# Bostanabad-Research-Group/GP-Plus

Hardware: AMD Instinct MI355X
Metric: MLL evals/sec (fwd+grad), NxN exact GP, N=20k d=8 (higher is better)
Workload: dtype f64; 1 GPU; C2: synthetic Borehole (Sobol seed 0, unique rows, z-scored) N=20000 d=8 fp64, GP_Plus Rough_RBF exact GP at theta1, one replica per GPU (restart-parallel); N=20000, d=8, streams_per_gpu=1

## Files before the change

### gp-plus_amd/_lib.py

```python
from __future__ import annotations

import ctypes
import os
import subprocess
from ctypes import POINTER, c_char_p, c_double, c_int, c_int32, c_int64, c_size_t, c_void_p
from pathlib import Path

import torch

_PKG_DIR = Path(__file__).resolve().parent
_LIB_PATH = _PKG_DIR / "libgpp_hip.so"
_CSRC = _PKG_DIR / "csrc"

_SIGNATURES = {
    "gpp_version": (c_char_p, []),
    "gpp_create": (c_int, [POINTER(c_void_p), c_int]),
    "gpp_destroy": (c_int, [c_void_p]),
    "gpp_set_stream": (c_int, [c_void_p, c_void_p]),
    "gpp_internal_stream": (c_int, [c_void_p, c_int, POINTER(c_void_p)]),
    "gpp_set_option": (c_int, [c_void_p, c_int, c_int]),
    "gpp_workspace_bytes": (c_size_t, [c_void_p, c_int, c_int64, c_int64, c_int, c_int]),
    "gpp_set_workspace": (c_int, [c_void_p, c_void_p, c_size_t]),
    "gpp_kernel_build": (c_int, [c_void_p, c_void_p, c_int64, c_int, c_void_p, c_void_p, c_void_p, c_void_p, c_int,
                                 c_double, c_int, c_int, c_int, c_void_p, c_int64, c_int64, c_int64]),
    "gpp_cross_kernel": (c_int, [c_void_p, c_void_p, c_int64, c_void_p, c_int64, c_int, c_void_p, c_void_p, c_int,
                                 c_int, c_void_p, c_int64]),
    "gpp_kernel_apply": (c_int, [c_void_p, c_void_p, c_int64, c_void_p, c_int64, c_int, c_void_p, c_void_p, c_int, c_int, c_void_p,
                                 c_int64, c_int, c_double, c_void_p, c_int64]),
    "gpp_rff_apply": (c_int, [c_void_p, c_void_p, c_int64, c_int, c_void_p, c_void_p, c_int64, c_void_p, c_void_p, c_int64, c_int,
                              c_double, c_void_p, c_int64]),
    "gpp_kernel_apply_grad": (c_int, [c_void_p, c_void_p, c_int64, c_void_p, c_int64, c_int, c_void_p, c_void_p, c_int, c_int, c_void_p,
                                      c_int64, c_int, c_void_p, c_int64, c_double, c_void_p, c_int64]),
    "gpp_rff_apply_grad": (c_int, [c_void_p, c_void_p, c_int64, c_int, c_void_p, c_void_p, c_int64, c_void_p, c_void_p, c_int64, c_int,
                                   c_void_p, c_int64, c_double, c_void_p, c_int64]),
    "gpp_potrf": (c_int, [c_void_p, c_void_p, c_int64, c_int64, c_void_p, c_int64, c_void_p]),
    "gpp_potrf_ws": (c_int, [c_void_p, c_void_p, c_int64, c_int64, c_void_p, c_int64, c_void_p, c_int64, c_void_p]),
    "gpp_build_potrf_ws": (c_int, [c_void_p, c_void_p, c_int64, c_int, c_void_p, c_void_p, c_void_p, c_void_p, c_int, c_double, c_int,
                                   c_int, c_void_p, c_int64, c_void_p, c_int64, c_void_p, c_int64, c_void_p]),
    "gpp_trtri": (c_int, [c_void_p, c_void_p, c_int64, c_int64, c_void_p, c_int64, c_void_p, c_int64]),
    "gpp_lauum": (c_int, [c_void_p, c_void_p, c_int64, c_int64, c_void_p, c_int64]),
    "gpp_lauum_grad": (c_int, [c_void_p, c_void_p, c_int64, c_int64, c_void_p, c_int, c_void_p, c_void_p, c_void_p, c_int, c_int, c_int,
                               c_void_p, c_void_p, c_void_p, c_void_p]),
    "gpp_post_cov_train": (c_int, [c_void_p, c_void_p, c_int64, c_int64, c_void_p, c_void_p, c_int, c_void_p, c_double, c_void_p,
                                   c_int64]),
    "gpp_syrk_rows": (c_int, [c_void_p, c_void_p, c_int64, c_void_p, c_int64, c_int64, c_int64, c_int64, c_int64, c_int, c_int]),
    "gpp_gemm_lower_cols": (c_int, [c_void_p, c_void_p, c_int64, c_void_p, c_int64, c_void_p, c_int64, c_int64, c_int64, c_double,
                                    c_double, c_int64, c_int64, c_int, c_int, c_int64, c_int64, c_int]),
    "gpp_shard_list_begin": (c_int, [c_void_p, c_int64, c_int64, c_int, c_int, c_void_p, c_int64, c_void_p, c_void_p, c_int64, c_void_p,
                                     c_void_p, c_void_p, c_void_p, c_int64, c_void_p, c_int, POINTER(c_int)]),
    "gpp_shard_piece_cols": (c_int64, []),
    "gpp_shard_list_gate": (c_int, [c_void_p, c_void_p, c_int, c_int]),
    "gpp_shard_list_signal": (c_int, [c_void_p, c_void_p, c_int, c_int]),
    "gpp_shard_list_end": (c_int, [c_void_p]),
    "gpp_set_comm": (c_int, [c_void_p, c_void_p, c_int, c_int]),
    "gpp_comm_unique_id": (c_int, [c_void_p]),
    "gpp_comm_init_rccl": (c_int, [c_void_p, c_void_p, c_int, c_int]),
    "gpp_shard_buffer_doubles": (c_size_t, [c_int64, c_int64, c_int, c_int, c_int]),
    "gpp_shard_eval": (c_int, [c_void_p, c_int64, c_int64, c_void_p, c_int, c_void_p, c_void_p, c_void_p, c_void_p, c_int, c_int, c_int,
                               c_double, c_int, c_int, c_void_p, POINTER(c_int)]),
    "gpp_push_create": (c_int, [c_int, c_int, c_int, c_int64, POINTER(c_void_p), c_void_p]),
    "gpp_push_connect": (c_int, [c_void_p, c_void_p]),
    "gpp_push_send": (c_int, [c_void_p, c_void_p, c_int64, c_void_p, c_int, c_int, POINTER(c_void_p), POINTER(c_int64), POINTER(c_int64),
                              POINTER(c_int64), POINTER(c_int64), POINTER(c_int64)]),
    "gpp_push_recv": (c_int, [c_void_p, c_void_p, c_int64, c_void_p, c_int, c_int, POINTER(c_void_p), POINTER(c_int64), POINTER(c_int64),
                              POINTER(c_int64), POINTER(c_int64), POINTER(c_int64)]),
    "gpp_push_ack": (c_int, [c_void_p, c_void_p, c_int64]),
    "gpp_push_info": (c_int, [c_void_p, POINTER(c_int64), POINTER(c_int)]),
    "gpp_push_destroy": (c_int, [c_void_p, c_int]),
    "gpp_shard_back_list": (c_int, [c_void_p, c_int64, c_int64, c_int, c_int, c_void_p, c_int64, c_void_p, c_void_p, c_int64, c_void_p,
                                    c_void_p, c_int, POINTER(c_int)]),
    "gpp_trmv_lower_cols": (c_int, [c_void_p, c_void_p, c_int64, c_int64, c_void_p, c_void_p, c_int64, c_int, c_int, c_int, c_int]),
    "gpp_mll_scalars": (c_int, [c_void_p, c_void_p, c_int64, c_int64, c_void_p, c_void_p]),
    "gpp_grad_reduce_cols": (c_int, [c_void_p, c_void_p, c_int64, c_int, c_void_p, c_void_p, c_void_p, c_int, c_int, c_int,
                                     c_void_p, c_void_p, c_int64, c_int, c_int64, c_int, c_int, c_void_p, c_void_p, c_void_p,
                                     c_void_p, c_int]),
    "gpp_lauum_rows": (c_int, [c_void_p, c_void_p, c_int64, c_int64, c_void_p, c_int64, c_int, c_int]),
    "gpp_lauum_rows_range": (c_int, [c_void_p, c_void_p, c_int64, c_int64, c_void_p, c_int64, c_int, c_int, c_int64, c_int64]),
    "gpp_transpose": (c_int, [c_void_p, c_void_p, c_int64, c_int64, c_int64, c_void_p, c_int64]),
    "gpp_mll_reduce": (c_int, [c_void_p, c_void_p, c_int64, c_void_p, c_int64, c_int64, c_void_p, c_void_p, c_void_p]),
    "gpp_alpha": (c_int, [c_void_p, c_void_p, c_int64, c_int64, c_void_p, c_void_p]),
    "gpp_grad_reduce": (c_int, [c_void_p, c_void_p, c_int64, c_int, c_void_p, c_void_p, c_void_p, c_int, c_int, c_int,
                                c_void_p, c_void_p, c_int64, c_int, c_void_p, c_void_p, c_void_p, c_void_p]),
    "gpp_loo_scalars": (c_int, [c_void_p, c_void_p, c_int64, c_int64, c_void_p, c_void_p, c_void_p, c_void_p, c_void_p, c_void_p, c_void_p,
                                c_void_p]),
    "gpp_sym_rowscale": (c_int, [c_void_p, c_void_p, c_int64, c_int64, c_void_p, c_void_p, c_int64]),
    "gpp_loo_grad_reduce": (c_int, [c_void_p, c_void_p, c_int64, c_int, c_void_p, c_void_p, c_void_p, c_int, c_int, c_int,
                                    c_void_p, c_void_p, c_void_p, c_int64, c_int, c_void_p, c_void_p, c_void_p, c_void_p]),
    "gpp_grad_reduce_rows": (c_int, [c_void_p, c_void_p, c_int64, c_int, c_void_p, c_void_p, c_void_p, c_int, c_int, c_int,
                                     c_void_p, c_void_p, c_int64, c_int, c_int64, c_int, c_int, c_void_p, c_void_p, c_void_p,
                                     c_void_p]),
    "gpp_predict": (c_int, [c_void_p, c_void_p, c_int64, c_int64, c_void_p, c_void_p, c_int64, c_int64, c_void_p,
                            c_void_p, c_int64, c_void_p, c_void_p]),
    "gpp_predict_tn": (c_int, [c_void_p, c_void_p, c_int64, c_int64, c_void_p, c_void_p, c_int64, c_int64, c_void_p,
                               c_void_p, c_int64, c_void_p, c_void_p]),
    "gpp_cross_grad": (c_int, [c_void_p, c_void_p, c_int64, c_void_p, c_int64, c_int, c_void_p, c_void_p, c_int, c_int, c_void_p,
                               c_void_p, c_void_p, c_void_p, c_int64, c_void_p, c_int, c_void_p, c_int, c_void_p, c_void_p]),
    "gpp_gemm": (c_int, [c_void_p, c_int, c_int, c_int64, c_int64, c_int64, c_double, c_void_p, c_int64, c_void_p,
                         c_int64, c_double, c_void_p, c_int64, c_int, c_int, c_int, c_int, c_int]),
    "gpp_gemm_batched": (c_int, [c_void_p, c_int, c_int, c_int64, c_int64, c_int64, c_double, c_void_p, c_int64, c_int64,
                                 c_void_p, c_int64, c_int64, c_double, c_void_p, c_int64, c_int64, c_int, c_int, c_int, c_int,
                                 c_int, c_int]),
    "gpp_kernel_build_batched": (c_int, [c_void_p, c_void_p, c_int64, c_int64, c_int, c_void_p, c_void_p, c_void_p, c_void_p, c_int,
                                         c_double, c_int, c_int, c_int, c_void_p, c_int64, c_int64, c_int]),
    "gpp_potrf_batched": (c_int, [c_void_p, c_void_p, c_int64, c_int64, c_int64, c_void_p, c_int64, c_int64, c_void_p, c_int]),
    "gpp_trtri_batched": (c_int, [c_void_p, c_void_p, c_int64, c_int64, c_int64, c_void_p, c_int64, c_int64, c_void_p, c_int64,
                                  c_int64, c_int]),
    "gpp_lauum_batched": (c_int, [c_void_p, c_void_p, c_int64, c_int64, c_int64, c_void_p, c_int64, c_int64, c_int]),
    "gpp_mll_reduce_batched": (c_int, [c_void_p, c_void_p, c_int64, c_int64, c_void_p, c_int64, c_int64, c_int64, c_void_p,
                                       c_void_p, c_int64, c_void_p, c_int]),
    "gpp_alpha_batched": (c_int, [c_void_p, c_void_p, c_int64, c_int64, c_int64, c_void_p, c_void_p, c_int64, c_int]),
    "gpp_grad_reduce_batched": (c_int, [c_void_p, c_void_p, c_int64, c_int64, c_int, c_void_p, c_void_p, c_void_p, c_int, c_int,
                                        c_int, c_void_p, c_int64, c_void_p, c_int64, c_int64, c_int, c_void_p, c_void_p, c_void_p,
                                        c_void_p, c_int]),
    "gpp_loo_scalars_batched": (c_int, [c_void_p, c_void_p, c_int64, c_int64, c_int64, c_void_p, c_void_p, c_void_p, c_void_p, c_void_p,
                                        c_void_p, c_void_p, c_int64, c_void_p, c_int]),
    "gpp_sym_rowscale_batched": (c_int, [c_void_p, c_void_p, c_int64, c_int64, c_int64, c_void_p, c_int64, c_void_p, c_int64, c_int64,
                                         c_int]),
    "gpp_loo_grad_reduce_batched": (c_int, [c_void_p, c_void_p, c_int64, c_int64, c_int, c_void_p, c_void_p, c_void_p, c_int, c_int,
                                            c_int, c_void_p, c_void_p, c_int64, c_void_p, c_int64, c_int64, c_int, c_void_p, c_void_p,
                                            c_void_p, c_void_p, c_int]),
    "gpp_cv_blocks": (c_int, [c_void_p, c_void_p, c_int64, c_int64, c_void_p, c_void_p, c_int, c_int, c_void_p, c_int64, c_int64]),
    "gpp_cv_rows": (c_int, [c_void_p, c_void_p, c_int64, c_int64, c_void_p, c_void_p, c_int, c_void_p, c_int64, c_int64, c_void_p,
                            c_int64]),
    "gpp_chol_append": (c_int, [c_void_p, c_void_p, c_int64, c_void_p, c_int64, c_int64, c_int64, c_void_p, c_int64, c_void_p, c_int64,
                                c_void_p, c_void_p, c_void_p, c_void_p]),
    "gpp_post_cross_sq": (c_int, [c_void_p, c_void_p, c_int64, c_void_p, c_int64, c_int, c_void_p, c_void_p, c_int, c_int, c_void_p,
                                  c_int64, c_void_p, c_int64, c_int64, c_int, c_void_p, c_void_p]),
    "gpp_post_cross_min": (c_int, [c_void_p, c_void_p, c_int64, c_void_p, c_int64, c_int, c_void_p, c_void_p, c_int, c_int, c_void_p,
                                   c_int64, c_void_p, c_int64, c_int64, c_int, c_void_p, c_void_p, c_void_p, c_int, c_void_p]),
}

_lib = None


class GppError(RuntimeError):
    """A libgpp_hip call returned a non-zero status."""


def build(force: bool = False) -> Path:
    if force:
        subprocess.run(["make", "-C", str(_CSRC), "clean"], check=True, capture_output=True)
    proc = subprocess.run(["make", "-C", str(_CSRC), "-j4"], capture_output=True, text=True)
    if proc.returncode != 0:
        raise RuntimeError("building libgpp_hip.so failed:\n" + proc.stdout + proc.stderr)
    return _LIB_PATH


def load() -> ctypes.CDLL:
    global _lib
    if _lib is not None:
        return _lib
    if not _LIB_PATH.exists():
        raise GppError(
            f"{_LIB_PATH} not found: the HIP extension is required (build it with "
            f"`make -C {_CSRC}` or `python -c 'import __graft_entry__ as g; g.build()'`); there is no CPU fallback."
        )
    lib = ctypes.CDLL(os.fspath(_LIB_PATH))
    for name, (restype, argtypes) in _SIGNATURES.items():
        fn = getattr(lib, name)
        fn.restype = restype
        fn.argtypes = argtypes
    _lib = lib
    return lib


def exported_symbols() -> list:
    return sorted(_SIGNATURES)


def check(status: int, what: str) -> None:
    if status == 0:
        return
    if status < 0:
        raise GppError(f"{what}: bad argument #{-status}")
    raise GppError(f"{what}: HIP runtime error {status - 1000}")
```

### gp-plus_amd/backend.py

```python
from __future__ import annotations

import atexit
import ctypes
import os
import threading
import weakref
from typing import Dict, Optional, Tuple

import torch

from . import _lib, settings
from ._lib import GppError, check

KIND_RBF, KIND_MATERN32, KIND_MATERN52 = 0, 1, 2
UPLO_FULL, UPLO_LOWER, UPLO_UPPER = 0, 1, 2
OPT_COOP_PANEL, OPT_PANEL_FAULT, OPT_PANEL_TIMEOUT_MS, OPT_EXEC_SCHED, OPT_DAG_SCHED = 1, 2, 3, 4, 5
OPT_GEMM_TILE = 6
OP_MLL_EVAL, OP_PREDICT, OP_PREDICT_GRAD = 0, 1, 2
OP_APPLY = 3
OP_APPLY_GRAD = 4
OP_APPEND = 5
OP_POST_CROSS = 6
OP_POST_CROSS_MIN = 7
MAX_NODES = 64
APPLY_SPLIT = 2048
NOT_SUPPORTED = 2001
NO_WORKSPACE = 2002
MAX_FEATURES = 64


def _check_features(D: int) -> None:
    if D < 1 or D > MAX_FEATURES:
        raise GppError(f"the covariance kernels take 1..{MAX_FEATURES} feature columns per point (got {D})")

_contexts: Dict[Tuple[int, int], "GppContext"] = {}
_contexts_lock = threading.Lock()


def _ptr(t: Optional[torch.Tensor]) -> Optional[int]:
    return None if t is None else t.data_ptr()


def _need(t: torch.Tensor, dtype, name: str) -> None:
    if not t.is_cuda:
        raise GppError(f"{name} must live on the GPU (got {t.device}); libgpp_hip has no CPU path")
    if t.dtype != dtype:
        raise GppError(f"{name} must be {dtype} (got {t.dtype})")
    if not t.is_contiguous() and t.dim() == 1:
        raise GppError(f"{name} must be contiguous")


INFO_PANEL_TIMEOUT = 1 << 30
INFO_EXEC_TIMEOUT = (1 << 30) | (1 << 29)


def check_status(info: int) -> None:
    if info >= INFO_PANEL_TIMEOUT:
        what = "an executor launch" if info & (1 << 29) else "the cooperative panel kernel"
        raise GppError(f"gpp_potrf: {what} timed out waiting for one of its work-groups (another kernel holding the stream's CUs "
                       "for seconds, or a caller-supplied CU-masked stream with fewer CUs than the launch assumed); "
                       "GPP_COOP_PANEL=0 selects the leaf-step factorisation, GPP_DAG_SCHED=0 the launch-per-product one")


def panel_timed_out(ctx: "GppContext", info: int) -> bool:
    if info < INFO_PANEL_TIMEOUT:
        return False
    import warnings

    ms = info & 0xFFFFF
    if info & (1 << 29):
        if not ctx.dag_sched:
            check_status(info)
        warnings.warn(f"libgpp_hip: an executor launch timed out after {ms} ms (another tenant of this GPU held part of its CUs, or "
                      "dispatches are serialised); this context now factors with one launch per product", RuntimeWarning)
        ctx.set_option(OPT_DAG_SCHED, 0)
        return True
    if not ctx.coop_panel:
        check_status(info)
    warnings.warn(f"libgpp_hip: a cooperative panel launch timed out after {ms} ms (another tenant of this GPU held part "
                  "of its CUs); this context now factors with leaf-step launches", RuntimeWarning)
    ctx.set_option(OPT_COOP_PANEL, 0)
    return True


def row_stride(n: int) -> int:
    return max(16, (n + 15) // 16 * 16)


def rows_buffer(m: int, n: int, device) -> torch.Tensor:
    return torch.empty((m, row_stride(n)), dtype=torch.float64, device=device)[:, :n]


def square_buffer(n: int, device) -> torch.Tensor:
    return rows_buffer(n, n, device)


def _ld(m: torch.Tensor) -> int:
    if m.dim() != 2 or m.stride(1) != 1:
        raise GppError("matrix must be 2-D with unit column stride")
    return m.stride(0) if m.shape[0] > 1 else max(m.shape[1], m.stride(0))


def _on_own_device(fn):
    import functools

    @functools.wraps(fn)
    def wrapper(self, *args, **kwargs):
        if torch.cuda.current_device() == self.index:
            return fn(self, *args, **kwargs)
        with torch.cuda.device(self.index):
            return fn(self, *args, **kwargs)

    return wrapper


class GppContext:
    def __init__(self, device: torch.device):
        if device.type != "cuda":
            raise GppError("GppContext needs a cuda (HIP) device; there is no CPU fallback")
        if not torch.cuda.is_available():
            raise GppError("no GPU visible to PyTorch: the HIP path cannot run")
        self.lib = _lib.load()
        self.device = device
        self.index = device.index if device.index is not None else torch.cuda.current_device()
        h = ctypes.c_void_p()
        with torch.cuda.device(self.index):
            check(self.lib.gpp_create(ctypes.byref(h), self.index), "gpp_create")
        self.h = h
        self.coop_panel = settings.ENV_COOP_PANEL
        self.dag_sched = settings.ENV_DAG_SCHED
        if any(os.environ.get(v, "0") not in ("", "0") for v in ("HIP_LAUNCH_BLOCKING", "AMD_SERIALIZE_KERNEL", "CUDA_LAUNCH_BLOCKING")):
            self.set_option(OPT_DAG_SCHED, 0)
        self._ws: Optional[torch.Tensor] = None

    def _stream(self) -> None:
        s = torch.cuda.current_stream(self.index).cuda_stream
        check(self.lib.gpp_set_stream(self.h, ctypes.c_void_p(s)), "gpp_set_stream")

    def set_option(self, option: int, value: int) -> None:
        check(self.lib.gpp_set_option(self.h, int(option), int(value)), "gpp_set_option")
        if option == OPT_COOP_PANEL:
            self.coop_panel = bool(value)
        elif option in (OPT_DAG_SCHED, OPT_EXEC_SCHED):
            self.dag_sched = bool(value)

    @_on_own_device
    def internal_streams(self):
        if getattr(self, "_istreams", None) is None:
            out = []
            for which in (0, 1, 2):
                p = ctypes.c_void_p()
                check(self.lib.gpp_internal_stream(self.h, which, ctypes.byref(p)), "gpp_internal_stream")
                out.append(torch.cuda.ExternalStream(p.value, device=self.device))
            self._istreams = tuple(out)
        return self._istreams

    @_on_own_device
    def ensure_workspace(self, op: int, N: int, M: int, D: int, S: int) -> None:
        need = int(self.lib.gpp_workspace_bytes(self.h, op, N, M, D, S))
        if self._ws is None or self._ws.numel() < need:
            self._ws = torch.empty(need, dtype=torch.uint8, device=self.device)
            check(self.lib.gpp_set_workspace(self.h, self._ws.data_ptr(), self._ws.numel()), "gpp_set_workspace")

    def _check_groups(self, grp: torch.Tensor, N: int, S: int) -> None:
        _need(grp, torch.int32, "grp")
        if grp.numel() != N:
            raise GppError(f"noise-group index has {grp.numel()} entries for {N} points (stale fidel_indices?)")
        seen = getattr(self, "_grp_ok", None)
        if seen is None or seen[0]() is not grp or seen[1:] != (grp._version, N, S):
            lo, hi = int(grp.min()), int(grp.max())
# ... 16 lines not shown
        if not U.is_contiguous():
            raise GppError("U must be contiguous")
        self._stream()
        check(self.lib.gpp_kernel_build(self.h, U.data_ptr(), N, D, w.data_ptr(), sf2.data_ptr(), _ptr(tau), _ptr(grp), S,
                                        float(jitter), kind, d_split, uplo, out.data_ptr(), _ld(out), row0,
                                        N - row0 if nrows is None else nrows), "gpp_kernel_build")
        return out

    @_on_own_device
    def cross_kernel(self, Ua, Ub, w, sf2, out, *, kind=KIND_RBF, d_split=0):
        _check_features(Ua.shape[1])
        for t, n in ((Ua, "Ua"), (Ub, "Ub"), (w, "w"), (sf2, "sf2"), (out, "Kab")):
            _need(t, torch.float64, n)
        if not (Ua.is_contiguous() and Ub.is_contiguous()):
            raise GppError("Ua/Ub must be contiguous")
        self._stream()
        check(self.lib.gpp_cross_kernel(self.h, Ua.data_ptr(), Ua.shape[0], Ub.data_ptr(), Ub.shape[0], Ua.shape[1],
                                        w.data_ptr(), sf2.data_ptr(), kind, d_split, out.data_ptr(), _ld(out)),
              "gpp_cross_kernel")
        return out

    def _apply_checks(self, Ua, second, C, out, sf2, g_Ua=None):
        M, D = Ua.shape
        L, S = C.shape
        _check_features(D)
        for t, n in ((Ua, "Ua"), (second, "Ub / Omega"), (C, "C / Theta"), (out, "Out")):
            _need(t, torch.float64, n)
        if not (Ua.is_contiguous() and second.is_contiguous()):
            raise GppError("Ua and Ub / Omega must be contiguous")
        if second.shape != (L, D):
            raise GppError(f"the second operand must be {L} x {D} (got {tuple(second.shape)})")
        if out.shape != (M, S):
            raise GppError(f"Out must be {M} x {S} (got {tuple(out.shape)})")
        if min(M, L, S) < 1:
            raise GppError("gpp_kernel_apply / gpp_rff_apply take M, N (F), S >= 1")
        _need(sf2, torch.float64, "sf2")
        if sf2.numel() < 1:
            raise GppError("sf2 must hold one value")
        if g_Ua is not None:
            _need(g_Ua, torch.float64, "g_Ua")
            if g_Ua.shape != (M, D):
                raise GppError(f"g_Ua must be {M} x {D} (got {tuple(g_Ua.shape)})")
        self.ensure_workspace(OP_APPLY if g_Ua is None else OP_APPLY_GRAD, L, M, D, S)
        return M, D, L, S

    @_on_own_device
    def kernel_apply(self, Ua, Ub, w, sf2, C, out, *, beta=0.0, kind=KIND_RBF, d_split=0):
        M, D, N, S = self._apply_checks(Ua, Ub, C, out, sf2)
        _need(w, torch.float64, "w")
        if w.numel() != D:
            raise GppError(f"w has {w.numel()} entries for {D} features")
        self._stream()
        check(self.lib.gpp_kernel_apply(self.h, Ua.data_ptr(), M, Ub.data_ptr(), N, D, w.data_ptr(), sf2.data_ptr(), kind, d_split,
                                        C.data_ptr(), _ld(C), S, float(beta), out.data_ptr(), _ld(out)), "gpp_kernel_apply")
        return out

    @_on_own_device
    def rff_apply(self, Ua, omega, phase, sf2, theta, out, *, beta=0.0):
        M, D, F, S = self._apply_checks(Ua, omega, theta, out, sf2)
        _need(phase, torch.float64, "phase")
        if phase.numel() != F:
            raise GppError(f"phase has {phase.numel()} entries for {F} features")
        self._stream()
        check(self.lib.gpp_rff_apply(self.h, Ua.data_ptr(), M, D, omega.data_ptr(), phase.data_ptr(), F, sf2.data_ptr(),
                                     theta.data_ptr(), _ld(theta), S, float(beta), out.data_ptr(), _ld(out)), "gpp_rff_apply")
        return out

    @_on_own_device
    def kernel_apply_grad(self, Ua, Ub, w, sf2, C, gbar, g_Ua, *, beta=0.0, kind=KIND_RBF, d_split=0):
        M, D, N, S = self._apply_checks(Ua, Ub, C, gbar, sf2, g_Ua)
        _need(w, torch.float64, "w")
        if w.numel() != D:
            raise GppError(f"w has {w.numel()} entries for {D} features")
        self._stream()
        check(self.lib.gpp_kernel_apply_grad(self.h, Ua.data_ptr(), M, Ub.data_ptr(), N, D, w.data_ptr(), sf2.data_ptr(), kind, d_split,
                                             C.data_ptr(), _ld(C), S, gbar.data_ptr(), _ld(gbar), float(beta), g_Ua.data_ptr(),
                                             _ld(g_Ua)), "gpp_kernel_apply_grad")
        return g_Ua

    @_on_own_device
    def rff_apply_grad(self, Ua, omega, phase, sf2, theta, gbar, g_Ua, *, beta=0.0):
        M, D, F, S = self._apply_checks(Ua, omega, theta, gbar, sf2, g_Ua)
        _need(phase, torch.float64, "phase")
        if phase.numel() != F:
            raise GppError(f"phase has {phase.numel()} entries for {F} features")
        self._stream()
        check(self.lib.gpp_rff_apply_grad(self.h, Ua.data_ptr(), M, D, omega.data_ptr(), phase.data_ptr(), F, sf2.data_ptr(),
                                          theta.data_ptr(), _ld(theta), S, gbar.data_ptr(), _ld(gbar), float(beta), g_Ua.data_ptr(),
                                          _ld(g_Ua)), "gpp_rff_apply_grad")
        return g_Ua

    @_on_own_device
    def potrf(self, A, Linv, info, T=None):
        _need(A, torch.float64, "A"); _need(Linv, torch.float64, "Linv"); _need(info, torch.int32, "info")
        self._stream()
        if T is None:
            check(self.lib.gpp_potrf(self.h, A.data_ptr(), A.shape[0], _ld(A), Linv.data_ptr(), _ld(Linv), info.data_ptr()),
                  "gpp_potrf")
        else:
            check(self.lib.gpp_potrf_ws(self.h, A.data_ptr(), A.shape[0], _ld(A), Linv.data_ptr(), _ld(Linv), T.data_ptr(),
                                        _ld(T), info.data_ptr()), "gpp_potrf_ws")

    @_on_own_device
    def build_potrf(self, U, w, sf2, tau, grp, A, Linv, info, T, *, jitter=0.0, kind=KIND_RBF, d_split=0):
        N, D = U.shape
        _check_features(D)
        for t, n in ((U, "U"), (w, "w"), (sf2, "sf2"), (A, "A"), (Linv, "Linv"), (T, "T")):
            _need(t, torch.float64, n)
        _need(info, torch.int32, "info")
        if tau is not None:
            _need(tau, torch.float64, "tau")
        S = 0 if tau is None else tau.numel()
        if grp is not None:
            self._check_groups(grp, N, S)
        if not U.is_contiguous():
            raise GppError("U must be contiguous")
        self._stream()
        check(self.lib.gpp_build_potrf_ws(self.h, U.data_ptr(), N, D, w.data_ptr(), sf2.data_ptr(), _ptr(tau), _ptr(grp), S,
                                          float(jitter), kind, d_split, A.data_ptr(), _ld(A), Linv.data_ptr(), _ld(Linv),
                                          T.data_ptr(), _ld(T), info.data_ptr()), "gpp_build_potrf_ws")

    @_on_own_device
    def trtri(self, U, Linv, T):
        self._stream()
        check(self.lib.gpp_trtri(self.h, U.data_ptr(), U.shape[0], _ld(U), Linv.data_ptr(), _ld(Linv), T.data_ptr(), _ld(T)),
              "gpp_trtri")

    @_on_own_device
    def lauum(self, Linv, Kinv):
        self._stream()
        check(self.lib.gpp_lauum(self.h, Linv.data_ptr(), Linv.shape[0], _ld(Linv), Kinv.data_ptr(), _ld(Kinv)), "gpp_lauum")

    @_on_own_device
    def lauum_grad(self, Linv, U, w, sf2, grp, S, alpha, dU, g_w, g_sf2, g_tau, *, kind=KIND_RBF) -> bool:
        N, D = U.shape
        for t, n in ((Linv, "Linv"), (U, "U"), (w, "w"), (sf2, "sf2"), (alpha, "alpha"), (g_w, "g_w"), (g_sf2, "g_sf2"),
                     (g_tau, "g_tau")):
            _need(t, torch.float64, n)
        if grp is not None:
            self._check_groups(grp, N, S)
        if not U.is_contiguous():
            raise GppError("U must be contiguous")
        self.ensure_workspace(OP_MLL_EVAL, N, 0, D, S)
        self._stream()
        status = self.lib.gpp_lauum_grad(self.h, Linv.data_ptr(), N, _ld(Linv), U.data_ptr(), D, w.data_ptr(), sf2.data_ptr(),
                                         _ptr(grp), S, kind, dU, alpha.data_ptr(), g_w.data_ptr(), g_sf2.data_ptr(),
                                         g_tau.data_ptr())
        if status == NOT_SUPPORTED:
            return False
        if status == NO_WORKSPACE:
            raise GppError("gpp_lauum_grad: the handle's scratch workspace is missing or too small")
        check(status, "gpp_lauum_grad")
        return True

    @_on_own_device
    def post_cov_train(self, Kinv, tau, grp, d, out, *, jitter=0.0):
        N = Kinv.shape[0]
        for t, n in ((Kinv, "Kinv"), (tau, "tau"), (out, "A")):
            _need(t, torch.float64, n)
        if d is not None:
            _need(d, torch.float64, "d")
            if d.numel() != N or not d.is_contiguous():
                raise GppError(f"d must be a contiguous vector of {N} doubles")
        if grp is not None:
            self._check_groups(grp, N, tau.numel())
        if out.shape[0] != N or out.shape[1] != N:
            raise GppError("post_cov_train: shapes do not match")
        self._stream()
        check(self.lib.gpp_post_cov_train(self.h, Kinv.data_ptr(), N, _ld(Kinv), tau.data_ptr(), _ptr(grp), tau.numel(), _ptr(d),
                                          float(jitter), out.data_ptr(), _ld(out)), "gpp_post_cov_train")
        return out

    @_on_own_device
    def syrk_rows(self, Urow, C, nb, first_block, rank, nranks):
        self._stream()
        check(self.lib.gpp_syrk_rows(self.h, Urow.data_ptr(), _ld(Urow), C.data_ptr(), _ld(C), C.shape[0], Urow.shape[0], nb,
                                     first_block, rank, nranks), "gpp_syrk_rows")

    @_on_own_device
    def shard_list_begin(self, N, nb, rank, nranks, A, Kc, Lc, D, W, info, workers=0) -> bool:
        self._stream()
        used = ctypes.c_int(0)
        check(self.lib.gpp_shard_list_begin(self.h, N, nb, rank, nranks, A.data_ptr(), _ld(A), Kc.data_ptr(), Lc.data_ptr(), _ld(Kc),
                                            D.data_ptr(), W[0].data_ptr(), W[1].data_ptr(), W[2].data_ptr(), _ld(W[0]),
                                            info.data_ptr(), int(workers), ctypes.byref(used)), "gpp_shard_list_begin")
        return bool(used.value)

    def shard_messages(self, N: int, nb: int, k: int):
        o, o2 = k * nb, min((k + 2) * nb, N)
        W = int(self.lib.gpp_shard_piece_cols()) or N
        return [(o, o2)] + [(c, min(c + W, N)) for c in range(o2, N, W)]

    @_on_own_device
    def shard_list_gate(self, stream, tail: int, k: int) -> None:
        check(self.lib.gpp_shard_list_gate(self.h, ctypes.c_void_p(stream.cuda_stream), int(tail), k), "gpp_shard_list_gate")

    @_on_own_device
    def shard_list_signal(self, stream, tail: int, k: int) -> None:
        check(self.lib.gpp_shard_list_signal(self.h, ctypes.c_void_p(stream.cuda_stream), int(tail), k), "gpp_shard_list_signal")

    @_on_own_device
    def shard_list_end(self) -> None:
        self._stream()
        check(self.lib.gpp_shard_list_end(self.h), "gpp_shard_list_end")

    @_on_own_device
    def shard_back_list(self, N, nb, rank, nranks, A, Kc, Lc, D, info, workers=0) -> bool:
        self._stream()
        used = ctypes.c_int(0)
        check(self.lib.gpp_shard_back_list(self.h, N, nb, rank, nranks, A.data_ptr(), _ld(A), Kc.data_ptr(), Lc.data_ptr(), _ld(Kc),
                                           D.data_ptr(), info.data_ptr(), int(workers), ctypes.byref(used)), "gpp_shard_back_list")
        return bool(used.value)

    @_on_own_device
    def gemm_lower_cols(self, A, B, C, alpha, beta, nb, first_block, rank, nranks, row0=0, row1=None, compact=False):
        M, K = A.shape[1], A.shape[0]
        if compact:
            if B.shape[0] != K or C.shape[0] != M:
                raise GppError("gemm_lower_cols: shapes do not match")
        elif A.shape != B.shape or C.shape[0] != C.shape[1] or C.shape[0] != M:
            raise GppError("gemm_lower_cols: shapes do not match")
        self._stream()
        check(self.lib.gpp_gemm_lower_cols(self.h, A.data_ptr(), _ld(A), B.data_ptr(), _ld(B), C.data_ptr(), _ld(C), M,
                                           K, float(alpha), float(beta), nb, first_block, rank, nranks, row0,
                                           M if row1 is None else row1, 1 if compact else 0),
              "gpp_gemm_lower_cols")

    @_on_own_device
    def trmv_lower_cols(self, T, x, y, nb, rank, nranks, trans=False, compact=False):
        for t, n in ((x, "x"), (y, "y")):
            _need(t, torch.float64, n)
        if trans:
            self.ensure_workspace(OP_MLL_EVAL, T.shape[0], 0, 1, 1)
        self._stream()
        check(self.lib.gpp_trmv_lower_cols(self.h, T.data_ptr(), _ld(T), T.shape[0], x.data_ptr(), y.data_ptr(), nb, rank, nranks,
                                           1 if trans else 0, 1 if compact else 0), "gpp_trmv_lower_cols")

    @_on_own_device
    def mll_scalars(self, U, z, out3):
        self._stream()
        check(self.lib.gpp_mll_scalars(self.h, U.data_ptr(), _ld(U), U.shape[0], z.data_ptr(), out3.data_ptr()), "gpp_mll_scalars")

    @_on_own_device
    def lauum_rows(self, Linv, Kinv, rank, nranks):
        self._stream()
        check(self.lib.gpp_lauum_rows(self.h, Linv.data_ptr(), Linv.shape[0], _ld(Linv), Kinv.data_ptr(), _ld(Kinv), rank, nranks),
              "gpp_lauum_rows")

    @_on_own_device
    def lauum_rows_range(self, Linv, Kinv, rank, nranks, row0, row1):
        self._stream()
        check(self.lib.gpp_lauum_rows_range(self.h, Linv.data_ptr(), Linv.shape[0], _ld(Linv), Kinv.data_ptr(), _ld(Kinv), rank,
                                            nranks, row0, row1), "gpp_lauum_rows_range")

    @_on_own_device
    def transpose(self, src, dst):
        if src.shape[0] != dst.shape[1] or src.shape[1] != dst.shape[0]:
            raise GppError("transpose: shapes do not match")
        self._stream()
        check(self.lib.gpp_transpose(self.h, src.data_ptr(), src.stride(0), src.shape[0], src.shape[1], dst.data_ptr(), dst.stride(0)),
              "gpp_transpose")

    @_on_own_device
    def mll_reduce(self, L, Linv, r, z, out3):
        for t, n in ((r, "r"), (z, "z"), (out3, "out3")):
            _need(t, torch.float64, n)
        self._stream()
        check(self.lib.gpp_mll_reduce(self.h, L.data_ptr(), _ld(L), Linv.data_ptr(), _ld(Linv), L.shape[0], r.data_ptr(),
                                      z.data_ptr(), out3.data_ptr()), "gpp_mll_reduce")

    @_on_own_device
    def alpha(self, Linv, z, alpha):
        N = Linv.shape[0]
        self._stream()
        check(self.lib.gpp_alpha(self.h, Linv.data_ptr(), _ld(Linv), N, z.data_ptr(), alpha.data_ptr()), "gpp_alpha")

    @_on_own_device
    def grad_reduce(self, U, w, sf2, grp, S, alpha, Kinv, dU, g_w, g_sf2, g_tau, g_U, *, kind=KIND_RBF, d_split=0):
        N, D = U.shape
        if grp is not None:
            self._check_groups(grp, N, S)
        self.ensure_workspace(OP_MLL_EVAL, N, 0, D, S)
        self._stream()
        check(self.lib.gpp_grad_reduce(self.h, U.data_ptr(), N, D, w.data_ptr(), sf2.data_ptr(), _ptr(grp), S, kind,
                                       d_split, alpha.data_ptr(), Kinv.data_ptr(), _ld(Kinv), dU, g_w.data_ptr(),
                                       g_sf2.data_ptr(), g_tau.data_ptr(), _ptr(g_U)), "gpp_grad_reduce")

    @_on_own_device
    def loo_scalars(self, Linv, alpha, y, d, mu=None, s2=None, a=None, sqrtb=None, loo=None):
        N = Linv.shape[0]
        _need(Linv, torch.float64, "Linv")
        for t, n, size in ((alpha, "alpha", N), (y, "y", N), (d, "d", N), (mu, "mu", N), (s2, "s2", N), (a, "a", N),
                           (sqrtb, "sqrtb", N), (loo, "loo", 1)):
            if t is None:
                continue
            _need(t, torch.float64, n)
            if t.numel() < size or not t.is_contiguous():
                raise GppError(f"{n} must be a contiguous vector of {size} doubles")
        if mu is not None and y is None:
            raise GppError("loo_scalars: mu needs y")
        self._stream()
        check(self.lib.gpp_loo_scalars(self.h, Linv.data_ptr(), _ld(Linv), N, alpha.data_ptr(), _ptr(y), d.data_ptr(), _ptr(mu),
                                       _ptr(s2), _ptr(a), _ptr(sqrtb), _ptr(loo)), "gpp_loo_scalars")

    @_on_own_device
    def sym_rowscale(self, Kinv, s, out):
# ... 467 lines not shown
```

### gp-plus_amd/csrc/gpp_api.hip

```cpp
#include "../../include/gpp.h"
#include "gpp_internal.h"

#include <algorithm>
#include <cmath>
#include <cstdio>
#include <cstdlib>
#include <cstring>
#include <new>

const GppEnv& gpp_env() {
  static const GppEnv env = [] {
    auto num = [](const char* name, long long unset) { const char* v = getenv(name); return v ? atoll(v) : unset; };
    GppEnv e;
    e.coop_panel = num("GPP_COOP_PANEL", 1) != 0;
    e.dag_sched = num("GPP_DAG_SCHED", 1) != 0;
    e.dag_phased = num("GPP_DAG_PHASED", 0) != 0;
    e.shard_list = num("GPP_SHARD_LIST", 1) != 0;
    e.shard_workers = (int)num("GPP_SHARD_WORKERS", 0);
    e.shard_fill = (int)num("GPP_SHARD_FILL", -1);
    e.shard_timeout_ms = num("GPP_SHARD_TIMEOUT_MS", 60000);
    const int64_t cols = num("GPP_SHARD_PIECE_COLS", 8192);
    e.shard_piece_cols = cols <= 0 ? (int64_t)0 : std::max<int64_t>(GPP_TILE, cols / GPP_TILE * GPP_TILE);
    e.sharded_force_collectives = num("GPP_SHARDED_FORCE_COLLECTIVES", 0) != 0;
    e.exec_verbose = getenv("GPP_EXEC_VERBOSE") != nullptr;
    e.dag_dump = (int)num("GPP_DAG_DUMP", 0);
    e.dag_check_verbose = getenv("GPP_DAG_CHECK_VERBOSE") != nullptr;
    return e;
  }();
  return env;
}

namespace {

constexpr int NBLK = GPP_TILE;
constexpr int64_t LOOKAHEAD_NB = 1024;

inline int rc(hipError_t e) { return e == hipSuccess ? 0 : 1000 + (int)e; }
#define GPP_TRY(expr)                   \
  do {                                  \
    hipError_t _e = (expr);             \
    if (_e != hipSuccess) return rc(_e); \
  } while (0)

inline bool aligned16(const void* p) { return (reinterpret_cast<uintptr_t>(p) & 15) == 0; }

GemmArgs mk(const double* A, int64_t lda, const double* B, int64_t ldb, double* C, int64_t ldc, int64_t M, int64_t N,
            int64_t K, double alpha, double beta) {
  GemmArgs g{};
  g.A = A; g.B = B; g.C = C;
  g.lda = lda; g.ldb = ldb; g.ldc = ldc;
  g.M = (int)M; g.N = (int)N; g.K = (int)K;
  g.alpha = alpha; g.beta = beta;
  return g;
}

inline int64_t split(int64_t n) {
  int64_t h = ((n / 2 + NBLK - 1) / NBLK) * NBLK;
  if (h >= n) h -= NBLK;
  return h;
}

struct Ctx {
  hipStream_t s;
  double* A; int64_t ld;
  double* Li; int64_t ldi;
  int32_t* info;
};

hipError_t trsm_rec(const Ctx& c, int64_t c0, int64_t m, int64_t o, int64_t n) {
  if (m <= 0 || n <= 0) return hipSuccess;
  if (n <= NBLK) {
    double* Bp = c.A + o * c.ld + c0;
    GemmArgs g = mk(c.Li + o * c.ldi + o, c.ldi, Bp, c.ld, Bp, c.ld, n, m, n, 1.0, 0.0);
    g.a_mask = 1;
    return gpp_launch_gemm(c.s, 2, g, 1, NBLK, (m + NBLK - 1) / NBLK >= 512 ? NBLK : 32);
  }
  const int64_t n1 = split(n), n2 = n - n1;
  hipError_t e = trsm_rec(c, c0, m, o, n1);
  if (e != hipSuccess) return e;
  GemmArgs g = mk(c.A + o * c.ld + (o + n1), c.ld, c.A + o * c.ld + c0, c.ld, c.A + (o + n1) * c.ld + c0, c.ld, n2, m, n1,
                  -1.0, 1.0);
  e = gpp_launch_gemm(c.s, 2, g, 1);
  if (e != hipSuccess) return e;
  return trsm_rec(c, c0, m, o + n1, n2);
}

constexpr int64_t BLK_MAX = 6144;
hipError_t potrf_blk(const Ctx& c, int64_t o, int64_t n) {
  for (int64_t j0 = 0; j0 < n; j0 += NBLK) {
    const int64_t nb = std::min<int64_t>(NBLK, n - j0), oo = o + j0, rem = n - j0 - nb;
    hipError_t e = gpp_launch_leaf(c.s, c.A + oo * c.ld + oo, c.ld, c.Li + oo * c.ldi + oo, c.ldi, (int)nb, c.info, (int)oo);
    if (e != hipSuccess) return e;
    if (rem == 0) break;
    double* Bp = c.A + oo * c.ld + (oo + nb);
    GemmArgs g = mk(c.Li + oo * c.ldi + oo, c.ldi, Bp, c.ld, Bp, c.ld, nb, rem, nb, 1.0, 0.0);
    g.a_mask = 1;
    e = gpp_launch_gemm(c.s, 2, g, 1, NBLK, 32);
    if (e != hipSuccess) return e;
    GemmArgs u = mk(Bp, c.ld, Bp, c.ld, c.A + (oo + nb) * c.ld + (oo + nb), c.ld, rem, rem, nb, -1.0, 1.0);
    u.c_lower = 2;
    e = gpp_launch_gemm(c.s, 2, u, 1, 32, 32);
    if (e != hipSuccess) return e;
  }
  return hipSuccess;
}

hipError_t potrf_blk_batched(const Ctx& c, int64_t n, int batch, int64_t sA, int64_t sLi) {
  for (int64_t j0 = 0; j0 < n; j0 += NBLK) {
    const int64_t nb = std::min<int64_t>(NBLK, n - j0), oo = j0, rem = n - j0 - nb;
    hipError_t e = gpp_launch_leaf(c.s, c.A + oo * c.ld + oo, c.ld, c.Li + oo * c.ldi + oo, c.ldi, (int)nb, c.info, (int)oo,
                                   batch, sA, sLi);
    if (e != hipSuccess) return e;
    if (rem == 0) break;
    double* Bp = c.A + oo * c.ld + (oo + nb);
    GemmArgs g = mk(c.Li + oo * c.ldi + oo, c.ldi, Bp, c.ld, Bp, c.ld, nb, rem, nb, 1.0, 0.0);
    g.a_mask = 1;
    g.sA = sLi; g.sB = sA; g.sC = sA;
    e = gpp_launch_gemm(c.s, 2, g, batch, NBLK, 32);
    if (e != hipSuccess) return e;
    GemmArgs u = mk(Bp, c.ld, Bp, c.ld, c.A + (oo + nb) * c.ld + (oo + nb), c.ld, rem, rem, nb, -1.0, 1.0);
    u.c_lower = 2;
    u.sA = sA; u.sB = sA; u.sC = sA;
    e = gpp_launch_gemm(c.s, 2, u, batch, 32, 32);
    if (e != hipSuccess) return e;
  }
  return hipSuccess;
}

hipError_t potrf_rec(const Ctx& c, int64_t o, int64_t n) {
  if (n <= 0) return hipSuccess;
  if (n <= NBLK)
    return gpp_launch_leaf(c.s, c.A + o * c.ld + o, c.ld, c.Li + o * c.ldi + o, c.ldi, (int)n, c.info, (int)o);
  if (n <= BLK_MAX) return potrf_blk(c, o, n);
  const int64_t n1 = split(n), n2 = n - n1;
  hipError_t e = potrf_rec(c, o, n1);
  if (e != hipSuccess) return e;
  e = trsm_rec(c, o + n1, n2, o, n1);
  if (e != hipSuccess) return e;
  const double* U12 = c.A + o * c.ld + (o + n1);
  GemmArgs g = mk(U12, c.ld, U12, c.ld, c.A + (o + n1) * c.ld + (o + n1), c.ld, n2, n2, n1, -1.0, 1.0);
  g.c_lower = 2;
  e = gpp_launch_gemm(c.s, 2, g, 1);
  if (e != hipSuccess) return e;
  return potrf_rec(c, o + n1, n2);
}

constexpr int64_t PANEL_MAX_N = 2048;
inline bool panel_fits(const gpp_handle_s* h, int64_t n) {
  return h->coop_panel && h->panel_flags && h->ncu >= 2 && n > 2 * NBLK && n <= PANEL_MAX_N && (n + NBLK - 1) / NBLK <= gpp_panel_max_leaves();
}
hipError_t launch_panel_at(gpp_handle_s* h, const Ctx& c, int64_t o, int64_t n, int max_wgs) {
  if (h->panel_fault) {
    h->panel_fault = 0;
    return gpp_launch_fill_i32(c.s, c.info, 1, GPP_INFO_PANEL_TIMEOUT);
  }
  hipStreamCaptureStatus cap = hipStreamCaptureStatusNone;
  if (hipStreamIsCapturing(c.s, &cap) != hipSuccess) {
    (void)hipGetLastError();
    cap = hipStreamCaptureStatusNone;
  }
  int slot;
  if (cap == hipStreamCaptureStatusActive) slot = GPP_PANEL_RING + (h->cap_next++ % GPP_PANEL_CAP_RING);
  else slot = h->panel_next++ % GPP_PANEL_RING;
  int* fl = reinterpret_cast<int*>(h->panel_flags + (size_t)slot * gpp_panel_flag_bytes());
  return gpp_launch_panel(c.s, c.A, c.ld, c.Li, c.ldi, (int)n, c.info, (int)o, fl, max_wgs, h->panel_timeout_ms);
}

hipError_t launch_panel(gpp_handle_s* h, const Ctx& c, int64_t o, int64_t n, int max_wgs) {
  Ctx b = c;
// ... 438 lines not shown
    (void)hipGetLastError();
    (void)dag_abort(h, P);
  }
  hipEvent_t E = next_event(h), F = next_event(h);
  HIP_TRY(hipEventRecord(E, cu.s));
  HIP_TRY(hipEventRecord(F, cp.s));
  HIP_TRY(hipStreamWaitEvent(cm.s, E, 0));
  HIP_TRY(hipStreamWaitEvent(cm.s, F, 0));
  HIP_TRY(hipEventRecord(P->last_use, cm.s));
  if (perr != hipSuccess) return perr;
  dag_note_inverted(h, P, N);
  *used = true;
  return hipSuccess;
}

inline int64_t owned_cols(int64_t N, int64_t nb, int rank, int nranks) {
  const int64_t nblk = (N + nb - 1) / nb;
  int64_t cols = 0;
  for (int64_t b = rank; b < nblk; b += nranks) cols += std::min(nb, N - b * nb);
  return cols;
}

int check_mat(const void* p, int64_t ld, int64_t n, int argi) {
  if (!p) return -argi;
  if (!aligned16(p) || (ld & 1) || ld < n) return -(argi + 1);
  return 0;
}

}

extern "C" {

#ifndef GPP_SRC_HASH
#define GPP_SRC_HASH "unknown"
#endif
const char* gpp_version(void) { return "gpp_hip 0.3 (gfx950, fp64 MFMA) src " GPP_SRC_HASH; }

#ifdef GPP_PANEL_STAMP
int gpp_debug_panel_flags(gpp_handle_t h, int* out, int nints, int* next_slot) {
  if (next_slot) *next_slot = h->panel_next % GPP_PANEL_RING;
  return (int)hipMemcpy(out, h->panel_flags, (size_t)nints * sizeof(int), hipMemcpyDeviceToHost);
}
#endif

static DagPlan* dag_mru(gpp_handle_t h) {
  DagPlan* P = nullptr;
  if (h)
    for (int i = 0; i < GPP_DAG_PLANS; ++i)
      if (h->dag_plans[i] && (!P || h->dag_plans[i]->stamp > P->stamp)) P = h->dag_plans[i];
  return P;
}
int gpp_debug_split_builds(gpp_handle_t h) { return h ? h->split_builds : -1; }
int gpp_debug_dag_info(gpp_handle_t h, int64_t* info8) {
  const DagPlan* P = dag_mru(h);
  if (!P) return -1;
  info8[8] = P->inv_rows;
  info8[9] = P->N;
  info8[0] = (int64_t)P->tasks.size(); info8[1] = (int64_t)P->groups.size(); info8[2] = P->B; info8[3] = P->nt;
  info8[4] = P->ncounters; info8[5] = (int64_t)(P->sim_ms * 1000.0); info8[6] = (int64_t)(P->sim_busy * 1000.0); info8[7] = P->flags;
  return 0;
}
int gpp_debug_dag_counters(gpp_handle_t h, int* out, int nmax) {
  DagPlan* P = dag_mru(h);
  if (!P || !P->d_counters) return -1;
  if (hipDeviceSynchronize() != hipSuccess) return 1;
  std::vector<int> c(P->ncounters);
  if (hipMemcpy(c.data(), P->d_counters, c.size() * sizeof(int), hipMemcpyDeviceToHost) != hipSuccess) return 2;
  int n = 0;
  auto put = [&](int v) { if (n < nmax) out[n++] = v; };
  put(c[0]); put(c[1]); put(P->B);
  for (int b = 0; b < P->B; ++b) put(c[P->c_pd + b]);
  for (int b = 0; b < P->B; ++b) put(c[P->c_g1d + b]);
  if (P->flags & DAG_SHARD) {
    for (int b = 0; b < P->B; ++b) put(c[P->c_cph + b]);
    for (int b = 0; b < P->B; ++b) put(c[P->c_cpt + b * P->GP]);
    for (int b = 0; b < P->B; ++b) put(c[P->c_art + b * P->GP]);
  }
  return n;
}
int gpp_debug_dag_trace(gpp_handle_t h, int on) {
  DagPlan* P = dag_mru(h);
  if (!P) return -1;
  if (hipDeviceSynchronize() != hipSuccess) return 1;
  if (on && !P->d_trace) {
    if (hipMalloc(&P->d_trace, 4 * P->tasks.size() * sizeof(unsigned long long)) != hipSuccess) return 2;
    (void)hipMemset(P->d_trace, 0, 4 * P->tasks.size() * sizeof(unsigned long long));
  } else if (!on && P->d_trace) {
    (void)hipFree(P->d_trace);
    P->d_trace = nullptr;
  }
  return 0;
}
int gpp_debug_dag_fetch(gpp_handle_t h, void* tasks, void* trace) {
  const DagPlan* P = dag_mru(h);
  if (!P) return -1;
  if (hipDeviceSynchronize() != hipSuccess) return 1;
  if (tasks) memcpy(tasks, P->tasks.data(), P->tasks.size() * sizeof(DagTask));
  if (trace) {
    if (!P->d_trace) return 2;
    if (hipMemcpy(trace, P->d_trace, 4 * P->tasks.size() * sizeof(unsigned long long), hipMemcpyDeviceToHost) != hipSuccess) return 3;
  }
  return 0;
}

int gpp_create(gpp_handle_t* out, int device) {
  if (!out) return -1;
  int ndev = 0;
  hipError_t e = hipGetDeviceCount(&ndev);
  if (e != hipSuccess) return rc(e);
  if (device < 0 || device >= ndev) return -2;
  e = hipSetDevice(device);
  if (e != hipSuccess) return rc(e);
  gpp_handle_s* h = new (std::nothrow) gpp_handle_s();
  if (!h) return rc(hipErrorOutOfMemory);
  h->device = device;
  h->stream = nullptr;
  h->ws = nullptr;
  h->ws_bytes = 0;
  h->panel_stream = nullptr;
  h->upd_stream = nullptr;
  h->fill_stream = nullptr;
  h->full_stream = nullptr;
  h->cu_split = -1;
  h->panel_cus = 0;
  h->n_events = 0;
  h->ev_next = 0;
  h->inv_N = 0;
  h->inv_nblocks = 0;
  h->panel_flags = nullptr;
  h->panel_next = 0;
  h->coop_panel = gpp_env().coop_panel ? 1 : 0;
  h->panel_fault = 0;
  h->panel_timeout_ms = 500;
  for (int i = 0; i < GPP_DAG_PLANS; ++i) h->dag_plans[i] = nullptr;
  h->shard_cur = nullptr;
  h->shard_info = nullptr;
  h->shard_ready = nullptr;
  h->dag_clock = 0;
  h->dag_sched = 1;
  h->gemm_tile = 0;
  h->ncu = 0;
  if (hipDeviceGetAttribute(&h->ncu, hipDeviceAttributeMultiprocessorCount, device) != hipSuccess || h->ncu < 2) {
    (void)hipGetLastError();
    h->ncu = 0;
  }
  h->cap_next = 0;
  h->handoff = nullptr;
  if (hipMalloc(reinterpret_cast<void**>(&h->panel_flags), (GPP_PANEL_RING + GPP_PANEL_CAP_RING) * gpp_panel_flag_bytes()) != hipSuccess ||
      hipMemset(h->panel_flags, 0, (GPP_PANEL_RING + GPP_PANEL_CAP_RING) * gpp_panel_flag_bytes()) != hipSuccess) {
    (void)hipGetLastError();
    if (h->panel_flags) (void)hipFree(h->panel_flags);
    h->panel_flags = nullptr;
  }
  *out = h;
  return 0;
}

int gpp_destroy(gpp_handle_t h) {
  if (!h) return -1;
  for (hipStream_t s : {h->panel_stream, h->upd_stream, h->fill_stream, h->full_stream})
    if (s) (void)hipStreamSynchronize(s);
  if (h->full_stream) (void)hipStreamDestroy(h->full_stream);
  if (h->fill_stream) (void)hipStreamDestroy(h->fill_stream);
  if (h->upd_stream) (void)hipStreamDestroy(h->upd_stream);
  if (h->panel_stream) (void)hipStreamDestroy(h->panel_stream);
  for (int i = 0; i < h->n_events; ++i) (void)hipEventDestroy(h->events[i]);
  if (h->handoff) (void)hipEventDestroy(h->handoff);
  if (h->shard_ready) (void)hipEventDestroy(h->shard_ready);
  if (h->panel_flags) (void)hipFree(h->panel_flags);
  for (int i = 0; i < GPP_DAG_PLANS; ++i)
    if (h->dag_plans[i]) gpp_dag_free(h->dag_plans[i]);
  gpp_shard_release_comm(h);
  delete h;
  return 0;
}

int gpp_set_stream(gpp_handle_t h, void* stream) {
  if (!h) return -1;
  hipStream_t s = reinterpret_cast<hipStream_t>(stream);
  if (s != h->stream) {
    hipStreamCaptureStatus a = hipStreamCaptureStatusNone, b = hipStreamCaptureStatusNone;
    if (hipStreamIsCapturing(h->stream, &a) != hipSuccess || hipStreamIsCapturing(s, &b) != hipSuccess) {
      (void)hipGetLastError();
      a = b = hipStreamCaptureStatusActive;
    }
    auto internal = [&](hipStream_t q) { return q && (q == h->panel_stream || q == h->upd_stream || q == h->fill_stream || q == h->full_stream); };
    if (a == hipStreamCaptureStatusNone && b == hipStreamCaptureStatusNone && !internal(s) && !internal(h->stream)) {
      if (!h->handoff) GPP_TRY(hipEventCreateWithFlags(&h->handoff, hipEventDisableTiming));
      GPP_TRY(hipEventRecord(h->handoff, h->stream));
      GPP_TRY(hipStreamWaitEvent(s, h->handoff, 0));
    }
    h->stream = s;
  }
  return 0;
}

int gpp_set_option(gpp_handle_t h, int option, int value) {
  if (!h) return -1;
  if (option == GPP_OPT_COOP_PANEL) h->coop_panel = value ? 1 : 0;
  else if (option == GPP_OPT_PANEL_FAULT) h->panel_fault = value ? 1 : 0;
  else if (option == GPP_OPT_DAG_SCHED || option == GPP_OPT_EXEC_SCHED) h->dag_sched = value ? 1 : 0;
  else if (option == GPP_OPT_PANEL_TIMEOUT_MS) {
    if (value < 1 || value > 60000) return -3;
    h->panel_timeout_ms = value;
  } else if (option == GPP_OPT_GEMM_TILE) {
    if (value < 0 || value > 4) return -3;
    h->gemm_tile = value;
  } else return -2;
  return 0;
}

int gpp_internal_stream(gpp_handle_t h, int which, void** out) {
  if (!h) return -1;
  if (which < 0 || which > 2) return -2;
  if (!out) return -3;
  GPP_TRY(ensure_streams(h));
  *out = reinterpret_cast<void*>(which == 0 ? h->panel_stream : which == 1 ? h->upd_stream : h->full_stream);
  return 0;
}

constexpr int64_t SHARD_LIST_MIN_N = 4096;
static long long shard_budget(const gpp_handle_s* h) {
  (void)h;
  return gpp_env().shard_timeout_ms * 100000;
}

int gpp_shard_list_begin(gpp_handle_t h, int64_t N, int64_t nb, int rank, int nranks, double* A, int64_t ld, double* Kc, double* Lc,
                         int64_t ldc, double* D, double* W0, double* W1, double* W2, int64_t ldw, int32_t* info, int workers,
                         int* used) {
  if (!h) return -1;
  if (!used) return -18;
  *used = 0;
  if (N < 2 || nb < 128 || nb % 128 != 0) return -2;
  if (rank < 0 || nranks < 1 || rank >= nranks) return -4;
  if (int e = check_mat(A, ld, N, 6)) return e;
  if (!Kc || !aligned16(Kc)) return -8;
  if (!Lc || !aligned16(Lc)) return -9;
  const int64_t wc = ((N + nb - 1) / nb - rank + nranks - 1) / nranks * nb;
  if ((ldc & 1) || ldc < wc) return -10;
  if (!D || !aligned16(D)) return -11;
  if (!W0 || !W1 || !W2 || !aligned16(W0) || !aligned16(W1) || !aligned16(W2)) return -12;
  if ((ldw & 1) || ldw < N) return -15;
  if (!info) return -16;
  if (h->shard_cur) return -1;
  const GppEnv& env = gpp_env();
  if (workers <= 0 && env.shard_workers > 0) workers = env.shard_workers;
  if (!env.shard_list || !h->dag_sched || !h->coop_panel || N < SHARD_LIST_MIN_N || N > DAG_MAX_N) return 0;
  GPP_TRY(ensure_streams(h));
  if (h->cu_split != 1) return 0;
  if (!panel_fits(h, nb)) return 0;
  const int flags = DAG_INV | DAG_SHARD;
  const int nworkers = workers > 0 ? workers : 2 * (h->ncu - h->panel_cus);
  DagPlan* P = dag_plan_cached(h, PlanKey{N, nb, ld, ldc, ldw, flags, N, rank, nranks, workers}, [&]() -> DagPlan* {
    DagTuning tune = gpp_dag_default_tuning();
    tune.workers = nworkers;
    tune.fill = env.shard_fill >= 0 ? env.shard_fill : workers > 0 ? 0 : (nranks > 1 ? h->panel_cus : 2 * h->panel_cus);
    tune.inv_rows = 0;
    tune.fuse = dag_fuse(N);
    DagPlan* Q = gpp_dag_plan(N, nb, ld, ldc, ldw, 0, flags, tune, rank, nranks);
    if (!Q) return nullptr;
    Q->workers = workers;
    Q->fill = tune.fill;
    if (gpp_dag_upload(Q) != hipSuccess) {
      (void)hipGetLastError();
      gpp_dag_free(Q);
      return nullptr;
    }
    return Q;
  });
  if (!P) return 0;
  hipStream_t sm = h->stream, sp = h->panel_stream, su = h->upd_stream;
  GPP_TRY(gpp_launch_fill_i32(sm, P->d_counters, P->ncounters, 0));
  DagBases bases{{reinterpret_cast<char*>(A), reinterpret_cast<char*>(Kc), reinterpret_cast<char*>(Lc), reinterpret_cast<char*>(D),
                  reinterpret_cast<char*>(W0), reinterpret_cast<char*>(W1), reinterpret_cast<char*>(W2), nullptr}};
  GPP_TRY(gpp_launch_dag_bind(sm, P->d_groups, P->d_groups_abs, (int)P->groups.size(), bases));
  if (!h->shard_ready) GPP_TRY(hipEventCreateWithFlags(&h->shard_ready, hipEventDisableTiming));
  hipEvent_t ev = h->shard_ready;
  GPP_TRY(hipEventRecord(ev, sm));
  GPP_TRY(hipStreamWaitEvent(sp, ev, 0));
  GPP_TRY(hipStreamWaitEvent(su, ev, 0));
  const long long budget = shard_budget(h);
  DagLaunch dl{};
  dl.groups = P->d_groups_abs; dl.tasks = P->d_tasks; dl.ntasks = (int)P->tasks.size();
  dl.counters = P->d_counters; dl.info = info; dl.budget = budget;
  dl.max_tasks = 0; dl.quit_id = -1; dl.quit_val = 0; dl.ticket_limit = 0;
  dl.trace = P->d_trace; dl.tag = 0;
  if (dl.ntasks > 0) GPP_TRY(gpp_launch_dag(su, nworkers, dl));
  Ctx cp{sp, A, ld, D, nb, info};
  auto enqueue_panel_stream = [&]() -> int {
    for (const DagPlan::Op& op : P->stream_ops) {
      const int b = op.arg;
      const int64_t o = (int64_t)b * nb, rows = std::min(nb, N - o);
      if (op.kind == 0) {
        GPP_TRY(gpp_launch_exec_gate(sp, P->d_counters, P->c_g1d + b, P->gate_target[b], info, budget));
      } else if (op.kind == 1) {
        Ctx cb = cp;
        cb.A = A + o * ld + o;
        cb.Li = D + (int64_t)b * nb * nb;
        GPP_TRY(launch_panel_at(h, cb, o, rows, h->panel_cus));
      } else if (op.kind == 2) {
        GPP_TRY(gpp_launch_exec_signal(sp, P->d_counters, P->c_pd + b));
      } else {
        DagLaunch fl = dl;
        fl.max_tasks = op.arg;
        fl.quit_id = op.n >= 0 ? P->c_g1d + op.n : -1;
        fl.quit_val = 1;
        fl.ticket_limit = op.lim;
        fl.tag = op.n >= 0 ? op.n : P->B;
        GPP_TRY(gpp_launch_dag(sp, std::max(P->fill, 1), fl));
      }
    }
    return 0;
  };
  const int erc = enqueue_panel_stream();
  h->shard_cur = P;
  h->shard_info = info;
  if (erc != 0) {
    (void)hipGetLastError();
    (void)dag_abort(h, P);
    return erc;
  }
  *used = 1;
  return 0;
}

static int shard_pieces(const DagPlan* P, int k) {
  const int hi = P->tb[std::min(k + 2, P->B)];
  return hi >= P->nt ? 0 : (P->nt - hi + P->piece_tiles - 1) / P->piece_tiles;
}
int gpp_shard_list_gate(gpp_handle_t h, void* stream, int tail, int k) {
  if (!h || !h->shard_cur) return -1;
  const DagPlan* P = h->shard_cur;
  if (k < 0 || k >= P->B || k % P->nranks != P->rank) return -4;
  if (tail < 0 || tail > shard_pieces(P, k)) return -3;
  hipStream_t s = reinterpret_cast<hipStream_t>(stream);
  const long long budget = shard_budget(h);
  GPP_TRY(hipStreamWaitEvent(s, h->shard_ready, 0));
  GPP_TRY(gpp_launch_exec_gate(s, P->d_counters, P->c_pd + k, 1, h->shard_info, budget));
  const int piece = k * P->GP + tail - 1;
  const int target = tail ? P->cpt_target[piece] : P->cph_target[k];
  if (target > 0) GPP_TRY(gpp_launch_exec_gate(s, P->d_counters, tail ? P->c_cpt + piece : P->c_cph + k, target, h->shard_info, budget));
  return 0;
}

int gpp_shard_list_signal(gpp_handle_t h, void* stream, int tail, int k) {
  if (!h || !h->shard_cur) return -1;
  const DagPlan* P = h->shard_cur;
  if (k < 0 || k >= P->B || k % P->nranks == P->rank) return -4;
  if (tail < 0 || tail > shard_pieces(P, k)) return -3;
  GPP_TRY(hipStreamWaitEvent(reinterpret_cast<hipStream_t>(stream), h->shard_ready, 0));
  return rc(gpp_launch_exec_signal(reinterpret_cast<hipStream_t>(stream), P->d_counters, tail ? P->c_art + k * P->GP + tail - 1 : P->c_pd + k));
}

int gpp_shard_list_end(gpp_handle_t h) {
// ... 214 lines not shown
  if (ldu < D) return -16;
  if (gpp_apply_pieces(F) > 1 && (!h->ws || h->ws_bytes < gpp_apply_ws_bytes(F, M, D))) return GPP_NO_WORKSPACE;
  GPP_TRY(gpp_launch_rff_apply_grad(h->stream, Ua, M, D, Omega, phase, F, sf2, Theta, ldt, S, Gbar, ldg, beta, g_Ua, ldu, h->ws,
                                    h->ws_bytes));
  return 0;
}

static int potrf_ws_impl(gpp_handle_t h, double* A, int64_t N, int64_t ld, double* Linv, int64_t ldi, double* T, int64_t ldt,
                         int32_t* info_dev, const KyBuild* build) {
  if (!h) return -1;
  if (N < 0) return -3;
  if (int r = check_mat(A, ld, N, 2)) return r;
  if (int r = check_mat(Linv, ldi, N, 5)) return r;
  if (T) {
    if (int r = check_mat(T, ldt, N, 7)) return r;
  }
  if (!info_dev) return -9;
  GPP_TRY(gpp_launch_fill_i32(h->stream, info_dev, 1, 0));
  Ctx c{h->stream, A, ld, Linv, ldi, info_dev};
  h->inv_N = N;
  h->inv_nblocks = 0;
  const int64_t la_min = T ? BORDER_MIN_N : 6 * LOOKAHEAD_NB;
  bool dag_used = false;
  hipStreamCaptureStatus cap = hipStreamCaptureStatusNone;
  if (build) GPP_TRY(hipStreamIsCapturing(h->stream, &cap));
  if (build && cap != hipStreamCaptureStatusNone) {
    GPP_TRY((*build)(h->stream, c, N, 0, N));
    build = nullptr;
  }
  GPP_TRY(potrf_dag(h, c, N, T, ldt, &dag_used, build));
  if (dag_used) return 0;
  if (build) GPP_TRY((*build)(h->stream, c, N, 0, N));
  if (N >= la_min) {
    GPP_TRY(potrf_lookahead(h, c, N, LOOKAHEAD_NB, T, ldt));
  } else if (panel_fits(h, N)) {
    int wgs = h->ncu;
    if (h->cu_split == 1 && h->stream == h->panel_stream) wgs = h->panel_cus;
    else if (h->cu_split == 1 && (h->stream == h->upd_stream || h->stream == h->fill_stream)) wgs = h->ncu - h->panel_cus;
    else if (h->stream) {
      uint32_t mask[32] = {0};
      if (hipExtStreamGetCUMask(h->stream, 32, mask) == hipSuccess) {
        int cus = 0;
        for (int c = 0; c < h->ncu && c < 1024; ++c) cus += (mask[c >> 5] >> (c & 31)) & 1u;
        if (cus >= 2 && cus < wgs) wgs = cus;
      } else {
        (void)hipGetLastError();
      }
    }
    GPP_TRY(launch_panel(h, c, 0, N, wgs));
    h->inv_nblocks = 1;
    h->inv_o[0] = 0;
    h->inv_n[0] = N;
  } else {
    GPP_TRY(potrf_rec(c, 0, N));
  }
  return 0;
}

int gpp_potrf_ws(gpp_handle_t h, double* A, int64_t N, int64_t ld, double* Linv, int64_t ldi, double* T, int64_t ldt,
                 int32_t* info_dev) {
  return potrf_ws_impl(h, A, N, ld, Linv, ldi, T, ldt, info_dev, nullptr);
}

int gpp_build_potrf_ws(gpp_handle_t h, const double* U, int64_t N, int D, const double* w, const double* sf2, const double* tau,
                       const int32_t* grp, int S, double jitter, int kind, int d_split, double* A, int64_t ld, double* Linv,
                       int64_t ldi, double* T, int64_t ldt, int32_t* info_dev) {
  if (!h) return -1;
  if (!U) return -2;
  if (N < 0) return -3;
  if (D < 1 || D > 64) return -4;
  if (!w) return -5;
  if (!sf2) return -6;
  if (tau && S < 1) return -9;
  if (kind < 0 || kind > 2) return -11;
  if (d_split < 0 || d_split > D) return -12;
  if (int r = check_mat(A, ld, N, 13)) return r;
  if (int r = check_mat(Linv, ldi, N, 15)) return r;
  if (T) {
    if (int r = check_mat(T, ldt, N, 17)) return r;
  }
  if (!info_dev) return -19;
  const KyBuild build{U, w, sf2, tau, grp, D, S, kind, d_split, jitter};
  return potrf_ws_impl(h, A, N, ld, Linv, ldi, T, ldt, info_dev, &build);
}

int gpp_potrf(gpp_handle_t h, double* A, int64_t N, int64_t ld, double* Linv, int64_t ldi, int32_t* info_dev) {
  const int r = gpp_potrf_ws(h, A, N, ld, Linv, ldi, nullptr, 0, info_dev);
  return r == -9 ? -7 : r;
}

int gpp_trtri(gpp_handle_t h, const double* U, int64_t N, int64_t ld, double* Linv, int64_t ldi, double* T, int64_t ldt) {
  if (!h) return -1;
  if (N < 0) return -3;
  if (int r = check_mat(U, ld, N, 2)) return r;
  if (int r = check_mat(Linv, ldi, N, 5)) return r;
  if (int r = check_mat(T, ldt, N, 7)) return r;
  const bool have = (h->inv_N == N && h->inv_nblocks > 0);
  for (int64_t s = NBLK; s < N; s *= 2) {
    auto skip = [&](int64_t b) {
      if (!have) return false;
      for (int i = 0; i < h->inv_nblocks; ++i)
        if (b >= h->inv_o[i] && b + 2 * s <= h->inv_o[i] + h->inv_n[i]) return true;
      for (int i = 0; i < h->inv_nblocks; ++i)
        if (b >= h->inv_o[i] && h->inv_o[i] + h->inv_n[i] == N && b + s < N) return true;
      return false;
    };
    GPP_TRY(trtri_level(h->stream, U, ld, Linv, ldi, T, ldt, 0, N, s, skip));
  }
  h->inv_N = 0;
  return 0;
}

int gpp_lauum(gpp_handle_t h, const double* Linv, int64_t N, int64_t ldi, double* Kinv, int64_t ldk) {
  if (!h) return -1;
  if (N < 0) return -3;
  if (int r = check_mat(Linv, ldi, N, 2)) return r;
  if (int r = check_mat(Kinv, ldk, N, 5)) return r;
  GemmArgs g = mk(Linv, ldi, Linv, ldi, Kinv, ldk, N, N, N, 1.0, 0.0);
  g.a_mask = 2; g.b_mask = 2; g.klo_mode = 3; g.c_lower = 1; g.tag = 1;
  const int t = N <= 2560 ? 32 : N <= 5120 ? 64 : NBLK;
  GPP_TRY(gpp_launch_gemm(h->stream, 2, g, 1, t, t));
  return 0;
}

int gpp_lauum_grad(gpp_handle_t h, const double* Linv, int64_t N, int64_t ldi, const double* U, int D, const double* w,
                   const double* sf2, const int32_t* grp, int S, int kind, int dU, const double* alpha, double* g_w,
                   double* g_sf2, double* g_tau) {
  if (!h) return -1;
  if (N < 0) return -3;
  if (int r = check_mat(Linv, ldi, N, 2)) return r;
  if (!U) return -5;
  if (D < 1 || D > 64) return -6;
  if (!w) return -7;
  if (!sf2) return -8;
  if (S < 1 || S > 64) return -10;
  if (kind < 0 || kind > 2) return -11;
  if (dU < 0 || dU > D) return -12;
  if (!alpha) return -13;
  if (!g_w) return -14;
  if (!g_sf2) return -15;
  if (!g_tau) return -16;
  if (kind != GPP_KIND_RBF || D > 16 || dU != 0) return GPP_NOT_SUPPORTED;
  if (!h->ws || h->ws_bytes < gpp_lauum_grad_ws_bytes(N, D)) return GPP_NO_WORKSPACE;
  GemmArgs g = mk(Linv, ldi, Linv, ldi, nullptr, ldi, N, N, N, 1.0, 0.0);
  g.a_mask = 2; g.b_mask = 2; g.klo_mode = 3; g.c_lower = 1;
  const int64_t tiles = (N + NBLK - 1) / NBLK, nrec = tiles * (tiles + 1) / 2;
  double* rec = reinterpret_cast<double*>(h->ws);
  double* wdiag = rec + nrec * (D + 1);
  GPP_TRY(gpp_launch_lauum_grad(h->stream, g, GradEpiArgs{U, w, sf2, alpha, rec, wdiag, D}));
  GPP_TRY(gpp_launch_grad_finish(h->stream, rec, nrec, D, S, wdiag, grp, N, g_w, g_sf2, g_tau));
  return 0;
}

int gpp_post_cov_train(gpp_handle_t h, const double* Kinv, int64_t N, int64_t ldk, const double* tau, const int32_t* grp, int S,
                       const double* d, double jitter, double* A, int64_t lda) {
  if (!h) return -1;
  if (N < 0) return -3;
  if (int r = check_mat(Kinv, ldk, N, 2)) return r;
  if (!tau) return -5;
  if (S < 1) return -7;
  if (int r = check_mat(A, lda, N, 10)) return r;
  if (A == Kinv && lda != ldk) return -11;
  GPP_TRY(gpp_launch_post_cov_train(h->stream, Kinv, ldk, N, tau, grp, d, jitter, A, lda));
  return 0;
}

int gpp_lauum_rows(gpp_handle_t h, const double* Linv, int64_t N, int64_t ldi, double* Kinv, int64_t ldk, int rank, int nranks) {
  if (!h) return -1;
  if (N < 0) return -3;
  if (int r = check_mat(Linv, ldi, N, 2)) return r;
  if (int r = check_mat(Kinv, ldk, N, 5)) return r;
  if (nranks < 1 || rank < 0 || rank >= nranks) return -7;
  GemmArgs g = mk(Linv, ldi, Linv, ldi, Kinv, ldk, N, N, N, 1.0, 0.0);
  g.a_mask = 2; g.b_mask = 2; g.klo_mode = 3; g.c_lower = 1; g.tag = 1;
  g.row_mod = nranks; g.row_off = rank;
  GPP_TRY(gpp_launch_gemm(h->stream, 2, g, 1, NBLK, NBLK));
  return 0;
}

int gpp_lauum_rows_range(gpp_handle_t h, const double* Linv, int64_t N, int64_t ldi, double* Kinv, int64_t ldk, int rank,
                         int nranks, int64_t row0, int64_t row1) {
  if (!h) return -1;
  if (N < 0) return -3;
  if (int r = check_mat(Linv, ldi, N, 2)) return r;
  if (int r = check_mat(Kinv, ldk, N, 5)) return r;
  if (nranks < 1 || rank < 0 || rank >= nranks) return -7;
  if (row0 < 0 || row1 < row0 || row1 > N || (row0 % NBLK) != 0) return -9;
  if (row1 == row0) return 0;
  GemmArgs g = mk(Linv, ldi, Linv, ldi, Kinv, ldk, N, N, N, 1.0, 0.0);
  g.a_mask = 2; g.b_mask = 2; g.klo_mode = 3; g.c_lower = 1; g.tag = 1;
  g.row_mod = nranks; g.row_off = rank;
  const int64_t t0 = row0 / NBLK, t1 = (row1 + NBLK - 1) / NBLK;
  auto first_i = [&](int64_t t) { return t <= rank ? (int64_t)0 : (t - rank + nranks - 1) / nranks; };
  g.row_i0 = (int)first_i(t0);
  g.row_i1 = (int)first_i(t1);
  if (g.row_i1 <= g.row_i0) return 0;
  GPP_TRY(gpp_launch_gemm(h->stream, 2, g, 1, NBLK, NBLK));
  return 0;
}

int gpp_transpose(gpp_handle_t h, const double* src, int64_t lds, int64_t rows, int64_t cols, double* dst, int64_t ldd) {
  if (!h) return -1;
  if (!src || lds < cols) return -2;
  if (rows < 0 || cols < 0) return -4;
  if (!dst || ldd < rows) return -6;
  GPP_TRY(gpp_launch_transpose(h->stream, src, lds, rows, cols, dst, ldd));
  return 0;
}

int gpp_syrk_rows(gpp_handle_t h, const double* Urow, int64_t ldu, double* C, int64_t ldc, int64_t Nt, int64_t K, int64_t nb,
                  int64_t first_block, int rank, int nranks) {
  if (!h) return -1;
  if (!Urow || !aligned16(Urow) || (ldu & 1)) return -2;
  if (!C || !aligned16(C) || (ldc & 1)) return -4;
  if (Nt < 0 || K < 0) return -6;
  if (nb < NBLK || nb % NBLK != 0) return -8;
  if (first_block < 0) return -9;
  if (nranks < 1 || rank < 0 || rank >= nranks) return -10;
  if (Nt == 0 || K == 0) return 0;
  GemmArgs g = mk(Urow, ldu, Urow, ldu, C, ldc, Nt, Nt, K, -1.0, 1.0);
  g.c_lower = 2;
  g.own_mod = nranks;
  g.own_bt = (int)(nb / NBLK);
  g.own_off = (int)(((first_block - rank) % nranks + nranks) % nranks);
  GPP_TRY(gpp_launch_gemm(h->stream, 2, g, 1, NBLK, NBLK));
  return 0;
}

int gpp_gemm_lower_cols(gpp_handle_t h, const double* A, int64_t lda, const double* B, int64_t ldb, double* C, int64_t ldc,
                        int64_t M, int64_t K, double alpha, double beta, int64_t nb, int64_t first_block, int rank, int nranks,
                        int64_t row0, int64_t row1, int compact) {
  if (!h) return -1;
  if (!A || !aligned16(A) || (lda & 1)) return -2;
  if (!B || !aligned16(B) || (ldb & 1)) return -4;
  if (!C || !aligned16(C) || (ldc & 1)) return -6;
  if (M < 0 || K < 0) return -8;
  if (nb < NBLK || nb % NBLK != 0) return -12;
  if (first_block < 0) return -13;
  if (nranks < 1 || rank < 0 || rank >= nranks) return -14;
  if (row0 < 0 || row1 < row0 || row1 > M || row0 % NBLK != 0) return -16;
  if (M == 0 || K == 0 || row1 == row0) return 0;
  GemmArgs g = mk(A, lda, B, ldb, C, ldc, M, M, K, alpha, beta);
  g.c_lower = 1;
  g.row_t0 = (int)(row0 / NBLK);
  g.row_t1 = (int)((row1 + NBLK - 1) / NBLK);
  g.own_mod = nranks;
  g.own_bt = (int)(nb / NBLK);
  g.own_off = (int)(((first_block - rank) % nranks + nranks) % nranks);
  g.compact_bc = compact ? 1 : 0;
  GPP_TRY(gpp_launch_gemm(h->stream, 2, g, 1, NBLK, NBLK));
  return 0;
}

int gpp_trmv_lower_cols(gpp_handle_t h, const double* T, int64_t ldt, int64_t N, const double* x, double* y, int64_t nb, int rank,
                        int nranks, int trans, int compact) {
  if (!h) return -1;
  if (N < 0) return -4;
  if (int q = check_mat(T, ldt, compact ? std::min<int64_t>(N, ldt) : N, 2)) return q;
  if (!x || !aligned16(x)) return -5;
  if (!y) return -6;
  if (nb < 64 || nb % 64 != 0) return -7;
  if (nranks < 1 || rank < 0 || rank >= nranks) return -8;
  if (trans != 0 && trans != 1) return -10;
  if (trans && (!h->ws || h->ws_bytes < gpp_trmv_t_ws_bytes(N))) return -1;
  if (compact && nranks >= 1 && rank >= 0 && ldt < owned_cols(N, nb, rank, nranks)) return -3;
  GPP_TRY(gpp_launch_trmv_lower_cols(h->stream, T, ldt, N, x, y, nb, rank, nranks, trans, h->ws, h->ws_bytes, compact));
  return 0;
}

int gpp_mll_scalars(gpp_handle_t h, const double* U, int64_t ld, int64_t N, const double* z, double* out3) {
  if (!h) return -1;
  if (N < 0) return -4;
  if (int q = check_mat(U, ld, N, 2)) return q;
  if (!z) return -5;
  if (!out3) return -6;
  GPP_TRY(gpp_launch_mll_scalars(h->stream, U, ld, N, z, out3));
  return 0;
}

int gpp_mll_reduce(gpp_handle_t h, const double* U, int64_t ld, const double* Linv, int64_t ldi, int64_t N,
                   const double* r, double* z, double* out3) {
  if (!h) return -1;
  if (N < 0) return -6;
  if (int q = check_mat(U, ld, N, 2)) return q;
  if (int q = check_mat(Linv, ldi, N, 4)) return q;
  if (!r || !aligned16(r)) return -7;
  if (!z) return -8;
  if (!out3) return -9;
  GPP_TRY(gpp_launch_trmv_lower(h->stream, Linv, ldi, N, r, z));
  GPP_TRY(gpp_launch_mll_scalars(h->stream, U, ld, N, z, out3));
  return 0;
}

int gpp_alpha(gpp_handle_t h, const double* Linv, int64_t ldi, int64_t N, const double* z, double* alpha) {
  if (!h) return -1;
  if (N < 0) return -4;
  if (int q = check_mat(Linv, ldi, N, 2)) return q;
  if (!z || !aligned16(z)) return -5;
  if (!alpha) return -6;
  GPP_TRY(gpp_launch_trmv_upper(h->stream, Linv, ldi, N, z, alpha));
  return 0;
}

int gpp_grad_reduce(gpp_handle_t h, const double* U, int64_t N, int D, const double* w, const double* sf2,
                    const int32_t* grp, int S, int kind, int d_split, const double* alpha, const double* Kinv,
                    int64_t ldk, int dU, double* g_w, double* g_sf2, double* g_tau, double* g_U) {
// ... 441 lines not shown
```

### gp-plus_amd/csrc/gpp_gemm.hip

```cpp
#include "../../include/gpp.h"
#include "gpp_internal.h"

#include <algorithm>
#include <atomic>
#include <cstdlib>

typedef double v2d __attribute__((ext_vector_type(2)));
typedef double v4d __attribute__((ext_vector_type(4)));

namespace {

constexpr int BK16 = 16;
constexpr int ldt_mc(int T, int BK = 16) { return BK == 16 ? T + 16 : T + 4; }
constexpr int LDK = BK16 + 2;

__device__ __forceinline__ bool keep_elem(int mask, int k, int row) {
  return (mask == 0) | ((mask == 1) & (k <= row)) | ((mask == 2) & (k >= row));
}

template <int T>
__device__ __forceinline__ unsigned load_kc(const double* __restrict__ P, int64_t ld, int R, int r0, int kb, int kend,
                                            int mask, int tid, v2d (&reg)[T / 32]) {
  unsigned keep = 0;
  const double* ptr[T / 32];
// ... 230 lines not shown
  constexpr bool SPLIT = (VAR == 2 && RB == 16 && CB == 4 && BK == 16);
  if constexpr (SPLIT) {
    if (row0 + TM <= Mld && col0 + TN <= Nld && nch > 1) {
      int k_lo = klo, k_hi = khi;
      if (p.a_mask == 1) k_hi = min(k_hi, row0 + 1);
      if (p.a_mask == 2) k_lo = max(k_lo, row0 + TM - 1);
      if (p.b_mask == 1) k_hi = min(k_hi, col0 + 1);
      if (p.b_mask == 2) k_lo = max(k_lo, col0 + TN - 1);
      int j_lo = (k_lo - klo + BK - 1) / BK, j_hi = (k_hi - klo) / BK;
      j_lo = max(j_lo, 0);
      j_hi = min(j_hi, nch);
      if (j_hi > j_lo) {
        const int ci_lo = p.k_reverse ? nch - j_hi : j_lo, ci_hi = p.k_reverse ? nch - j_lo : j_hi;
        ca = max(ci_lo - 1, 0);
        cb = min(ci_hi - 1, nch - 1);
        if (cb < ca) ca = cb = 0;
      }
    }
  }
  auto general_iter = [&](int c) {
    const int cur = (NBUF == 2) ? (c & 1) : 0;
    const bool more = (c + 1 < nch);
    if (more) stage_load(kpos(c + 1));
    compute(cur);
    if (NBUF == 1) __syncthreads();
    if (more) {
      const int nxt = (NBUF == 2) ? (cur ^ 1) : 0;
      stage_store(smem + nxt * (OPA + OPB), smem + nxt * (OPA + OPB) + OPA);
    }
    __syncthreads();
  };
  int c = 0;
  for (; c < ca; ++c) general_iter(c);
  if constexpr (SPLIT) {
    for (; c < cb; ++c) {
      const int cur = (NBUF == 2) ? (c & 1) : 0, nxt = (NBUF == 2) ? (cur ^ 1) : 0;
      const int kb = kpos(c + 1);
      load_fast<NVA>(ubaseA + (int64_t)kb * stepA, offa, ra);
      load_fast<NVB>(ubaseB + (int64_t)kb * stepB, offb, rb);
      if constexpr (TAG != 0) __builtin_amdgcn_s_setprio(1);
      compute(cur);
      if constexpr (TAG != 0) __builtin_amdgcn_s_setprio(0);
      if (NBUF == 1) __syncthreads();
      store_mc<TM, BK, false, NTH>(smem + nxt * (OPA + OPB), tid, ra, 0);
      store_mc<TN, BK, false, NTH>(smem + nxt * (OPA + OPB) + OPA, tid, rb, 0);
      __syncthreads();
    }
  }
  for (; c < nch; ++c) general_iter(c);
  before_epilogue();
  if constexpr (!__is_same(E, GemmStoreC)) {
    static_assert((VAR == 2 || VAR == 0) && WTM == 64 && WTN == 64 && WR == 2, "accumulator epilogues are written for the big tile");
    epi(acc4, row0, col0, p.M, smem);
    return;
  }

  const double alpha = p.alpha, beta = p.beta;
  constexpr int GA = RB < 4 ? RB : 4;
#pragma unroll
  for (int a0 = 0; a0 < RB; a0 += GA) {
    double cold[GA][CB];
    if (beta != 0.0) {
#pragma unroll
      for (int a = 0; a < GA; ++a) {
        const int m = row0 + wm + 4 * (a0 + a) + lk;
#pragma unroll
        for (int b = 0; b < CB; ++b) {
          const int n = col0 + wn + 16 * b + li;
          const bool ok = (m < p.M) && (n < p.N) && (p.c_lower == 0 || (p.c_lower == 1 ? n <= m : n >= m));
          const double* src = ok ? C + (int64_t)m * p.ldc + n : Cd;
          cold[a][b] = *src;
        }
      }
    }
#pragma unroll
    for (int a = 0; a < GA; ++a) {
      const int m = row0 + wm + 4 * (a0 + a) + lk;
#pragma unroll
      for (int b = 0; b < CB; ++b) {
        const int n = col0 + wn + 16 * b + li;
        const bool ok = (m < p.M) && (n < p.N) && (p.c_lower == 0 || (p.c_lower == 1 ? n <= m : n >= m));
        double v = alpha * acc4[(a0 + a) >> 2][b][(a0 + a) & 3];
        if (beta != 0.0) v = fma(beta, cold[a][b], v);
        if (ok) {
          C[(int64_t)m * p.ldc + n] = v;
          if (C2)
            C2[(int64_t)n * p.ldc2 + m] = v;
        }
      }
    }
  }
}

template <int VAR, int WTM, int WTN, int TAG = 0, int BK = 16, int NBUF = 2, int WR = 2>
__global__ __launch_bounds__(128 * WR, ((VAR == 2 && !(BK > 16 && WTM >= 64)) || WTM < 64) ? 2 : 1) void gpp_gemm_f64(GemmArgs p) {
  constexpr int TM = WR * WTM, TN = 2 * WTN;
  extern __shared__ __attribute__((aligned(16))) double smem[];
  int tm, tn;
  if (p.swz) {
    const int b = blockIdx.x, xcd = b & 7, i = b >> 3;
    const int S = (i >> 6) * 8 + xcd, w = i & 63;
    const int super_n = (p.tiles_n + 7) >> 3;
    const int sm = S / super_n, sn = S - sm * super_n;
    tm = sm * 8 + (w >> 3);
    tn = sn * 8 + (w & 7);
    if (tm >= p.tiles_m || tn >= p.tiles_n) return;
    if ((p.c_lower == 1 && tn > tm) || (p.c_lower == 2 && tn < tm)) return;
  } else {
    const int t = (p.batch_fast ? (int)(blockIdx.x / (unsigned)p.nbatch) : (int)blockIdx.x) + (int)p.tile_base;
    if (p.c_lower == 1 && p.row_mod >= 1) {
      const float a = 0.5f * (float)p.row_mod, b = (float)p.row_off + 1.f - a;
      int i = (int)((-b + sqrtf(b * b + 4.f * a * (float)t)) / (2.f * a));
      auto S = [&](int q) { return q * (p.row_off + 1) + p.row_mod * (q * (q - 1) / 2); };
      while (S(i + 1) <= t) ++i;
      while (S(i) > t) --i;
      tm = p.row_off + p.row_mod * i;
      tn = t - S(i);
    } else if (p.c_lower == 1 && TM == 2 * TN) {
      tm = (int)((sqrtf(4.f * (float)t + 1.f) - 1.f) * 0.5f);
      while ((tm + 1) * (tm + 2) <= t) ++tm;
      while (tm * (tm + 1) > t) --tm;
      tn = t - tm * (tm + 1);
      if (tn >= p.tiles_n) return;
    } else if (p.c_lower) {
      tm = (int)((sqrtf(8.f * (float)t + 1.f) - 1.f) * 0.5f);
      while ((tm + 1) * (tm + 2) / 2 <= t) ++tm;
      while (tm * (tm + 1) / 2 > t) --tm;
      tn = t - tm * (tm + 1) / 2;
      if (p.c_lower == 1 && p.own_mod > 1 && (tn / p.own_bt + p.own_off) % p.own_mod != 0) return;
      if (p.c_lower == 2) {
        const int q = tm;
        tm = tn;
        tn = q;
        if (p.own_mod > 1 && (tm / p.own_bt + p.own_off) % p.own_mod != 0) return;
        if ((tn + 1) * TN <= p.skip_lead) return;
        if (p.row_limit > 0 && tm * TM >= p.row_limit) return;
      }
    } else if (p.col_major) {
      tn = t / p.tiles_m;
      tm = t - tn * p.tiles_m;
    } else {
      tm = t / p.tiles_n;
      tn = t - tm * p.tiles_n;
      if (p.row_reverse) tm = p.tiles_m - 1 - tm;
    }
  }
  const int64_t bi = p.batch_fast ? (int64_t)(blockIdx.x % (unsigned)p.nbatch) : (int64_t)blockIdx.y;
  gemm_tile<VAR, WTM, WTN, TAG, BK, NBUF, WR>(p, tm, tn, p.A + bi * p.sA + (int64_t)blockIdx.z * p.zA, p.B + bi * p.sB + (int64_t)blockIdx.z * p.zB,
                                             p.C + bi * p.sC + (int64_t)blockIdx.z * p.zC,
                                             p.C2 ? p.C2 + bi * p.sC2 + (int64_t)blockIdx.z * p.zC2 : nullptr, smem);

}

__device__ __forceinline__ double wave_sum(double v) {
#pragma unroll
  for (int o = 32; o > 0; o >>= 1) v += __shfl_xor(v, o);
  return v;
}
template <int DT>
struct GradEpilogue {
  GradEpiArgs e;
  int tile;
  static constexpr int T = 128;
  static constexpr int FIXED = 2 * DT * T + 2 * T + DT + 4 * (DT + 1);
  static constexpr int SLAB = (FIXED + 1) & ~1;
  static_assert((SLAB + 16 * 256) * sizeof(double) <= 2 * 2 * BK16 * ldt_mc(T) * sizeof(double), "the epilogue lives in the main loop's LDS");
  __device__ __forceinline__ void operator()(const v4d (&acc4)[4][4], int row0, int col0, int N, double* __restrict__ smem) const {
    const int tid = threadIdx.x, wave = tid >> 6, lane = tid & 63;
    const int wm = (wave >> 1) * 64, wn = (wave & 1) * 64, li = lane & 15, lk = lane >> 4;
    const int D = e.D;
    double* __restrict__ sa = smem;
    double* __restrict__ sb = sa + DT * T;
    double* __restrict__ sal_a = sb + DT * T;
    double* __restrict__ sal_b = sal_a + T;
    double* __restrict__ sw = sal_b + T;
    double* __restrict__ red = sw + DT;
    double* __restrict__ slab = smem + SLAB;
    for (int x = tid; x < DT * T; x += 256) {
      const int d = x / T, r = x - d * T;
      sa[x] = (d < D && row0 + r < N) ? e.U[(int64_t)(row0 + r) * D + d] : 0.0;
      sb[x] = (d < D && col0 + r < N) ? e.U[(int64_t)(col0 + r) * D + d] : 0.0;
    }
    if (tid < T) {
      sal_a[tid] = (row0 + tid < N) ? e.alpha[row0 + tid] : 0.0;
      sal_b[tid] = (col0 + tid < N) ? e.alpha[col0 + tid] : 0.0;
    }
    if (tid < DT) sw[tid] = (tid < D) ? e.w[tid] : 0.0;
    __syncthreads();

    const double sf2 = *e.sf2;
    const GppExpConsts ec = gpp_exp_consts();
    const bool diag_tile = (row0 == col0);
    double my_sf2 = 0.0, my_w[DT];
#pragma unroll
    for (int d = 0; d < DT; ++d) my_w[d] = 0.0;
#pragma unroll
    for (int a4 = 0; a4 < 4; ++a4) {
#pragma unroll
      for (int v = 0; v < 4; ++v)
#pragma unroll
        for (int b = 0; b < 4; ++b) slab[(v * 4 + b) * 256 + tid] = acc4[a4][b][v];
#pragma unroll 1
      for (int h = 0; h < 2; ++h) {
        const int ra = wm + 16 * a4 + 8 * h + lk;
        const int cb = wn + li;
        double r2[2][4];
#pragma unroll
        for (int a = 0; a < 2; ++a)
#pragma unroll
          for (int b = 0; b < 4; ++b) r2[a][b] = 0.0;
#pragma unroll 2
        for (int d = 0; d < DT; ++d) {
          const double ua[2] = {sa[d * T + ra], sa[d * T + ra + 4]};
          const double wd = sw[d];
#pragma unroll
          for (int b = 0; b < 4; ++b) {
            const double ub = sb[d * T + cb + 16 * b];
#pragma unroll
            for (int a = 0; a < 2; ++a) {
              const double df = ua[a] - ub;
              r2[a][b] = fma(wd * df, df, r2[a][b]);
            }
          }
        }
        __asm__ volatile("" ::: "memory");
        double g2[2][4];
#pragma unroll
        for (int a = 0; a < 2; ++a) {
          const int i = row0 + ra + 4 * a;
          const double al_i = sal_a[ra + 4 * a];
#pragma unroll
          for (int b = 0; b < 4; ++b) {
            const int j = col0 + cb + 16 * b;
            const bool ok = (i < N) & (j <= i);
            const double kv = gpp_exp_nonpos(-r2[a][b], ec);
            const double kin = slab[((2 * h + a) * 4 + b) * 256 + tid];
            double Wij = 0.5 * (al_i * sal_b[cb + 16 * b] - kin);
            Wij = ok ? Wij : 0.0;
            const double mult = (i == j) ? 1.0 : 2.0;
            my_sf2 = fma(mult * Wij, kv, my_sf2);
            g2[a][b] = mult * Wij * sf2 * kv;
            if (diag_tile && ok && i == j) e.wdiag[i] = Wij;
          }
        }
#pragma unroll
        for (int d = 0; d < DT; ++d) {
          const double ua[2] = {sa[d * T + ra], sa[d * T + ra + 4]};
          double s = 0.0;
#pragma unroll
          for (int b = 0; b < 4; ++b) {
            const double ub = sb[d * T + cb + 16 * b];
#pragma unroll
            for (int a = 0; a < 2; ++a) {
              const double df = ua[a] - ub;
              s = fma(-g2[a][b] * df, df, s);
            }
          }
          my_w[d] += s;
          __builtin_amdgcn_sched_barrier(0);
        }
      }
    }
#pragma unroll
    for (int q = 0; q <= DT; ++q) {
      const double v = wave_sum(q < DT ? my_w[q < DT ? q : 0] : my_sf2);
      if (lane == 0) red[wave * (DT + 1) + q] = v;
    }
    __syncthreads();
    if (tid <= D) {
      const int q = (tid == D) ? DT : tid;
      e.rec[(int64_t)tile * (D + 1) + tid] = ((red[q] + red[(DT + 1) + q]) + red[2 * (DT + 1) + q]) + red[3 * (DT + 1) + q];
    }
  }
};

template <int DT>
__global__ __launch_bounds__(256, 2) void gpp_lauum_grad_f64(GemmArgs p, GradEpiArgs e) {
  extern __shared__ __attribute__((aligned(16))) double smem[];
  const int t = (int)blockIdx.x;
  int tm = (int)((sqrtf(8.f * (float)t + 1.f) - 1.f) * 0.5f);
  while ((tm + 1) * (tm + 2) / 2 <= t) ++tm;
  while (tm * (tm + 1) / 2 > t) --tm;
  const int tn = t - tm * (tm + 1) / 2;
  gemm_tile<2, 64, 64, 2, 16, 2, 2>(p, tm, tn, p.A, p.B, nullptr, nullptr, smem, GemmNoHook(), GradEpilogue<DT>{e, t});
}

template <bool MAT>
struct PostCrossEpilogue {
  PostCrossArgs e;
  int tile, Mr;
  static constexpr int T = 128, DC = 16;
  static constexpr int SLAB = 2 * DC * T + T + 2 * T;
  static_assert((SLAB & 1) == 0 && (SLAB + 16 * 256) * sizeof(double) <= 2 * 2 * BK16 * ldt_mc(T) * sizeof(double) &&
                    (SLAB + 16 * 256) * sizeof(double) <= 2 * 2 * T * LDK * sizeof(double),
                "the epilogue lives in the main loop's LDS");
  __device__ __forceinline__ void operator()(const v4d (&acc4)[4][4], int row0, int col0, int Mc, double* __restrict__ smem) const {
    const int tid = threadIdx.x, wave = tid >> 6, lane = tid & 63;
    const int wm = (wave >> 1) * 64, wn = (wave & 1) * 64, li = lane & 15, lk = lane >> 4;
    const int D = e.dk & 255, kind = (e.dk >> 8) & 255;
    const int dsp = (!MAT || kind == 0) ? D : (e.dk >> 16);
    double* __restrict__ sa = smem;
    double* __restrict__ sb = sa + DC * T;
    double* __restrict__ som = sb + DC * T;
    double* __restrict__ rs = som + T;
    double* __restrict__ slab = smem + SLAB;
    const double* __restrict__ Uc = e.Uc;
    const double* __restrict__ Ur = e.Ur;
    const double* __restrict__ wp = e.w;
    double* __restrict__ rec = e.rec + (int64_t)tile * T;
    Uc += (int64_t)row0 * (e.dk & 255);
    Ur += (int64_t)col0 * (e.dk & 255);
    int rlim = Mc - row0, clim = Mr - col0;
    asm volatile("" : "+v"(Uc), "+v"(Ur), "+v"(wp), "+v"(rec), "+v"(rlim), "+v"(clim));
    auto stage = [&](int d0) {
      for (int x = tid; x < DC * T; x += 256) {
        const int dd = x / T, r = x - dd * T, d = d0 + dd;
        const bool okd = d < D;
        const double sw = okd ? sqrt(wp[okd ? d : 0]) : 0.0;
        sa[x] = (okd && r < rlim) ? Uc[r * D + d] * sw : 0.0;
        sb[x] = (okd && r < clim) ? Ur[r * D + d] * sw : 0.0;
      }
    };
    if (tid < T) som[tid] = (tid < clim) ? (e.omega ? e.omega[col0 + tid] : 1.0) : 0.0;
    const bool one = (D <= DC);
    if (one) stage(0);
    __syncthreads();

    const double sf2 = *e.sf2;
    const GppExpConsts ec = gpp_exp_consts();
#pragma unroll
    for (int a4 = 0; a4 < 4; ++a4) {
#pragma unroll
      for (int v = 0; v < 4; ++v)
#pragma unroll
        for (int b = 0; b < 4; ++b) slab[(v * 4 + b) * 256 + tid] = acc4[a4][b][v];
#pragma unroll 1
      for (int h = 0; h < 2; ++h) {
        const int ra = wm + 16 * a4 + 8 * h + lk;
        const int cb = wn + li;
        double r2[2][4], r2m[MAT ? 2 : 1][MAT ? 4 : 1];
#pragma unroll
        for (int a = 0; a < 2; ++a)
#pragma unroll
          for (int b = 0; b < 4; ++b) {
            r2[a][b] = 0.0;
            if (MAT) r2m[MAT ? a : 0][MAT ? b : 0] = 0.0;
          }
#pragma unroll 1
        for (int d0 = 0; d0 < D; d0 += DC) {
          if (!one) {
            __syncthreads();
            stage(d0);
            __syncthreads();
          }
          const int nd = min(DC, D - d0);
#pragma unroll 2
          for (int dd = 0; dd < nd; ++dd) {
            const double ua[2] = {sa[dd * T + ra], sa[dd * T + ra + 4]};
            const bool second = MAT && (d0 + dd >= dsp);
#pragma unroll
            for (int b = 0; b < 4; ++b) {
              const double ub = sb[dd * T + cb + 16 * b];
#pragma unroll
              for (int a = 0; a < 2; ++a) {
                const double df = ua[a] - ub;
                if (MAT && second) r2m[MAT ? a : 0][MAT ? b : 0] = fma(df, df, r2m[MAT ? a : 0][MAT ? b : 0]);
                else r2[a][b] = fma(df, df, r2[a][b]);
              }
            }
          }
        }
#pragma unroll
        for (int a = 0; a < 2; ++a) {
          double s = 0.0;
#pragma unroll
          for (int b = 0; b < 4; ++b) {
            double kv = gpp_exp_nonpos(-r2[a][b], ec);
            if constexpr (MAT) {
              if (kind == 1) {
                const double r = sqrt(3.0 * 2.0 * r2m[MAT ? a : 0][MAT ? b : 0]);
                kv *= (1.0 + r) * gpp_exp_nonpos(-r, ec);
              } else if (kind == 2) {
                const double r = sqrt(5.0 * 2.0 * r2m[MAT ? a : 0][MAT ? b : 0]);
                kv *= (1.0 + r + r * r * (1.0 / 3.0)) * gpp_exp_nonpos(-r, ec);
              }
            }
            const double c = sf2 * kv - slab[((2 * h + a) * 4 + b) * 256 + tid];
            double t = c * c;
            t = (cb + 16 * b < clim) ? t : 0.0;
            s = fma(som[cb + 16 * b], t, s);
          }
#pragma unroll
          for (int o = 8; o > 0; o >>= 1) s += __shfl_xor(s, o);
          if (li == 0) rs[(wave & 1) * T + ra + 4 * a] = s;
        }
      }
    }
    __syncthreads();
    if (tid < T) rec[tid] = rs[tid] + rs[T + tid];
  }
};

template <int VAR, bool MAT>
__global__ __launch_bounds__(256, VAR == 2 ? 2 : 1) void gpp_post_cross_f64(GemmArgs p, PostCrossArgs e) {
  extern __shared__ __attribute__((aligned(16))) double smem[];
  const int t = (int)blockIdx.x;
  const int tm = t / p.tiles_n, tn = t - tm * p.tiles_n;
  gemm_tile<VAR, 64, 64, 2, 16, 2, 2>(p, tm, tn, p.A, p.B, nullptr, nullptr, smem, GemmNoHook(), PostCrossEpilogue<MAT>{e, t, p.N});
}

template <bool MAT>
struct PostCrossMinEpilogue {
  PostCrossMinArgs e;
  int tile, Mr;
  static constexpr int T = 128, DC = 16, QMAX = 64;
  static constexpr int SLAB = 2 * DC * T + 2 * T + QMAX;
  static_assert((SLAB & 1) == 0 && (SLAB + 16 * 256) * sizeof(double) <= 2 * 2 * BK16 * ldt_mc(T) * sizeof(double) &&
                    (SLAB + 16 * 256) * sizeof(double) <= 2 * 2 * T * LDK * sizeof(double),
                "the epilogue lives in the main loop's LDS");
  __device__ __forceinline__ void operator()(const v4d (&acc4)[4][4], int row0, int col0, int Mc, double* __restrict__ smem) const {
    const int tid = threadIdx.x, wave = tid >> 6, lane = tid & 63;
    const int wm = (wave >> 1) * 64, wn = (wave & 1) * 64, li = lane & 15, lk = lane >> 4;
    const int D = e.dk & 255, kind = (e.dk >> 8) & 255;
    const int dsp = (!MAT || kind == 0) ? D : ((e.dk >> 16) & 255);
    const int Q = e.dk >> 24;
    double* __restrict__ sa = smem;
    double* __restrict__ sb = sa + DC * T;
    double* __restrict__ sm = sb + DC * T;
    double* __restrict__ ss = sm + T;
    double* __restrict__ sz = ss + T;
    double* __restrict__ slab = smem + SLAB;
    const double* __restrict__ Uc = e.Uc;
    const double* __restrict__ Ur = e.Ur;
    const double* __restrict__ wp = e.w;
    double* __restrict__ rec = e.rec + ((int64_t)tile * 2 + (wave & 1)) * T * Q;
    Uc += (int64_t)row0 * (e.dk & 255);
    Ur += (int64_t)col0 * (e.dk & 255);
// ... 8 lines not shown
        sb[x] = (okd && r < clim) ? Ur[r * D + d] * sw : 0.0;
      }
    };
    if (tid < T) sm[tid] = (tid < clim) ? e.m[col0 + tid] : __builtin_huge_val();
    else ss[tid - T] = (tid - T < rlim) ? e.scale[row0 + tid - T] : 0.0;
    if (tid < Q) sz[tid] = e.nodes[tid];
    const bool one = (D <= DC);
    if (one) stage(0);
    __syncthreads();

    const double sf2 = *e.sf2;
    const GppExpConsts ec = gpp_exp_consts();
#pragma unroll
    for (int a4 = 0; a4 < 4; ++a4) {
#pragma unroll
      for (int v = 0; v < 4; ++v)
#pragma unroll
        for (int b = 0; b < 4; ++b) slab[(v * 4 + b) * 256 + tid] = acc4[a4][b][v];
#pragma unroll 1
      for (int h = 0; h < 2; ++h) {
        const int ra = wm + 16 * a4 + 8 * h + lk;
        const int cb = wn + li;
        double r2[2][4], r2m[MAT ? 2 : 1][MAT ? 4 : 1];
#pragma unroll
        for (int a = 0; a < 2; ++a)
#pragma unroll
          for (int b = 0; b < 4; ++b) {
            r2[a][b] = 0.0;
            if (MAT) r2m[MAT ? a : 0][MAT ? b : 0] = 0.0;
          }
#pragma unroll 1
        for (int d0 = 0; d0 < D; d0 += DC) {
          if (!one) {
            __syncthreads();
            stage(d0);
            __syncthreads();
          }
          const int nd = min(DC, D - d0);
#pragma unroll 2
          for (int dd = 0; dd < nd; ++dd) {
            const double ua[2] = {sa[dd * T + ra], sa[dd * T + ra + 4]};
            const bool second = MAT && (d0 + dd >= dsp);
#pragma unroll
            for (int b = 0; b < 4; ++b) {
              const double ub = sb[dd * T + cb + 16 * b];
#pragma unroll
              for (int a = 0; a < 2; ++a) {
                const double df = ua[a] - ub;
                if (MAT && second) r2m[MAT ? a : 0][MAT ? b : 0] = fma(df, df, r2m[MAT ? a : 0][MAT ? b : 0]);
                else r2[a][b] = fma(df, df, r2[a][b]);
              }
            }
          }
        }
        double cv[2][4], mb[4];
#pragma unroll
        for (int b = 0; b < 4; ++b) mb[b] = sm[cb + 16 * b];
#pragma unroll
        for (int a = 0; a < 2; ++a)
#pragma unroll
          for (int b = 0; b < 4; ++b) {
            double kv = gpp_exp_nonpos(-r2[a][b], ec);
            if constexpr (MAT) {
              if (kind == 1) {
                const double r = sqrt(3.0 * 2.0 * r2m[MAT ? a : 0][MAT ? b : 0]);
                kv *= (1.0 + r) * gpp_exp_nonpos(-r, ec);
              } else if (kind == 2) {
                const double r = sqrt(5.0 * 2.0 * r2m[MAT ? a : 0][MAT ? b : 0]);
                kv *= (1.0 + r + r * r * (1.0 / 3.0)) * gpp_exp_nonpos(-r, ec);
              }
            }
            const double c = sf2 * kv - slab[((2 * h + a) * 4 + b) * 256 + tid];
            cv[a][b] = (cb + 16 * b < clim) ? c : 0.0;
          }
        const double sc[2] = {ss[ra], ss[ra + 4]};
        double keep[2] = {0.0, 0.0};
#pragma unroll 1
        for (int k = 0; k < Q; ++k) {
          const double z = sz[k];
#pragma unroll
          for (int a = 0; a < 2; ++a) {
            const double t = z * sc[a];
            double s = fma(cv[a][0], t, mb[0]);
#pragma unroll
            for (int b = 1; b < 4; ++b) s = fmin(s, fma(cv[a][b], t, mb[b]));
#pragma unroll
            for (int o = 8; o > 0; o >>= 1) s = fmin(s, __shfl_xor(s, o));
            keep[a] = (li == (k & 15)) ? s : keep[a];
          }
          if ((k & 15) == 15 || k + 1 == Q) {
            const int kn = (k & ~15) + li;
            if (kn <= k) {
              rec[(int64_t)ra * Q + kn] = keep[0];
              rec[(int64_t)(ra + 4) * Q + kn] = keep[1];
            }
          }
        }
      }
    }
    __syncthreads();
  }
};

template <int VAR, bool MAT>
__global__ __launch_bounds__(256, VAR == 2 ? 2 : 1) void gpp_post_cross_min_f64(GemmArgs p, PostCrossMinArgs e) {
  extern __shared__ __attribute__((aligned(16))) double smem[];
  const int t = (int)blockIdx.x;
  const int tm = t / p.tiles_n, tn = t - tm * p.tiles_n;
  gemm_tile<VAR, 64, 64, 2, 16, 2, 2>(p, tm, tn, p.A, p.B, nullptr, nullptr, smem, GemmNoHook(), PostCrossMinEpilogue<MAT>{e, t, p.N});
}

constexpr size_t gemm_lds_bytes(int var, int tm, int tn, int bk, int nbuf) {
  const int tx = tm > tn ? tm : tn;
  const int mc = bk * ldt_mc(tx, bk), kc = tx * LDK;
  return (size_t)nbuf * 2 * ((var != 2 && kc > mc) ? kc : mc) * sizeof(double);
}
template <int VAR, int WTM, int WTN, int TAG, int BK, int NBUF>
hipError_t launch_inst(hipStream_t s, dim3 grid, const GemmArgs& a) {
  constexpr size_t bytes = gemm_lds_bytes(VAR, 2 * WTM, 2 * WTN, BK, NBUF);
  auto* fn = gpp_gemm_f64<VAR, WTM, WTN, TAG, BK, NBUF>;
  if (bytes > 48 * 1024) {
    static std::atomic<bool> attr_set[64];
    int dev = 0;
    hipError_t e = hipGetDevice(&dev);
    if (e != hipSuccess) return e;
    if (dev < 0 || dev >= 64 || !attr_set[dev]) {
      e = hipFuncSetAttribute(reinterpret_cast<const void*>(fn), hipFuncAttributeMaxDynamicSharedMemorySize, (int)bytes);
      if (e != hipSuccess) return e;
      if (dev >= 0 && dev < 64) attr_set[dev] = true;
    }
  }
  hipLaunchKernelGGL(fn, grid, dim3(256), bytes, s, a);
  return hipGetLastError();
}
#ifndef GPP_SMALL_BK
#define GPP_SMALL_BK 64
#endif
template <int VAR>
hipError_t launch_var(hipStream_t s, int tm, int tn, dim3 grid, const GemmArgs& a) {
  constexpr int SBK = (VAR == 2) ? GPP_SMALL_BK : 16;
  constexpr int SNB = (VAR == 2 && GPP_SMALL_BK > 16) ? 1 : 2;
  if (tm == 128 && tn == 128 && a.tag == 1 && VAR == 2) return launch_inst<2, 64, 64, 1, 16, 2>(s, grid, a);
  if (tm == 128 && tn == 128) return launch_inst<VAR, 64, 64, 0, 16, 2>(s, grid, a);
  if (tm == 64 && tn == 64) return launch_inst<VAR, 32, 32, 0, SBK, SNB>(s, grid, a);
  if (tm == 32 && tn == 32) return launch_inst<VAR, 16, 16, 0, SBK, SNB>(s, grid, a);
  if (tm == 128 && tn == 32) return launch_inst<VAR, 64, 16, 0, SBK, SNB>(s, grid, a);
  return hipErrorInvalidValue;
}


#define GPP_AS4 __attribute__((address_space(4)))
typedef const GemmArgs GPP_AS4 CGemmArgs;

__device__ __forceinline__ int exec_load(const int* p) { return __hip_atomic_load(p, __ATOMIC_RELAXED, __HIP_MEMORY_SCOPE_AGENT); }

__device__ __forceinline__ bool exec_poll(int* counters, int w0, int v0, int w1, int v1, long long budget, int32_t* info,
                                          int status = GPP_INFO_EXEC_TIMEOUT) {
  long long t0 = 0;
  bool timed = false;
  for (;;) {
    const bool r0 = w0 < 0 || exec_load(counters + w0) >= v0;
    const bool r1 = w1 < 0 || exec_load(counters + w1) >= v1;
    if (r0 & r1) return true;
    if (!timed) {
      t0 = (long long)wall_clock64();
      timed = true;
    }
    const long long waited = (long long)wall_clock64() - t0;
    if (exec_load(counters) != 0) return false;
    if (waited > budget) {
      const long long ms = waited / 100000;
      __hip_atomic_store(counters, 1, __ATOMIC_RELAXED, __HIP_MEMORY_SCOPE_AGENT);
      atomicCAS(info, 0, status | (int)(ms > 0xFFFFF ? 0xFFFFF : ms));
      return false;
    }
    __builtin_amdgcn_s_sleep(2);
  }
}

typedef const DagTask GPP_AS4 CDagTask;
__global__ __launch_bounds__(64) void gpp_dag_bind(const GemmArgs* rel, GemmArgs* abs, int n, DagBases bases) {
  const int g = blockIdx.x * 64 + threadIdx.x;
  if (g >= n) return;
  GemmArgs a = rel[g];
  auto base = [&](int b) {
    return b == 0 ? bases.p[0] : b == 1 ? bases.p[1] : b == 2 ? bases.p[2] : b == 3 ? bases.p[3] : b == 4 ? bases.p[4] : b == 5 ? bases.p[5]
                                                                                                     : b == 6 ? bases.p[6] : bases.p[7];
  };
  a.A = reinterpret_cast<const double*>(base(a.buf[0]) + reinterpret_cast<uintptr_t>(a.A));
  a.B = reinterpret_cast<const double*>(base(a.buf[1]) + reinterpret_cast<uintptr_t>(a.B));
  a.C = reinterpret_cast<double*>(base(a.buf[2]) + reinterpret_cast<uintptr_t>(a.C));
  a.C2 = a.buf[3] >= 0 ? reinterpret_cast<double*>(base(a.buf[3]) + reinterpret_cast<uintptr_t>(a.C2)) : nullptr;
  abs[g] = a;
}
__global__ __launch_bounds__(256, 2) void gpp_dag_f64(DagLaunch e) {
  extern __shared__ __attribute__((aligned(16))) double smem[];
  __shared__ int s_idx, s_ok;
  const int tid = threadIdx.x;
#pragma clang diagnostic push
#pragma clang diagnostic ignored "-Wold-style-cast"
  CDagTask* tasks = (CDagTask*)e.tasks;
  CGemmArgs* groups = (CGemmArgs*)e.groups;
#pragma clang diagnostic pop
  int pre = -2;
  auto take = [&](int done_after) -> int {
    if (e.max_tasks > 0 && done_after >= e.max_tasks) return -1;
    if (e.quit_id >= 0 && (exec_load(e.counters) != 0 || exec_load(e.counters + e.quit_id) >= e.quit_val)) return -1;
    if (e.ticket_limit <= 0) return __hip_atomic_fetch_add(e.counters + 1, 1, __ATOMIC_RELAXED, __HIP_MEMORY_SCOPE_AGENT);
    int old = exec_load(e.counters + 1);
    while (old < e.ticket_limit &&
           !__hip_atomic_compare_exchange_strong(e.counters + 1, &old, old + 1, __ATOMIC_RELAXED, __ATOMIC_RELAXED, __HIP_MEMORY_SCOPE_AGENT)) {
    }
    return old < e.ticket_limit ? old : -1;
  };
  for (int done = 0;; ++done) {
    if (tid == 0) {
      s_idx = pre != -2 ? pre : take(done);
      pre = -2;
    }
    __syncthreads();
    const int idx = __builtin_amdgcn_readfirstlane(s_idx);
    __syncthreads();
    if (idx < 0 || idx >= e.ntasks) break;
    if (e.trace && tid == 0) {
      e.trace[4 * (size_t)idx] = wall_clock64();
      e.trace[4 * (size_t)idx + 3] = (unsigned long long)blockIdx.x | ((unsigned long long)(unsigned)e.tag << 32);
    }
    const int w0 = tasks[idx].wait_id[0], w1 = tasks[idx].wait_id[1], w2 = tasks[idx].wait_id[2];
    if (w0 >= 0 || w1 >= 0 || w2 >= 0) {
      if (tid == 0) {
        const int v0 = tasks[idx].wait_val[0], v1 = tasks[idx].wait_val[1], v2 = tasks[idx].wait_val[2];
        const int c0 = w0 >= 0 ? exec_load(e.counters + w0) : v0, c1 = w1 >= 0 ? exec_load(e.counters + w1) : v1,
                  c2 = w2 >= 0 ? exec_load(e.counters + w2) : v2;
        bool ok = (c0 >= v0) & (c1 >= v1) & (c2 >= v2);
        if (!ok) {
          ok = exec_poll(e.counters, w0, v0, w1, v1, e.budget, e.info, GPP_INFO_EXEC_TIMEOUT);
          if (ok && w2 >= 0) ok = exec_poll(e.counters, w2, v2, -1, 0, e.budget, e.info, GPP_INFO_EXEC_TIMEOUT);
        }
        s_ok = ok ? 1 : 0;
      }
      __syncthreads();
      const int ok = s_ok;
      __builtin_amdgcn_fence(__ATOMIC_ACQUIRE, "agent");
      __syncthreads();
      if (!ok) break;
    }
    if (e.trace && tid == 0) e.trace[4 * (size_t)idx + 1] = wall_clock64();
    const CGemmArgs& p = groups[tasks[idx].group];
    const int tm = tasks[idx].tm, tn = tasks[idx].tn;
    if (p.op == 0) {
      auto ahead = [&]() {
        if (tid == 0) pre = take(done + 1);
      };
      if (p.etile == 64) gemm_tile<2, 32, 32, 0, 64, 1, 2>(p, tm, tn, p.A, p.B, p.C, p.C2, smem);
      else gemm_tile<2, 64, 64, 0, 16, 2, 2>(p, tm, tn, p.A, p.B, p.C, p.C2, smem, ahead);
    } else {
      const int c = tn * 128 + ((tid & 63) << 1), r4 = tid >> 6;
      if (c < p.N) {
        const bool pair = c + 1 < p.N;
        for (int r0 = 0; r0 < p.M; r0 += 32) {
          v2d v[8];
#pragma unroll
          for (int q = 0; q < 8; ++q) {
            const int r = r0 + 4 * q + r4;
            const double* src = p.B + (int64_t)(r < p.M ? r : 0) * p.ldb + c;
            if (pair) v[q] = *reinterpret_cast<const v2d*>(src);
            else v[q] = (v2d){*src, 0.0};
          }
#pragma unroll
          for (int q = 0; q < 8; ++q) {
            const int r = r0 + 4 * q + r4;
            if (r < p.M) {
              double* dst = p.C + (int64_t)r * p.ldc + c;
              if (pair) *reinterpret_cast<v2d*>(dst) = v[q];
              else *dst = v[q].x;
            }
          }
        }
      }
    }
    const int i0 = tasks[idx].inc_id[0], i1 = tasks[idx].inc_id[1];
    if (i0 >= 0 || i1 >= 0) {
      asm volatile("s_waitcnt vmcnt(0)" ::: "memory");
      __syncthreads();
      if (tid == 0) {
        __builtin_amdgcn_fence(__ATOMIC_RELEASE, "agent");
        asm volatile("s_waitcnt vmcnt(0)" ::: "memory");
        if (i0 >= 0) __hip_atomic_fetch_add(e.counters + i0, (int)tasks[idx].inc_val[0], __ATOMIC_RELAXED, __HIP_MEMORY_SCOPE_AGENT);
        if (i1 >= 0) __hip_atomic_fetch_add(e.counters + i1, (int)tasks[idx].inc_val[1], __ATOMIC_RELAXED, __HIP_MEMORY_SCOPE_AGENT);
      }
    }
    if (e.trace) {
      asm volatile("s_waitcnt vmcnt(0)" ::: "memory");
      if (tid == 0) e.trace[4 * (size_t)idx + 2] = wall_clock64();
    }
  }
}

__global__ __launch_bounds__(64) void gpp_exec_gate(int* counters, int id, int target, int32_t* info, long long budget) {
  if (threadIdx.x == 0) (void)exec_poll(counters, id, target, -1, 0, budget, info);
}
__global__ __launch_bounds__(64) void gpp_exec_signal(int* counters, int id) {
  if (threadIdx.x == 0) {
    __builtin_amdgcn_fence(__ATOMIC_RELEASE, "agent");
    asm volatile("s_waitcnt vmcnt(0)" ::: "memory");
    __hip_atomic_fetch_add(counters + id, 1, __ATOMIC_RELAXED, __HIP_MEMORY_SCOPE_AGENT);
  }
}

}

hipError_t gpp_launch_gemm(hipStream_t s, int variant, const GemmArgs& a_in, int batch, int tile_m, int tile_n) {
  GemmArgs a = a_in;
  if (a.M <= 0 || a.N <= 0 || batch <= 0) return hipSuccess;
  auto ntiles = [&](int T) -> int64_t {
    const int64_t tm = (a.M + T - 1) / T, tn = (a.N + T - 1) / T;
    return (a.c_lower ? tm * (tm + 1) / 2 : tm * tn) * batch * (a.batch2 > 1 ? a.batch2 : 1);
  };
  if (tile_m == 0) {
    constexpr int64_t t128 = 256, t64 = 192;
    const int64_t cus = a.cu_hint > 0 ? a.cu_hint : 256;
    if (ntiles(128) * 256 >= t128 * cus) tile_m = 128;
    else if (ntiles(64) * 256 >= t64 * cus) tile_m = 64;
    else tile_m = 32;
    tile_n = tile_m;
  }
  if (a.c_lower && tile_m != tile_n) return hipErrorInvalidValue;
  a.tiles_m = (a.M + tile_m - 1) / tile_m;
  a.tiles_n = (a.N + tile_n - 1) / tile_n;
  int64_t nt = a.c_lower ? (int64_t)a.tiles_m * (a.tiles_m + 1) / 2 : (int64_t)a.tiles_m * a.tiles_n;
  a.tile_base = 0;
  if (a.c_lower == 1 && (a.row_mod > 1 || a.row_i1 > 0)) {
    if (a.row_mod < 1) { a.row_mod = 1; a.row_off = 0; }
    if (a.row_off < 0 || a.row_off >= a.row_mod) return hipErrorInvalidValue;
    const int64_t rows = a.tiles_m > a.row_off ? (a.tiles_m - a.row_off + a.row_mod - 1) / a.row_mod : 0;
    auto S = [&](int64_t i) { return i * (a.row_off + 1) + (int64_t)a.row_mod * (i * (i - 1) / 2); };
    const int64_t i0 = std::min<int64_t>(std::max(a.row_i0, 0), rows), i1 = a.row_i1 > 0 ? std::min<int64_t>(a.row_i1, rows) : rows;
    if (i1 <= i0) return hipSuccess;
    a.tile_base = S(i0);
    nt = S(i1) - S(i0);
  } else {
    a.row_mod = 0;
    if (a.c_lower == 1 && a.row_t1 > 0) {
      const int64_t t0 = std::min<int64_t>(std::max(a.row_t0, 0), a.tiles_m), t1 = std::min<int64_t>(a.row_t1, a.tiles_m);
      if (t1 <= t0) return hipSuccess;
      a.tile_base = t0 * (t0 + 1) / 2;
      nt = t1 * (t1 + 1) / 2 - a.tile_base;
    }
  }
  a.swz = 0;
  if (false && nt >= 1024) {
    const int64_t n_super = (int64_t)((a.tiles_m + 7) / 8) * ((a.tiles_n + 7) / 8);
    nt = ((n_super + 7) / 8) * 8 * 64;
    a.swz = 1;
  }
  const int batch2 = a.batch2 > 1 ? a.batch2 : 1;
  dim3 grid((unsigned)nt, (unsigned)batch, (unsigned)batch2);
  if (a.batch_fast && batch > 1 && !a.swz && nt * batch < (int64_t)1 << 31) {
    a.nbatch = batch;
    grid = dim3((unsigned)(nt * batch), 1u, (unsigned)batch2);
  } else {
    a.batch_fast = 0;
  }
  switch (variant) {
    case 0: return launch_var<0>(s, tile_m, tile_n, grid, a);
    case 1: return launch_var<1>(s, tile_m, tile_n, grid, a);
    case 2: return launch_var<2>(s, tile_m, tile_n, grid, a);
    default: return hipErrorInvalidValue;
  }
}

hipError_t gpp_launch_lauum_grad(hipStream_t s, const GemmArgs& a_in, const GradEpiArgs& e) {
  GemmArgs a = a_in;
  if (a.M <= 0) return hipSuccess;
  if (a.M != a.N || a.c_lower != 1 || e.D < 1 || e.D > 16) return hipErrorInvalidValue;
  a.tiles_m = a.tiles_n = (a.M + 127) / 128;
  a.row_mod = 0;
  a.swz = 0;
  a.batch_fast = 0;
  a.tile_base = 0;
  const int64_t nt = (int64_t)a.tiles_m * (a.tiles_m + 1) / 2;
  constexpr size_t bytes = gemm_lds_bytes(2, 128, 128, 16, 2);
  auto* fn = e.D <= 8 ? gpp_lauum_grad_f64<8> : gpp_lauum_grad_f64<16>;
  static std::atomic<bool> attr_set[2][64];
  int dev = 0;
  hipError_t err = hipGetDevice(&dev);
  if (err != hipSuccess) return err;
  const int which = e.D <= 8 ? 0 : 1;
  if (dev < 0 || dev >= 64 || !attr_set[which][dev]) {
    err = hipFuncSetAttribute(reinterpret_cast<const void*>(fn), hipFuncAttributeMaxDynamicSharedMemorySize, (int)bytes);
    if (err != hipSuccess) return err;
    if (dev >= 0 && dev < 64) attr_set[which][dev] = true;
  }
  hipLaunchKernelGGL(fn, dim3((unsigned)nt), dim3(256), bytes, s, a, e);
  return hipGetLastError();
}

hipError_t gpp_launch_post_cross(hipStream_t s, int variant, const GemmArgs& a_in, const PostCrossArgs& e) {
  GemmArgs a = a_in;
  if (a.M <= 0 || a.N <= 0 || a.K <= 0 || (variant != 0 && variant != 2)) return hipErrorInvalidValue;
  a.tiles_m = (a.M + 127) / 128;
  a.tiles_n = (a.N + 127) / 128;
  const int64_t nt = (int64_t)a.tiles_m * a.tiles_n;
  if (nt >= (int64_t)1 << 31) return hipErrorInvalidValue;
  const bool mat = ((e.dk >> 8) & 255) != 0;
  const size_t bytes = gemm_lds_bytes(variant, 128, 128, 16, 2);
  auto* fn = variant == 2 ? (mat ? gpp_post_cross_f64<2, true> : gpp_post_cross_f64<2, false>)
                          : (mat ? gpp_post_cross_f64<0, true> : gpp_post_cross_f64<0, false>);
  static std::atomic<bool> attr_set[4][64];
  int dev = 0;
  hipError_t err = hipGetDevice(&dev);
  if (err != hipSuccess) return err;
  const int which = (variant == 2 ? 2 : 0) + (mat ? 1 : 0);
  if (dev < 0 || dev >= 64 || !attr_set[which][dev]) {
    err = hipFuncSetAttribute(reinterpret_cast<const void*>(fn), hipFuncAttributeMaxDynamicSharedMemorySize, (int)bytes);
    if (err != hipSuccess) return err;
    if (dev >= 0 && dev < 64) attr_set[which][dev] = true;
  }
  hipLaunchKernelGGL(fn, dim3((unsigned)nt), dim3(256), bytes, s, a, e);
  return hipGetLastError();
}

hipError_t gpp_launch_post_cross_min(hipStream_t s, int variant, const GemmArgs& a_in, const PostCrossMinArgs& e) {
  GemmArgs a = a_in;
  const int Q = e.dk >> 24;
  if (a.M <= 0 || a.N <= 0 || a.K <= 0 || (variant != 0 && variant != 2) || Q < 1 || Q > 64) return hipErrorInvalidValue;
  a.tiles_m = (a.M + 127) / 128;
  a.tiles_n = (a.N + 127) / 128;
  const int64_t nt = (int64_t)a.tiles_m * a.tiles_n;
  if (nt >= (int64_t)1 << 31) return hipErrorInvalidValue;
  const bool mat = ((e.dk >> 8) & 255) != 0;
  const size_t bytes = gemm_lds_bytes(variant, 128, 128, 16, 2);
  auto* fn = variant == 2 ? (mat ? gpp_post_cross_min_f64<2, true> : gpp_post_cross_min_f64<2, false>)
                          : (mat ? gpp_post_cross_min_f64<0, true> : gpp_post_cross_min_f64<0, false>);
  static std::atomic<bool> attr_set[4][64];
  int dev = 0;
  hipError_t err = hipGetDevice(&dev);
  if (err != hipSuccess) return err;
  const int which = (variant == 2 ? 2 : 0) + (mat ? 1 : 0);
  if (dev < 0 || dev >= 64 || !attr_set[which][dev]) {
    err = hipFuncSetAttribute(reinterpret_cast<const void*>(fn), hipFuncAttributeMaxDynamicSharedMemorySize, (int)bytes);
    if (err != hipSuccess) return err;
    if (dev >= 0 && dev < 64) attr_set[which][dev] = true;
  }
  hipLaunchKernelGGL(fn, dim3((unsigned)nt), dim3(256), bytes, s, a, e);
  return hipGetLastError();
}

hipError_t gpp_launch_dag_bind(hipStream_t s, const GemmArgs* rel, GemmArgs* abs, int n, const DagBases& bases) {
  if (n <= 0) return hipSuccess;
  hipLaunchKernelGGL(gpp_dag_bind, dim3((unsigned)((n + 63) / 64)), dim3(64), 0, s, rel, abs, n, bases);
  return hipGetLastError();
}
hipError_t gpp_launch_dag(hipStream_t s, int nworkers, const DagLaunch& e) {
  if (nworkers <= 0) return hipSuccess;
  constexpr size_t b128 = gemm_lds_bytes(2, 128, 128, 16, 2), b64 = gemm_lds_bytes(2, 64, 64, 64, 1);
  constexpr size_t bytes = b128 > b64 ? b128 : b64;
  static std::atomic<bool> attr_set[64];
  int dev = 0;
  hipError_t err = hipGetDevice(&dev);
  if (err != hipSuccess) return err;
  if (dev < 0 || dev >= 64 || !attr_set[dev]) {
    err = hipFuncSetAttribute(reinterpret_cast<const void*>(gpp_dag_f64), hipFuncAttributeMaxDynamicSharedMemorySize, (int)bytes);
    if (err != hipSuccess) return err;
    if (dev >= 0 && dev < 64) attr_set[dev] = true;
  }
  hipLaunchKernelGGL(gpp_dag_f64, dim3((unsigned)nworkers), dim3(256), bytes, s, e);
  return hipGetLastError();
}
hipError_t gpp_launch_exec_gate(hipStream_t s, int* counters, int id, int target, int32_t* info, long long budget) {
  hipLaunchKernelGGL(gpp_exec_gate, dim3(1), dim3(64), 0, s, counters, id, target, info, budget);
  return hipGetLastError();
}
hipError_t gpp_launch_exec_signal(hipStream_t s, int* counters, int id) {
  hipLaunchKernelGGL(gpp_exec_signal, dim3(1), dim3(64), 0, s, counters, id);
  return hipGetLastError();
}
```

### gp-plus_amd/csrc/gpp_internal.h

```cpp
#pragma once
#include <hip/hip_runtime.h>
#include <stdint.h>
#include <stddef.h>
#include <vector>
#include "../../include/gpp.h"

#define GPP_TILE 128
#define GPP_DAG_PLANS 20

struct gpp_handle_s {
  int device;
  hipStream_t stream;
  void* ws;
  size_t ws_bytes;
  hipStream_t panel_stream;
  hipStream_t upd_stream;
  hipStream_t full_stream;
  hipStream_t fill_stream;
  int panel_cus;
  int cu_split;
  hipEvent_t events[16];
  int n_events, ev_next;
  int64_t inv_N;
  int inv_nblocks;
  int64_t inv_o[128], inv_n[128];
  char* panel_flags;
  int panel_next;
  int cap_next;
  hipEvent_t handoff;
  int ncu;
  int coop_panel;
  int panel_fault;
  int panel_timeout_ms;
  struct DagPlan* dag_plans[GPP_DAG_PLANS];
  uint64_t dag_clock;
  struct DagPlan* shard_cur;
  int32_t* shard_info;
  hipEvent_t shard_ready;
  int dag_sched;
  int gemm_tile;
  int split_builds;
  gpp_comm_t comm;
  int comm_rank, comm_nranks;
  void* rccl_comm;
  hipStream_t comm_stream;
  hipEvent_t comm_event;
};
struct GppInvBlocks {
  int64_t N;
  int nblocks;
  decltype(gpp_handle_s::inv_o) o;
  decltype(gpp_handle_s::inv_n) n;
};
inline GppInvBlocks gpp_inv_blocks_save(const gpp_handle_s* h) {
  GppInvBlocks k;
  k.N = h->inv_N;
  k.nblocks = h->inv_nblocks;
  static_assert(sizeof(k.o) == sizeof(h->inv_o) && sizeof(k.n) == sizeof(h->inv_n), "one record");
  for (size_t i = 0; i < sizeof(k.o) / sizeof(k.o[0]); ++i) { k.o[i] = h->inv_o[i]; k.n[i] = h->inv_n[i]; }
  return k;
}
inline void gpp_inv_blocks_restore(gpp_handle_s* h, const GppInvBlocks& k) {
  h->inv_N = k.N;
  h->inv_nblocks = k.nblocks;
  for (size_t i = 0; i < sizeof(k.o) / sizeof(k.o[0]); ++i) { h->inv_o[i] = k.o[i]; h->inv_n[i] = k.n[i]; }
}
extern "C" void gpp_shard_release_comm(gpp_handle_s* h);

struct GppEnv {
  bool coop_panel;
  bool dag_sched;
  bool dag_phased;
  bool shard_list;
  int shard_workers;
  int shard_fill;
  long long shard_timeout_ms;
  int64_t shard_piece_cols;
  bool sharded_force_collectives;
  bool exec_verbose;
  int dag_dump;
  bool dag_check_verbose;
};
const GppEnv& gpp_env();
constexpr int GPP_PANEL_RING = 8;
constexpr int GPP_PANEL_CAP_RING = 16;

#ifdef __HIPCC__
struct GppExpConsts {
  double log2e, ln2_hi, ln2_lo, c[11];
};
__device__ __forceinline__ GppExpConsts gpp_exp_consts() {
  GppExpConsts k = {1.44269504088896338700e+00, 6.93147180369123816490e-01, 1.90821492927058770002e-10,
                    {2.08767569878680989792e-09,
                     2.50521083854417187751e-08,
                     2.75573192239858906526e-07,
                     2.75573192239858906526e-06,
                     2.48015873015873015873e-05,
                     1.98412698412698412698e-04,
                     1.38888888888888888889e-03,
                     8.33333333333333333333e-03,
                     4.16666666666666666667e-02,
                     1.66666666666666666667e-01,
                     0.5}};
  asm volatile("" : "+s"(k.log2e), "+s"(k.ln2_hi), "+s"(k.ln2_lo));
#pragma unroll
  for (int i = 0; i < 10; ++i) asm volatile("" : "+s"(k.c[i]));
  return k;
}
__device__ __forceinline__ double gpp_exp_nonpos(double x, const GppExpConsts& k) {
  x = (x < -800.0) ? -800.0 : x;
  const double n = __builtin_rint(x * k.log2e);
  double r = __builtin_fma(-n, k.ln2_hi, x);
  r = __builtin_fma(-n, k.ln2_lo, r);
  double p = k.c[0];
#pragma unroll
  for (int i = 1; i < 11; ++i) p = __builtin_fma(p, r, k.c[i]);
  p = __builtin_fma(p, r, 1.0);
  p = __builtin_fma(p, r, 1.0);
  return __builtin_ldexp(p, (int)n);
}
#endif

struct GemmArgs {
  const double* A;
  const double* B;
  double* C;
  int64_t lda, ldb, ldc;
  int M, N, K;
  double alpha, beta;
  int a_mask, b_mask;
  int klo_mode, khi_mode;
  int c_lower;
  int64_t sA, sB, sC;
  int64_t zA, zB, zC, zC2;
  int batch2;
  int tiles_m, tiles_n;
  double* C2;
  int64_t ldc2, sC2;
  int k_reverse;
  int tag;
  int col_major;
  int row_reverse;
  int swz;
  int own_mod, own_off, own_bt;
  int skip_lead;
  int row_limit;
  int batch_fast, nbatch;
  int row_i0, row_i1;
  int64_t tile_base;
  int row_t0, row_t1;
  int cu_hint;
  int row_mod, row_off;
  int op;
  int compact_bc;
  int etile;
  int buf[4];
  int pad_ok;
};
hipError_t gpp_launch_gemm(hipStream_t s, int variant, const GemmArgs& a, int batch, int tile_m = 0, int tile_n = 0);

struct GradEpiArgs {
  const double* U;
  const double* w;
  const double* sf2;
  const double* alpha;
  double* rec;
  double* wdiag;
  int D;
};
hipError_t gpp_launch_lauum_grad(hipStream_t s, const GemmArgs& lauum, const GradEpiArgs& e);

struct PostCrossArgs {
  const double* Uc;
  const double* Ur;
  const double* w;
  const double* sf2;
  const double* omega;
  double* rec;
  int dk;
};
hipError_t gpp_launch_post_cross(hipStream_t s, int variant, const GemmArgs& p, const PostCrossArgs& e);
size_t gpp_post_cross_ws_bytes(int64_t Mc, int64_t Mr);

struct PostCrossMinArgs {
  const double* Uc;
  const double* Ur;
  const double* w;
  const double* sf2;
  const double* m;
  const double* scale;
  const double* nodes;
  double* rec;
  int dk;
};
hipError_t gpp_launch_post_cross_min(hipStream_t s, int variant, const GemmArgs& p, const PostCrossMinArgs& e);
size_t gpp_post_cross_min_ws_bytes(int64_t Mc, int64_t Mr, int Q);

hipError_t gpp_launch_exec_gate(hipStream_t s, int* counters, int id, int target, int32_t* info, long long budget);
hipError_t gpp_launch_exec_signal(hipStream_t s, int* counters, int id);

struct DagTask {
  int32_t group;
  int16_t tm, tn;
  int32_t wait_id[3];
  int32_t wait_val[3];
  int32_t inc_id[2];
  int32_t kind;
  int16_t inc_val[2];
};
static_assert(sizeof(DagTask) == 48, "the device reads 48-byte task records");
struct DagLaunch {
  const GemmArgs* groups;
  const DagTask* tasks;
  int ntasks;
  int* counters;
  int32_t* info;
  long long budget;
  int max_tasks;
  int quit_id, quit_val;
  int ticket_limit;
  unsigned long long* trace;
  int tag;
};
hipError_t gpp_launch_dag(hipStream_t s, int nworkers, const DagLaunch& e);
struct DagBases { char* p[8]; };
hipError_t gpp_launch_dag_bind(hipStream_t s, const GemmArgs* rel, GemmArgs* abs, int n, const DagBases& bases);

enum { DK_S = 0, DK_U = 1, DK_CP = 2, DK_XB = 3, DK_XA = 4, DK_SH = 5, DK_UD = 6, DK_NKINDS = 7 };
struct DagTuning {
  double t0_big, tc_big;
  double t0_64, tc_64;
  double t0_32, tc_32;
  double t_copy;
  double t_panel0, t_panel_leaf;
  double t_gate;
  int chain_tile;
  int workers;
  int fill;
  int fuse;
  int64_t inv_rows;
  int64_t piece_cols;
};
struct DagPlan {
  int64_t N = 0, nb = 0, ld = 0, ldi = 0, ldt = 0, ldk = 0, inv_rows = 0;
  int rank = 0, nranks = 1, workers = 0, fill = 0;
  int c_cph = 0, c_cpt = 0, c_art = 0;
  int piece_tiles = 0, GP = 1;
  std::vector<int> cph_target, cpt_target;
  int flags = 0;
  int B = 0, nt = 0;
  std::vector<int> tb;
  std::vector<GemmArgs> groups;
  std::vector<DagTask> tasks;
  struct Op { int kind, arg, n, lim; };
  std::vector<Op> stream_ops;
  std::vector<int> gate_target;
  std::vector<int> level_first;
  int ncounters = 0;
  int c_pd = 0, c_g1d = 0;
  double sim_ms = 0, sim_busy = 0;
  GemmArgs* d_groups = nullptr;
  GemmArgs* d_groups_abs = nullptr;
  DagTask* d_tasks = nullptr;
  int* d_counters = nullptr;
  unsigned long long* d_trace = nullptr;
  hipEvent_t last_use = nullptr;
  uint64_t stamp = 0;
};
enum { DAG_INV = 1, DAG_SHARD = 4, DAG_BACK = 8 };
DagPlan* gpp_dag_plan(int64_t N, int64_t nb, int64_t ld, int64_t ldi, int64_t ldt, int64_t ldk, int flags, const DagTuning& tune,
                      int rank = 0, int nranks = 1);
DagTuning gpp_dag_default_tuning();
hipError_t gpp_dag_upload(DagPlan* P);
void gpp_dag_free(DagPlan* P);

hipError_t gpp_launch_fill_i32(hipStream_t s, int32_t* p, int n, int32_t value);
size_t gpp_panel_flag_bytes();
int gpp_panel_max_leaves();
hipError_t gpp_launch_panel(hipStream_t s, double* A, int64_t lda, double* Linv, int64_t ldi, int n, int32_t* info, int row_offset,
                            int* flags, int max_wgs, int timeout_ms);
hipError_t gpp_launch_leaf(hipStream_t s, double* A, int64_t lda, double* Linv, int64_t ldi, int n, int32_t* info,
                           int row_offset, int batch = 1, int64_t sA = 0, int64_t sLi = 0);

hipError_t gpp_launch_kernel_build(hipStream_t s, const double* U, int64_t N, int D, const double* w, const double* sf2,
                                   const double* tau, const int32_t* grp, int S, double jitter, int kind, int d_split,
                                   int uplo, double* Ky, int64_t ld, int64_t row0, int64_t nrows, int batch = 1,
                                   int64_t sU = 0, int64_t sK = 0);
hipError_t gpp_launch_cross_kernel(hipStream_t s, const double* Ua, int64_t Ma, const double* Ub, int64_t Nb, int D,
                                   const double* w, const double* sf2, int kind, int d_split, double* Kab, int64_t ld);
hipError_t gpp_launch_post_cov_train(hipStream_t s, const double* Kinv, int64_t ldk, int64_t N, const double* tau, const int32_t* grp,
                                     const double* d, double jitter, double* A, int64_t lda);
hipError_t gpp_launch_sym_rowscale(hipStream_t s, const double* Kinv, int64_t ldk, int64_t N, const double* sv, double* S, int64_t lds);
hipError_t gpp_launch_sym_rowscale_batched(hipStream_t s, const double* Kinv, int64_t ldk, int64_t N, const double* sv, double* S,
                                           int64_t lds, int batch, int64_t sK, int64_t sv_stride, int64_t sS);

int gpp_apply_pieces(int64_t L);
size_t gpp_apply_ws_bytes(int64_t L, int64_t M, int S);
hipError_t gpp_launch_kernel_apply(hipStream_t s, const double* Ua, int64_t M, const double* Ub, int64_t N, int D, const double* w,
                                   const double* sf2, int kind, int d_split, const double* C, int64_t ldc, int S, double beta,
                                   double* Out, int64_t ldo, void* ws, size_t ws_bytes);
hipError_t gpp_launch_rff_apply(hipStream_t s, const double* Ua, int64_t M, int D, const double* Omega, const double* phase, int64_t F,
                                const double* sf2, const double* Theta, int64_t ldt, int S, double beta, double* Out, int64_t ldo,
                                void* ws, size_t ws_bytes);
hipError_t gpp_launch_kernel_apply_grad(hipStream_t s, const double* Ua, int64_t M, const double* Ub, int64_t N, int D, const double* w,
                                        const double* sf2, int kind, int d_split, const double* C, int64_t ldc, int S,
                                        const double* Gbar, int64_t ldg, double beta, double* g_Ua, int64_t ldu, void* ws,
                                        size_t ws_bytes);
hipError_t gpp_launch_rff_apply_grad(hipStream_t s, const double* Ua, int64_t M, int D, const double* Omega, const double* phase,
                                     int64_t F, const double* sf2, const double* Theta, int64_t ldt, int S, const double* Gbar,
                                     int64_t ldg, double beta, double* g_Ua, int64_t ldu, void* ws, size_t ws_bytes);

size_t gpp_append_ws_bytes(int64_t N, int64_t q);

hipError_t gpp_launch_trmv_lower(hipStream_t s, const double* T, int64_t ldt, int64_t N, const double* x, double* y,
                                 int batch = 1, int64_t sT = 0, int64_t sv = 0);
hipError_t gpp_launch_trmv_upper(hipStream_t s, const double* T, int64_t ldt, int64_t N, const double* x, double* y,
                                 int batch = 1, int64_t sT = 0, int64_t sv = 0);
hipError_t gpp_launch_mll_scalars(hipStream_t s, const double* L, int64_t ld, int64_t N, const double* z, double* out3,
                                  int batch = 1, int64_t sL = 0, int64_t sv = 0);
size_t gpp_grad_ws_bytes(int64_t N, int D, int S, int dU);
hipError_t gpp_launch_grad_reduce(hipStream_t s, const double* U, int64_t N, int D, const double* w, const double* sf2,
                                  const int32_t* grp, int S, int kind, int d_split, const double* alpha,
                                  const double* Kinv, int64_t ldk, int dU, double* g_w, double* g_sf2, double* g_tau,
// ... 24 lines not shown
```

### gp-plus_amd/csrc/gpp_reduce.hip

```cpp
#include "gpp_internal.h"

#include <algorithm>

typedef double v2d __attribute__((ext_vector_type(2)));

namespace {

__device__ __forceinline__ double wave_sum(double v) {
#pragma unroll
  for (int o = 32; o > 0; o >>= 1) v += __shfl_xor(v, o);
  return v;
}

__global__ __launch_bounds__(256) void gpp_trmv_lower(const double* __restrict__ T, int64_t ldt, int64_t N,
                                                      const double* __restrict__ x, double* __restrict__ y, int64_t sT,
                                                      int64_t sv) {
  const int wave = threadIdx.x >> 6, lane = threadIdx.x & 63;
  const int64_t i = (int64_t)blockIdx.x * 4 + wave;
  if (i >= N) return;
  T += (int64_t)blockIdx.y * sT;
  x += (int64_t)blockIdx.y * sv;
  y += (int64_t)blockIdx.y * sv;
  const double* row = T + i * ldt;
  double acc = 0.0;
  const int64_t len = i + 1;
  const int64_t len2 = len & ~(int64_t)1;
  for (int64_t k = 2 * lane; k < len2; k += 128) {
    const v2d t = *reinterpret_cast<const v2d*>(row + k);
    const v2d xx = *reinterpret_cast<const v2d*>(x + k);
    acc = fma(t.x, xx.x, acc);
    acc = fma(t.y, xx.y, acc);
  }
  if (lane == 0 && (len & 1)) acc = fma(row[len - 1], x[len - 1], acc);
  acc = wave_sum(acc);
  if (lane == 0) y[i] = acc;
}

__global__ __launch_bounds__(256) void gpp_trmv_upper(const double* __restrict__ T, int64_t ldt, int64_t N,
                                                      const double* __restrict__ x, double* __restrict__ y, int64_t sT,
                                                      int64_t sv) {
  const int wave = threadIdx.x >> 6, lane = threadIdx.x & 63;
  const int64_t j = (int64_t)blockIdx.x * 4 + wave;
  if (j >= N) return;
  T += (int64_t)blockIdx.y * sT;
  x += (int64_t)blockIdx.y * sv;
  y += (int64_t)blockIdx.y * sv;
  const double* row = T + j * ldt;
  double acc = 0.0;
  int64_t k0 = j;
  if (k0 & 1) {
    if (lane == 0) acc = fma(row[k0], x[k0], acc);
    ++k0;
  }
  const int64_t nvec = (N - k0) >> 1;
  for (int64_t v = lane; v < nvec; v += 64) {
    const v2d t = *reinterpret_cast<const v2d*>(row + k0 + 2 * v);
    const v2d xx = *reinterpret_cast<const v2d*>(x + k0 + 2 * v);
    acc = fma(t.x, xx.x, acc);
    acc = fma(t.y, xx.y, acc);
  }
  if (lane == 0 && ((N - k0) & 1)) acc = fma(row[N - 1], x[N - 1], acc);
  acc = wave_sum(acc);
  if (lane == 0) y[j] = acc;
}

__global__ __launch_bounds__(256) void gpp_trmv_lower_cols(const double* __restrict__ T, int64_t ldt, int64_t N,
                                                           const double* __restrict__ x, double* __restrict__ y, int64_t nb,
                                                           int rank, int nranks, int compact) {
  const int wave = threadIdx.x >> 6, lane = threadIdx.x & 63;
  const int64_t i = (int64_t)blockIdx.x * 4 + wave;
  if (i >= N) return;
  const double* row = T + i * ldt;
  double acc = 0.0;
  int64_t q = 0;
  for (int64_t c0 = (int64_t)rank * nb; c0 <= i; c0 += (int64_t)nranks * nb, ++q) {
    const int64_t c1 = (c0 + nb < i + 1) ? c0 + nb : i + 1;
    const int64_t len = c1 - c0, len2 = len & ~(int64_t)1;
    const double* seg = row + (compact ? q * nb : c0);
    for (int64_t k = 2 * lane; k < len2; k += 128) {
      const v2d t = *reinterpret_cast<const v2d*>(seg + k);
      const v2d xx = *reinterpret_cast<const v2d*>(x + c0 + k);
      acc = fma(t.x, xx.x, acc);
      acc = fma(t.y, xx.y, acc);
    }
    if (lane == 0 && (len & 1)) acc = fma(seg[len - 1], x[c1 - 1], acc);
  }
  acc = wave_sum(acc);
  if (lane == 0) y[i] = acc;
}

constexpr int TRT_CHUNKS = 16;
__global__ __launch_bounds__(256) void gpp_trmv_lower_t_cols(const double* __restrict__ T, int64_t ldt, int64_t N,
                                                             const double* __restrict__ x, double* __restrict__ part, int64_t nb,
                                                             int rank, int nranks, int64_t chunk, int compact) {
  __shared__ double red[4][64];
  const int wave = threadIdx.x >> 6, lane = threadIdx.x & 63;
  const int64_t k0 = (int64_t)blockIdx.x * 64, k = k0 + lane;
  const bool owned = (int)((k0 / nb) % nranks) == rank;
  double acc = 0.0;
  const int64_t r0 = (int64_t)blockIdx.y * chunk, r1 = (r0 + chunk < N) ? r0 + chunk : N;
  if (owned && k < N && r1 > k0) {
    int64_t i = (r0 > k0 ? r0 : k0) + wave;
    const double* p = T + (compact ? ((k0 / nb) / nranks) * nb + (k0 % nb) + lane : k);
    for (; i + 28 < r1; i += 32) {
      double t[8], xv[8];
#pragma unroll
      for (int u = 0; u < 8; ++u) {
        t[u] = p[(i + 4 * u) * ldt];
        xv[u] = x[i + 4 * u];
      }
#pragma unroll
      for (int u = 0; u < 8; ++u) acc = (i + 4 * u >= k) ? fma(t[u], xv[u], acc) : acc;
    }
    for (; i < r1; i += 4)
      if (i >= k) acc = fma(p[i * ldt], x[i], acc);
  }
  red[wave][lane] = acc;
  __syncthreads();
  if (wave == 0 && k < N) part[(int64_t)blockIdx.y * N + k] = (red[0][lane] + red[1][lane]) + (red[2][lane] + red[3][lane]);
}
__global__ __launch_bounds__(256) void gpp_trmv_lower_t_finish(const double* __restrict__ part, int64_t N, int chunks,
                                                               double* __restrict__ y) {
  const int64_t k = (int64_t)blockIdx.x * 256 + threadIdx.x;
  if (k >= N) return;
  double s = 0.0;
  for (int r = 0; r < chunks; ++r) s += part[(int64_t)r * N + k];
  y[k] = s;
}

__global__ __launch_bounds__(1024) void gpp_mll_scalars(const double* __restrict__ L, int64_t ld, int64_t N,
                                                        const double* __restrict__ z, double* __restrict__ out3, int64_t sL,
                                                        int64_t sv) {
  __shared__ double sq[16], sl[16];
  L += (int64_t)blockIdx.x * sL;
  z += (int64_t)blockIdx.x * sv;
  out3 += 3 * (int64_t)blockIdx.x;
  double q = 0.0, l = 0.0;
  for (int64_t i = threadIdx.x; i < N; i += 1024) {
    const double zi = z[i];
    q = fma(zi, zi, q);
    l += log(L[i * ld + i]);
  }
  q = wave_sum(q);
  l = wave_sum(l);
  const int wave = threadIdx.x >> 6, lane = threadIdx.x & 63;
  if (lane == 0) {
    sq[wave] = q;
    sl[wave] = l;
  }
  __syncthreads();
  if (threadIdx.x == 0) {
    double qq = 0.0, ll = 0.0;
    for (int w = 0; w < 16; ++w) {
      qq += sq[w];
      ll += sl[w];
    }
    ll *= 2.0;
    out3[0] = qq;
    out3[1] = ll;
    out3[2] = -0.5 * (qq + ll + (double)N * 1.8378770664093454835606594728112);
  }
}

__global__ __launch_bounds__(256) void gpp_loo_rows(const double* __restrict__ Linv, int64_t ldi, int64_t N,
                                                    const double* __restrict__ alpha, const double* __restrict__ y,
                                                    double* __restrict__ d, double* __restrict__ mu, double* __restrict__ s2,
                                                    double* __restrict__ a, double* __restrict__ sb, int64_t sLi, int64_t sv) {
  const int wave = threadIdx.x >> 6, lane = threadIdx.x & 63;
  const int64_t i = (int64_t)blockIdx.x * 4 + wave;
  if (i >= N) return;
  const int64_t vo = (int64_t)blockIdx.y * sv;
  const double* row = Linv + (int64_t)blockIdx.y * sLi + i * ldi;
  double acc = 0.0;
  int64_t k0 = i;
  if (k0 & 1) {
    if (lane == 0) acc = row[k0] * row[k0];
    ++k0;
  }
  const int64_t nvec = (N - k0) >> 1;
#pragma unroll 4
  for (int64_t v = lane; v < nvec; v += 64) {
    const v2d t = *reinterpret_cast<const v2d*>(row + k0 + 2 * v);
    acc = fma(t.x, t.x, acc);
    acc = fma(t.y, t.y, acc);
  }
  if (lane == 0 && ((N - k0) & 1)) acc = fma(row[N - 1], row[N - 1], acc);
  acc = wave_sum(acc);
  if (lane == 0) {
    const int64_t o = vo + i;
    const double di = acc, al = alpha[o], inv = 1.0 / di;
    d[o] = di;
    if (mu) mu[o] = y[o] - al * inv;
    if (s2) s2[o] = inv;
    if (a) a[o] = -al * inv;
    if (sb) sb[o] = sqrt(0.5 * inv + 0.5 * (al * inv) * (al * inv));
  }
}

__global__ __launch_bounds__(1024) void gpp_loo_value(const double* __restrict__ d, const double* __restrict__ alpha, int64_t N,
                                                      double* __restrict__ out, int64_t sv) {
  __shared__ double sp[16];
  d += (int64_t)blockIdx.x * sv;
  alpha += (int64_t)blockIdx.x * sv;
  out += blockIdx.x;
  double s = 0.0;
  for (int64_t i = threadIdx.x; i < N; i += 1024) {
    const double di = d[i], al = alpha[i];
    s += 0.5 * log(di) - 0.5 * al * al / di;
  }
  s = wave_sum(s);
  const int wave = threadIdx.x >> 6, lane = threadIdx.x & 63;
  if (lane == 0) sp[wave] = s;
  __syncthreads();
  if (threadIdx.x == 0) {
    double t = 0.0;
// ... 751 lines not shown
```

### gp-plus_amd/linalg.py

```python
from __future__ import annotations

import math
import threading
from contextlib import contextmanager, nullcontext
from dataclasses import dataclass
from typing import Dict, Optional, Tuple

import torch

from .backend import KIND_RBF, UPLO_FULL, UPLO_UPPER, GppContext, get_context, rows_buffer, square_buffer
from .psd_safe import inputs_nan_probe, psd_safe
from . import settings

__all__ = ["KernelSpec", "exact_mll", "ExactMLLFunction", "exact_loo", "ExactLOOFunction", "loo_moments", "exact_cv", "ExactCVFunction",
           "cv_moments", "EvalWorkspace", "dense_kernel", "cross_kernel",
           "FactorCache", "factorize", "append_to_cache", "dense_log_prob", "predict_mean", "predict_var", "predictive_cov_upper",
           "train_post_cov_upper", "mvn_root", "mvn_draw"]


@dataclass
class KernelSpec:
    w: torch.Tensor
    sf2: torch.Tensor
    kind: int = KIND_RBF
    d_split: int = 0


class EvalWorkspace:

    def __init__(self, ctx: GppContext, N: int):
        dev = ctx.device
        self.N = N
        self.A = square_buffer(N, dev)
        self.Li = square_buffer(N, dev)
        self.Ki = square_buffer(N, dev)
        self.z = torch.empty(N, dtype=torch.float64, device=dev)
        self.alpha = torch.empty(N, dtype=torch.float64, device=dev)
        self.r = torch.empty(N, dtype=torch.float64, device=dev)
        self.out3 = torch.empty(3, dtype=torch.float64, device=dev)
        self.info = torch.zeros(1, dtype=torch.int32, device=dev)
        self.info_host = torch.zeros(1, dtype=torch.int32).pin_memory()
        self.info_event = torch.cuda.Event()
        self.epoch = 0
        self._loo = None

    def loo_vectors(self):
        if self._loo is None:
            from types import SimpleNamespace
            v = lambda n: torch.empty(n, dtype=torch.float64, device=self.A.device)
            self._loo = SimpleNamespace(d=v(self.N), a=v(self.N), sb=v(self.N), beta=v(self.N), z=v(self.N), out3=v(3), val=v(1))
        return self._loo


_workspaces: Dict[Tuple[int, int, int], EvalWorkspace] = {}
_workspaces_lock = threading.Lock()
_tls = threading.local()


@contextmanager
def eval_slot(slot: int):
    old = getattr(_tls, "slot", 0)
    _tls.slot = slot
    try:
        yield
    finally:
        _tls.slot = old


def current_slot() -> int:
    return getattr(_tls, "slot", 0)

LOOKAHEAD_MIN_N = 3840

FUSED_GRAD_MIN_N = 5120

STAGE_EVENTS = None


class _stage:
    def __init__(self, name: str):
        self.name = name

    def __enter__(self):
        if STAGE_EVENTS is not None:
            self.e0 = torch.cuda.Event(enable_timing=True)
            self.e0.record()
        return self

    def __exit__(self, *exc):
        if STAGE_EVENTS is not None:
            e1 = torch.cuda.Event(enable_timing=True)
            e1.record()
            STAGE_EVENTS.append((self.name, self.e0, e1))
        return False


def get_workspace(ctx: GppContext, N: int, slot: int = 0) -> EvalWorkspace:
    key = (ctx.index, N, slot)
    ws = _workspaces.get(key)
    if ws is None:
        with _workspaces_lock:
            for k in [k for k in _workspaces if k[0] == ctx.index and k[2] == slot]:
                del _workspaces[k]
            ws = EvalWorkspace(ctx, N)
            _workspaces[key] = ws
    return ws


def _as_f64(t: torch.Tensor, device) -> torch.Tensor:
    return t.to(device=device, dtype=torch.float64).contiguous()


def _factor(ctx: GppContext, ws: EvalWorkspace, U, w, sf2, tau, grp, kind, d_split, after=None) -> float:
    if torch.cuda.is_current_stream_capturing():
        if ws.N >= LOOKAHEAD_MIN_N:
            raise RuntimeError("graph capture of the evaluation is limited to the single-stream factorisation (N < 3840)")
        ctx.kernel_build(U, w, sf2, tau, grp, ws.A, jitter=0.0, kind=kind, d_split=d_split, uplo=UPLO_UPPER)
        ctx.potrf(ws.A, ws.Li, ws.info, ws.Ki)
        if after is not None:
            after()
        return 0.0

    def attempt(jit):
        if ws.N >= LOOKAHEAD_MIN_N:
            torch.cuda.current_stream(ctx.index).synchronize()
        with _stage("kernel_build"):
            pass
        with _stage("potrf"):
            ctx.build_potrf(U, w, sf2, tau, grp, ws.A, ws.Li, ws.info, ws.Ki, jitter=jit, kind=kind, d_split=d_split)
        ws.info_host.copy_(ws.info, non_blocking=True)
        ws.info_event.record(torch.cuda.current_stream(ctx.index))
        if after is not None:
            after()
        ws.info_event.synchronize()
        return int(ws.info_host[0])

    return psd_safe(ctx, attempt, inputs_nan_probe(U, w, sf2, tau))


def _operands(U, w, sf2, tau, grp):
    dev = U.device
    Ud, wd, sd, td = _as_f64(U.detach(), dev), _as_f64(w.detach(), dev), _as_f64(sf2.detach().reshape(1), dev), \
        _as_f64(tau.detach().reshape(-1), dev)
    if grp is not None and grp.dtype != torch.int32:
        grp = grp.to(torch.int32)
    return Ud, wd, sd, td, grp


def _eval_operands(ctx, U, w, sf2, tau, mean, y, grp, dU):
    Ud, wd, sd, td, grp = _operands(U, w, sf2, tau, grp)
    need = ctx.needs_input_grad
    ctx.in_dtypes = (U.dtype, w.dtype, sf2.dtype, tau.dtype, mean.dtype, y.dtype)
    ctx.shapes = (sf2.shape, tau.shape)
    return Ud, wd, sd, td, grp, td.numel(), any(need[:6]), need[0] and dU > 0


def _eval_backward(ctx, grad_out, g_w, g_s, g_t, g_Ud, g_mean):
    need = ctx.needs_input_grad
    go = grad_out.to(torch.float64)
    g_U = None
    if need[0]:
        g_U = torch.zeros(g_mean.shape[0], g_w.shape[0], dtype=torch.float64, device=g_mean.device)
        if g_Ud is not None:
            g_U[:, :g_Ud.shape[1]] = g_Ud
    dt = ctx.in_dtypes
    sf2_shape, tau_shape = ctx.shapes
    return (None if g_U is None else (go * g_U).to(dt[0]),
            (go * g_w).to(dt[1]) if need[1] else None,
            (go * g_s).reshape(sf2_shape).to(dt[2]) if need[2] else None,
            (go * g_t).reshape(tau_shape).to(dt[3]) if need[3] else None,
            (go * g_mean).to(dt[4]) if need[4] else None,
            (-go * g_mean).to(dt[5]) if need[5] else None)


def _exact_forward(fn, ctx, U, w, sf2, tau, mean, y, grp, kind, d_split, dU, slot):
    gctx = get_context(U.device)
    with torch.cuda.device(U.device):
        if not fn.capturable and torch.cuda.is_current_stream_capturing():
            raise NotImplementedError(f"{getattr(fn, 'what', 'the leave-one-out objective')} is not available inside a graph capture")
        dev = U.device
        N, D = U.shape
        Ud, wd, sd, td, grp, S, need_grad, need_U = _eval_operands(ctx, U, w, sf2, tau, mean, y, grp, dU)
        ws = get_workspace(gctx, N, slot)
        ws.epoch += 1
        torch.sub(_as_f64(y.detach(), dev), _as_f64(mean.detach(), dev), out=ws.r)
        g_w = g_s = g_t = g_Ud = None
        if need_grad:
            g_w = torch.empty(D, dtype=torch.float64, device=dev)
            g_s = torch.empty(1, dtype=torch.float64, device=dev)
            g_t = torch.empty(S, dtype=torch.float64, device=dev)
            g_Ud = torch.empty(N, dU, dtype=torch.float64, device=dev) if need_U else None
        ops, grads = (Ud, wd, sd, grp, S), (dU if need_U else 0, g_w, g_s, g_t, g_Ud)

        def rest():
            with _stage("trtri"):
                gctx.trtri(ws.A, ws.Li, ws.Ki)
            with _stage("mll_reduce"):
                gctx.mll_reduce(ws.A, ws.Li, ws.r, ws.z, ws.out3)
            if need_grad or fn.value_needs_alpha:
                with _stage("alpha"):
                    gctx.alpha(ws.Li, ws.z, ws.alpha)
            fn.tail(gctx, ws, need_grad, ops, grads, kind, d_split)

        _factor(gctx, ws, Ud, wd, sd, td, grp, kind, d_split, after=rest)
        value, g_mean = fn.result(ws, need_grad)
        ctx.saved = (g_w, g_s, g_t, g_Ud, g_mean)
        return value


class ExactMLLFunction(torch.autograd.Function):

    capturable, value_needs_alpha = True, False

    @staticmethod
    def forward(ctx, U, w, sf2, tau, mean, y, grp, kind, d_split, dU, slot):
        return _exact_forward(ExactMLLFunction, ctx, U, w, sf2, tau, mean, y, grp, kind, d_split, dU, slot)

    @staticmethod
    def tail(gctx, ws, need_grad, ops, grads, kind, d_split):
        if not need_grad:
            return
        fused = False
        with _stage("lauum"):
            if ws.N > FUSED_GRAD_MIN_N:
                fused = gctx.lauum_grad(ws.Li, *ops, ws.alpha, *grads[:4], kind=kind)
            if not fused:
                gctx.lauum(ws.Li, ws.Ki)
        with _stage("grad_reduce"):
            if not fused:
                gctx.grad_reduce(*ops, ws.alpha, ws.Ki, *grads, kind=kind, d_split=d_split)

    @staticmethod
    def result(ws, need_grad):
        return ws.out3[2].clone(), (ws.alpha.clone() if need_grad else None)

    @staticmethod
    def backward(ctx, grad_out):
        return _eval_backward(ctx, grad_out, *ctx.saved) + (None,) * 5


def exact_mll(U: torch.Tensor, spec: KernelSpec, tau: torch.Tensor, mean: torch.Tensor, y: torch.Tensor,
              grp: Optional[torch.Tensor] = None, n_grad_dims: Optional[int] = None, slot: Optional[int] = None) -> torch.Tensor:
    if slot is None:
        slot = current_slot()
    if n_grad_dims is None:
        n_grad_dims = U.shape[1] if U.requires_grad else 0
    shard = settings.sharded_evaluation.value()
    if shard is not None:
        from .sharded import sharded_mll
        return sharded_mll(U, spec.w, spec.sf2, tau, mean, y, grp, spec.kind, spec.d_split, int(n_grad_dims),
                           group=shard.get("group"), nb=int(shard.get("nb", 1024)))
    return ExactMLLFunction.apply(U, spec.w, spec.sf2, tau, mean, y, grp, spec.kind, spec.d_split, int(n_grad_dims), slot)


class ExactLOOFunction(torch.autograd.Function):

    capturable, value_needs_alpha = False, True

    @staticmethod
    def forward(ctx, U, w, sf2, tau, mean, y, grp, kind, d_split, dU, slot):
        return _exact_forward(ExactLOOFunction, ctx, U, w, sf2, tau, mean, y, grp, kind, d_split, dU, slot)

    @staticmethod
    def tail(gctx, ws, need_grad, ops, grads, kind, d_split):
        N, lv = ws.N, ws.loo_vectors()
        with _stage("loo_scalars"):
            gctx.loo_scalars(ws.Li, ws.alpha, None, lv.d, a=lv.a, sqrtb=lv.sb, loo=lv.val)
        if not need_grad:
            return
        with _stage("loo_beta"):
            gctx.mll_reduce(ws.A, ws.Li, lv.a, lv.z, lv.out3)
            gctx.alpha(ws.Li, lv.z, lv.beta)
        with _stage("lauum"):
            gctx.lauum(ws.Li, ws.Ki)
        with _stage("sym_rowscale"):
            gctx.sym_rowscale(ws.Ki, lv.sb, ws.A)
        with _stage("loo_gemm"):
            gctx.gemm(1, 0, N, N, N, 1.0, ws.A, ws.A, 0.0, ws.Li, c_tri=1)
        with _stage("loo_grad_reduce"):
            gctx.loo_grad_reduce(*ops, ws.alpha, lv.beta, ws.Li, *grads, kind=kind, d_split=d_split)

    @staticmethod
    def result(ws, need_grad):
        lv = ws.loo_vectors()
        return lv.val[0].clone(), (lv.beta.neg() if need_grad else None)

    @staticmethod
    def backward(ctx, grad_out):
        return _eval_backward(ctx, grad_out, *ctx.saved) + (None,) * 5


def exact_loo(U: torch.Tensor, spec: KernelSpec, tau: torch.Tensor, mean: torch.Tensor, y: torch.Tensor,
              grp: Optional[torch.Tensor] = None, n_grad_dims: Optional[int] = None, slot: Optional[int] = None) -> torch.Tensor:
    if slot is None:
        slot = current_slot()
    if n_grad_dims is None:
        n_grad_dims = U.shape[1] if U.requires_grad else 0
    if settings.sharded_evaluation.value() is not None:
        raise NotImplementedError("the leave-one-out objective is not available under settings.sharded_evaluation")
    return ExactLOOFunction.apply(U, spec.w, spec.sf2, tau, mean, y, grp, spec.kind, spec.d_split, int(n_grad_dims), slot)


class _CVEvaluation:

    capturable, value_needs_alpha, what = False, True, "the cross-validation objective"

    def __init__(self, folds):
        self.folds, self.terms, self.infos = folds, None, None

    def tail(self, gctx, ws, need_grad, ops, grads, kind, d_split):
        from .cv import fold_gradient_factors, fold_solves
        N, lv = ws.N, ws.loo_vectors()
        with _stage("cv_folds"):
            a, _, self.terms, self.infos, kept = fold_solves(gctx, ws.Li, ws.alpha, self.folds, keep_factors=need_grad)
        if not need_grad:
            return
        lv.a.copy_(a)
        with _stage("cv_beta"):
            gctx.mll_reduce(ws.A, ws.Li, lv.a, lv.z, lv.out3)
            gctx.alpha(ws.Li, lv.z, lv.beta)
        with _stage("lauum"):
            gctx.lauum(ws.Li, ws.Ki)
        with _stage("sym_rowscale"):
            gctx.sym_rowscale(ws.Ki, torch.ones(N, dtype=torch.float64, device=ws.A.device), ws.A)
        with _stage("cv_rows"):
            for b, Li_b, z, na, out3 in kept:
                G = fold_gradient_factors(b, Li_b, z, na, out3)
                gctx.cv_rows(G, b.idx, b.off, ws.A, ws.Li[b.base:b.base + b.rows])
                del G
        del kept
        with _stage("cv_gemm"):
            gctx.gemm(1, 0, N, N, N, 1.0, ws.Li, ws.Li, 0.0, ws.A, c_tri=1)
        with _stage("loo_grad_reduce"):
            gctx.loo_grad_reduce(*ops, ws.alpha, lv.beta, ws.A, *grads, kind=kind, d_split=d_split)

    def result(self, ws, need_grad):
        from .cv import check_infos
        check_infos(self.infos, self.folds)
        value = self.terms.sum() - 0.5 * ws.N * math.log(2.0 * math.pi)
        return value, (ws.loo_vectors().beta.neg() if need_grad else None)


class ExactCVFunction(torch.autograd.Function):

    @staticmethod
    def forward(ctx, U, w, sf2, tau, mean, y, grp, kind, d_split, dU, slot, folds):
        return _exact_forward(_CVEvaluation(folds), ctx, U, w, sf2, tau, mean, y, grp, kind, d_split, dU, slot)

    @staticmethod
    def backward(ctx, grad_out):
        return _eval_backward(ctx, grad_out, *ctx.saved) + (None,) * 6


def exact_cv(U: torch.Tensor, spec: KernelSpec, tau: torch.Tensor, mean: torch.Tensor, y: torch.Tensor, folds,
             grp: Optional[torch.Tensor] = None, n_grad_dims: Optional[int] = None, slot: Optional[int] = None) -> torch.Tensor:
    from .cv import FoldIndex
    folds = FoldIndex.make(folds, U.shape[0])
    if slot is None:
        slot = current_slot()
    if n_grad_dims is None:
        n_grad_dims = U.shape[1] if U.requires_grad else 0
    if settings.sharded_evaluation.value() is not None:
        raise NotImplementedError("the cross-validation objective is not available under settings.sharded_evaluation")
    return ExactCVFunction.apply(U, spec.w, spec.sf2, tau, mean, y, grp, spec.kind, spec.d_split, int(n_grad_dims), slot, folds)

# ... 584 lines not shown
```

### include/gpp.h

```cpp
#ifndef GPP_H
#define GPP_H

#include <stddef.h>
#include <stdint.h>

#ifdef __cplusplus
extern "C" {
#endif

typedef struct gpp_handle_s* gpp_handle_t;

#define GPP_KIND_RBF      0
#define GPP_KIND_MATERN32 1
#define GPP_KIND_MATERN52 2

#define GPP_UPLO_FULL  0
#define GPP_UPLO_LOWER 1
#define GPP_UPLO_UPPER 2

#define GPP_OP_MLL_EVAL 0
#define GPP_OP_PREDICT  1
#define GPP_OP_PREDICT_GRAD 2
#define GPP_OP_APPLY 3
#define GPP_OP_APPLY_GRAD 4
#define GPP_OP_APPEND 5
#define GPP_OP_POST_CROSS 6
#define GPP_OP_POST_CROSS_MIN 7

const char* gpp_version(void);

int gpp_create(gpp_handle_t* out, int device);
int gpp_destroy(gpp_handle_t h);
int gpp_set_stream(gpp_handle_t h, void* stream);
int gpp_internal_stream(gpp_handle_t h, int which, void** out);
#define GPP_OPT_COOP_PANEL 1
#define GPP_OPT_PANEL_FAULT 2
#define GPP_OPT_PANEL_TIMEOUT_MS 3
#define GPP_OPT_EXEC_SCHED 4
#define GPP_OPT_DAG_SCHED 5
#define GPP_OPT_GEMM_TILE 6
#define GPP_INFO_PANEL_TIMEOUT (1 << 30)
#define GPP_INFO_EXEC_TIMEOUT ((1 << 30) | (1 << 29))
int gpp_set_option(gpp_handle_t h, int option, int value);
size_t gpp_workspace_bytes(gpp_handle_t h, int op, int64_t N, int64_t M, int D, int S);
int gpp_set_workspace(gpp_handle_t h, void* ws, size_t bytes);

int gpp_kernel_build(gpp_handle_t h, const double* U, int64_t N, int D, const double* w, const double* sf2,
                     const double* tau, const int32_t* grp, int S, double jitter, int kind, int d_split,
                     int uplo, double* Ky, int64_t ld, int64_t row0, int64_t nrows);

int gpp_cross_kernel(gpp_handle_t h, const double* Ua, int64_t Ma, const double* Ub, int64_t Nb, int D,
                     const double* w, const double* sf2, int kind, int d_split, double* Kab, int64_t ld);

int gpp_kernel_apply(gpp_handle_t h, const double* Ua, int64_t M, const double* Ub, int64_t N, int D, const double* w,
                     const double* sf2, int kind, int d_split, const double* C, int64_t ldc, int S, double beta, double* Out,
                     int64_t ldo);
int gpp_rff_apply(gpp_handle_t h, const double* Ua, int64_t M, int D, const double* Omega, const double* phase, int64_t F,
                  const double* sf2, const double* Theta, int64_t ldt, int S, double beta, double* Out, int64_t ldo);

int gpp_kernel_apply_grad(gpp_handle_t h, const double* Ua, int64_t M, const double* Ub, int64_t N, int D, const double* w,
                          const double* sf2, int kind, int d_split, const double* C, int64_t ldc, int S, const double* Gbar,
                          int64_t ldg, double beta, double* g_Ua, int64_t ldu);
int gpp_rff_apply_grad(gpp_handle_t h, const double* Ua, int64_t M, int D, const double* Omega, const double* phase, int64_t F,
                       const double* sf2, const double* Theta, int64_t ldt, int S, const double* Gbar, int64_t ldg, double beta,
                       double* g_Ua, int64_t ldu);

int gpp_potrf(gpp_handle_t h, double* A, int64_t N, int64_t ld, double* Linv, int64_t ldi, int32_t* info_dev);
int gpp_potrf_ws(gpp_handle_t h, double* A, int64_t N, int64_t ld, double* Linv, int64_t ldi, double* T, int64_t ldt,
                 int32_t* info_dev);

int gpp_build_potrf_ws(gpp_handle_t h, const double* U, int64_t N, int D, const double* w, const double* sf2, const double* tau,
                       const int32_t* grp, int S, double jitter, int kind, int d_split, double* A, int64_t ld, double* Linv,
                       int64_t ldi, double* T, int64_t ldt, int32_t* info_dev);

int gpp_trtri(gpp_handle_t h, const double* U, int64_t N, int64_t ld, double* Linv, int64_t ldi, double* T, int64_t ldt);

int gpp_lauum(gpp_handle_t h, const double* Linv, int64_t N, int64_t ldi, double* Kinv, int64_t ldk);

#define GPP_NOT_SUPPORTED 2001
#define GPP_NO_WORKSPACE 2002
int gpp_lauum_grad(gpp_handle_t h, const double* Linv, int64_t N, int64_t ldi, const double* U, int D, const double* w,
                   const double* sf2, const int32_t* grp, int S, int kind, int dU, const double* alpha, double* g_w,
                   double* g_sf2, double* g_tau);

int gpp_post_cov_train(gpp_handle_t h, const double* Kinv, int64_t N, int64_t ldk, const double* tau, const int32_t* grp, int S,
                       const double* d, double jitter, double* A, int64_t lda);

int gpp_syrk_rows(gpp_handle_t h, const double* Urow, int64_t ldu, double* C, int64_t ldc, int64_t Nt, int64_t K, int64_t nb,
                  int64_t first_block, int rank, int nranks);

int gpp_gemm_lower_cols(gpp_handle_t h, const double* A, int64_t lda, const double* B, int64_t ldb, double* C, int64_t ldc,
                        int64_t M, int64_t K, double alpha, double beta, int64_t nb, int64_t first_block, int rank, int nranks,
                        int64_t row0, int64_t row1, int compact);

int gpp_shard_list_begin(gpp_handle_t h, int64_t N, int64_t nb, int rank, int nranks, double* A, int64_t ld, double* Kc, double* Lc,
                         int64_t ldc, double* D, double* W0, double* W1, double* W2, int64_t ldw, int32_t* info, int workers,
                         int* used);
int64_t gpp_shard_piece_cols(void);
int gpp_shard_list_gate(gpp_handle_t h, void* stream, int tail, int k);
int gpp_shard_list_signal(gpp_handle_t h, void* stream, int tail, int k);
int gpp_shard_list_end(gpp_handle_t h);

int gpp_shard_back_list(gpp_handle_t h, int64_t N, int64_t nb, int rank, int nranks, const double* A, int64_t ld, double* Kc, double* Lc,
                        int64_t ldc, const double* D, int32_t* info, int workers, int* used);

enum { GPP_COMM_SUM_F64 = 0, GPP_COMM_MAX_I32 = 1 };
#define GPP_SHARD_UNSUPPORTED 2000
typedef struct gpp_comm {
  void* user;
  int (*bcast)(void* user, void* dev_buf, size_t bytes, int root, void* stream);
  int (*allreduce)(void* user, void* dev_buf, size_t count, int kind, void* stream);
} gpp_comm_t;
typedef struct gpp_shard_buffers {
  double* A; int64_t ld;
  double* Kc; double* Lc; int64_t ldc;
  double* D;
  double* W0; double* W1; double* W2; int64_t ldw;
  double* msg;
  double* z; double* alpha; double* r;
  double* flat;
  double* out3; int32_t* info;
} gpp_shard_buffers_t;
int gpp_set_comm(gpp_handle_t h, const gpp_comm_t* comm, int rank, int nranks);
int gpp_comm_unique_id(void* out128);
int gpp_comm_init_rccl(gpp_handle_t h, const void* unique_id128, int rank, int nranks);
size_t gpp_shard_buffer_doubles(int64_t N, int64_t nb, int rank, int nranks, int which);
int gpp_shard_eval(gpp_handle_t h, int64_t N, int64_t nb, const double* U, int D, const double* w, const double* sf2, const double* tau,
                   const int32_t* grp, int S, int kind, int d_split, double jitter, int dU, int need_grad, const gpp_shard_buffers_t* b,
                   int32_t* info_host);

typedef struct gpp_push* gpp_push_t;
#define GPP_PUSH_HANDLE_BYTES 128
int gpp_push_create(int device, int rank, int nranks, int64_t slot_bytes, gpp_push_t* out, void* handle_out);
int gpp_push_connect(gpp_push_t p, const void* handles );
int gpp_push_send(gpp_push_t p, void* after_stream, int64_t seq, int32_t* status, int code, int nparts, const void* const* src,
                  const int64_t* spitch, const int64_t* offset, const int64_t* dpitch, const int64_t* width, const int64_t* height);
int gpp_push_recv(gpp_push_t p, void* stream, int64_t seq, int32_t* status, int code, int nparts, void* const* dst, const int64_t* dpitch,
                  const int64_t* offset, const int64_t* spitch, const int64_t* width, const int64_t* height);
int gpp_push_ack(gpp_push_t p, void* stream, int64_t seq);
int gpp_push_info(gpp_push_t p, int64_t* slot_bytes, int* flag_kind );
int gpp_push_destroy(gpp_push_t p, int stage);

int gpp_trmv_lower_cols(gpp_handle_t h, const double* T, int64_t ldt, int64_t N, const double* x, double* y, int64_t nb, int rank,
                        int nranks, int trans, int compact);

int gpp_mll_scalars(gpp_handle_t h, const double* U, int64_t ld, int64_t N, const double* z, double* out3);

int gpp_lauum_rows(gpp_handle_t h, const double* Linv, int64_t N, int64_t ldi, double* Kinv, int64_t ldk, int rank, int nranks);

int gpp_lauum_rows_range(gpp_handle_t h, const double* Linv, int64_t N, int64_t ldi, double* Kinv, int64_t ldk, int rank,
                         int nranks, int64_t row0, int64_t row1);

int gpp_transpose(gpp_handle_t h, const double* src, int64_t lds, int64_t rows, int64_t cols, double* dst, int64_t ldd);

int gpp_mll_reduce(gpp_handle_t h, const double* U, int64_t ld, const double* Linv, int64_t ldi, int64_t N,
                   const double* r, double* z, double* out3);

int gpp_alpha(gpp_handle_t h, const double* Linv, int64_t ldi, int64_t N, const double* z, double* alpha);

int gpp_grad_reduce(gpp_handle_t h, const double* U, int64_t N, int D, const double* w, const double* sf2,
                    const int32_t* grp, int S, int kind, int d_split, const double* alpha, const double* Kinv,
                    int64_t ldk, int dU, double* g_w, double* g_sf2, double* g_tau, double* g_U);

int gpp_loo_scalars(gpp_handle_t h, const double* Linv, int64_t ldi, int64_t N, const double* alpha, const double* y, double* d,
                    double* mu, double* s2, double* a, double* sqrtb, double* loo);

int gpp_sym_rowscale(gpp_handle_t h, const double* Kinv, int64_t N, int64_t ldk, const double* s, double* S, int64_t lds);

int gpp_loo_grad_reduce(gpp_handle_t h, const double* U, int64_t N, int D, const double* w, const double* sf2,
                        const int32_t* grp, int S, int kind, int d_split, const double* alpha, const double* beta,
                        const double* C, int64_t ldc, int dU, double* g_w, double* g_sf2, double* g_tau, double* g_U);

int gpp_grad_reduce_rows(gpp_handle_t h, const double* U, int64_t N, int D, const double* w, const double* sf2,
                         const int32_t* grp, int S, int kind, int d_split, const double* alpha, const double* Kinv,
                         int64_t ldk, int dU, int64_t nb, int rank, int nranks, double* g_w, double* g_sf2, double* g_tau,
                         double* g_U);

int gpp_grad_reduce_cols(gpp_handle_t h, const double* U, int64_t N, int D, const double* w, const double* sf2,
                         const int32_t* grp, int S, int kind, int d_split, const double* alpha, const double* Kinv,
                         int64_t ldk, int dU, int64_t nb, int rank, int nranks, double* g_w, double* g_sf2, double* g_tau,
                         double* g_U, int compact);

int gpp_predict(gpp_handle_t h, const double* Linv, int64_t ldi, int64_t N, const double* alpha, const double* Ksn,
                int64_t lds, int64_t M, const double* kss, double* V, int64_t ldv, double* mean_out, double* var_out);

int gpp_predict_tn(gpp_handle_t h, const double* Linv, int64_t ldi, int64_t N, const double* z, const double* Kns, int64_t ldk,
                   int64_t M, const double* kss, double* V, int64_t ldv, double* mean_out, double* var_out);

int gpp_cross_grad(gpp_handle_t h, const double* Ua, int64_t M, const double* Ub, int64_t N, int D, const double* w,
                   const double* sf2, int kind, int d_split, const double* gmean, const double* alpha, const double* gvar,
                   const double* B, int64_t ldb, double* g_Ua, int dA, double* g_Ub, int dB, double* g_w, double* g_sf2);

int gpp_gemm(gpp_handle_t h, int transA, int transB, int64_t M, int64_t N, int64_t K, double alpha, const double* A,
             int64_t lda, const double* B, int64_t ldb, double beta, double* C, int64_t ldc, int a_mask, int b_mask,
             int klo_mode, int khi_mode, int c_tri);

int gpp_gemm_batched(gpp_handle_t h, int transA, int transB, int64_t M, int64_t N, int64_t K, double alpha, const double* A,
                     int64_t lda, int64_t sA, const double* B, int64_t ldb, int64_t sB, double beta, double* C, int64_t ldc,
                     int64_t sC, int batch, int a_mask, int b_mask, int klo_mode, int khi_mode, int c_tri);

int gpp_kernel_build_batched(gpp_handle_t h, const double* U, int64_t sU, int64_t N, int D, const double* w, const double* sf2,
                             const double* tau, const int32_t* grp, int S, double jitter, int kind, int d_split, int uplo,
                             double* Ky, int64_t ld, int64_t sK, int batch);
int gpp_potrf_batched(gpp_handle_t h, double* A, int64_t N, int64_t ld, int64_t sA, double* Linv, int64_t ldi, int64_t sLi,
                      int32_t* info_dev, int batch);
int gpp_trtri_batched(gpp_handle_t h, const double* U, int64_t N, int64_t ld, int64_t sA, double* Linv, int64_t ldi,
                      int64_t sLi, double* T, int64_t ldt, int64_t sT, int batch);
int gpp_lauum_batched(gpp_handle_t h, const double* Linv, int64_t N, int64_t ldi, int64_t sLi, double* Kinv, int64_t ldk,
                      int64_t sK, int batch);
int gpp_mll_reduce_batched(gpp_handle_t h, const double* U, int64_t ld, int64_t sA, const double* Linv, int64_t ldi,
                           int64_t sLi, int64_t N, const double* r, double* z, int64_t sv, double* out3, int batch);
int gpp_alpha_batched(gpp_handle_t h, const double* Linv, int64_t ldi, int64_t sLi, int64_t N, const double* z, double* alpha,
                      int64_t sv, int batch);
int gpp_grad_reduce_batched(gpp_handle_t h, const double* U, int64_t sU, int64_t N, int D, const double* w, const double* sf2,
                            const int32_t* grp, int S, int kind, int d_split, const double* alpha, int64_t sv,
                            const double* Kinv, int64_t ldk, int64_t sK, int dU, double* g_w, double* g_sf2, double* g_tau,
                            double* g_U, int batch);

int gpp_loo_scalars_batched(gpp_handle_t h, const double* Linv, int64_t ldi, int64_t sLi, int64_t N, const double* alpha,
                            const double* y, double* d, double* mu, double* s2, double* a, double* sqrtb, int64_t sv, double* loo,
                            int batch);
int gpp_sym_rowscale_batched(gpp_handle_t h, const double* Kinv, int64_t N, int64_t ldk, int64_t sK, const double* s, int64_t sv,
                             double* S, int64_t lds, int64_t sS, int batch);
int gpp_loo_grad_reduce_batched(gpp_handle_t h, const double* U, int64_t sU, int64_t N, int D, const double* w, const double* sf2,
                                const int32_t* grp, int S, int kind, int d_split, const double* alpha, const double* beta,
                                int64_t sv, const double* C, int64_t ldc, int64_t sC, int dU, double* g_w, double* g_sf2,
                                double* g_tau, double* g_U, int batch);

int gpp_cv_blocks(gpp_handle_t h, const double* Linv, int64_t ldi, int64_t N, const int32_t* idx, const int32_t* off, int nfolds,
                  int mp, double* B, int64_t ldb, int64_t sB);
int gpp_cv_rows(gpp_handle_t h, const double* G, int64_t ldg, int64_t sG, const int32_t* idx, const int32_t* off, int nfolds,
                const double* Psq, int64_t ldp, int64_t N, double* S, int64_t lds);

int gpp_chol_append(gpp_handle_t h, double* A, int64_t ld, double* Linv, int64_t ldi, int64_t N, int64_t q, const double* k,
                    int64_t ldk, const double* C, int64_t ldc, const double* rq, double* z, double* alpha, int32_t* info_dev);

// ... 13 lines not shown
```

Before: 7.954 evals/s.

## Fuse z/alpha triangular matvecs into the LAUUM-grad launch via counter-gated workgroups

Adds a persistent-style LAUUM-gradient kernel whose first workgroups compute z = Linv·r and alpha = Linv^T·z as triangular matvecs. They signal progress through device atomic counters, and the GEMM tiles wait on those counters before reading alpha in their epilogue. This removes the separate mll_reduce matvec launches and their serialization before the LAUUM, and lets the matvec bandwidth overlap with tile compute. It also unrolls the trmv row loops 8-way. The change adds spin-waiting with a timeout fallback, a host-pinned status flag, and a dependency on workgroup dispatch order.

```diff
diff --git a/gp-plus_amd/_lib.py b/gp-plus_amd/_lib.py
--- a/gp-plus_amd/_lib.py
+++ b/gp-plus_amd/_lib.py
@@ -41,6 +41,9 @@
     "gpp_lauum": (c_int, [c_void_p, c_void_p, c_int64, c_int64, c_void_p, c_int64]),
     "gpp_lauum_grad": (c_int, [c_void_p, c_void_p, c_int64, c_int64, c_void_p, c_int, c_void_p, c_void_p, c_void_p, c_int, c_int, c_int,
                                c_void_p, c_void_p, c_void_p, c_void_p]),
+    "gpp_lauum_grad_carry": (c_int, [c_void_p, c_void_p, c_int64, c_int64, c_void_p, c_int, c_void_p, c_void_p, c_void_p, c_int, c_int,
+                                     c_int, c_void_p, c_void_p, c_void_p, c_void_p, c_void_p, c_void_p]),
+    "gpp_lauum_carry_status": (c_int, [c_void_p, c_void_p]),
     "gpp_post_cov_train": (c_int, [c_void_p, c_void_p, c_int64, c_int64, c_void_p, c_void_p, c_int, c_void_p, c_double, c_void_p,
                                    c_int64]),
     "gpp_syrk_rows": (c_int, [c_void_p, c_void_p, c_int64, c_void_p, c_int64, c_int64, c_int64, c_int64, c_int64, c_int, c_int]),
diff --git a/gp-plus_amd/backend.py b/gp-plus_amd/backend.py
--- a/gp-plus_amd/backend.py
+++ b/gp-plus_amd/backend.py
@@ -16,6 +16,8 @@
 UPLO_FULL, UPLO_LOWER, UPLO_UPPER = 0, 1, 2
 OPT_COOP_PANEL, OPT_PANEL_FAULT, OPT_PANEL_TIMEOUT_MS, OPT_EXEC_SCHED, OPT_DAG_SCHED = 1, 2, 3, 4, 5
 OPT_GEMM_TILE = 6
+OPT_LAUUM_CARRY = 7
+LAUUM_CARRY_MIN_N = 5248
 OP_MLL_EVAL, OP_PREDICT, OP_PREDICT_GRAD = 0, 1, 2
 OP_APPLY = 3
 OP_APPLY_GRAD = 4
@@ -338,6 +340,40 @@
             raise GppError("gpp_lauum_grad: the handle's scratch workspace is missing or too small")
         check(status, "gpp_lauum_grad")
         return True
+
+    @_on_own_device
+    def lauum_grad_carry(self, Linv, U, w, sf2, grp, S, r, z, alpha, dU, g_w, g_sf2, g_tau, *, kind=KIND_RBF) -> bool:
+        N, D = U.shape
+        for t, n in ((Linv, "Linv"), (U, "U"), (w, "w"), (sf2, "sf2"), (r, "r"), (z, "z"), (alpha, "alpha"), (g_w, "g_w"),
+                     (g_sf2, "g_sf2"), (g_tau, "g_tau")):
+            _need(t, torch.float64, n)
+        if grp is not None:
+            self._check_groups(grp, N, S)
+        if not U.is_contiguous():
+            raise GppError("U must be contiguous")
+        self.ensure_workspace(OP_MLL_EVAL, N, 0, D, S)
+        self._stream()
+        status = self.lib.gpp_lauum_grad_carry(self.h, Linv.data_ptr(), N, _ld(Linv), U.data_ptr(), D, w.data_ptr(), sf2.data_ptr(),
+                                               _ptr(grp), S, kind, dU, r.data_ptr(), z.data_ptr(), alpha.data_ptr(), g_w.data_ptr(),
+                                               g_sf2.data_ptr(), g_tau.data_ptr())
+        if status == NOT_SUPPORTED:
+            return False
+        if status == NO_WORKSPACE:
+            raise GppError("gpp_lauum_grad_carry: the handle's scratch workspace is missing or too small")
+        check(status, "gpp_lauum_grad_carry")
+        return True
+
+    def lauum_carry_timed_out(self) -> bool:
+        out = ctypes.c_int(0)
+        check(self.lib.gpp_lauum_carry_status(self.h, ctypes.byref(out)), "gpp_lauum_carry_status")
+        return out.value != 0
+
+    def check_lauum_carry(self) -> None:
+        if not getattr(self, "_carry_reported", False) and self.lauum_carry_timed_out():
+            self._carry_reported = True
+            raise GppError("gpp_lauum_grad_carry: a wait inside the previous evaluation's LAUUM launch timed out (another kernel "
+                           "holding the GPU for seconds); that evaluation's gradients are invalid — evaluate again: the handle "
+                           "now runs z, alpha and the LAUUM as separate launches (GPP_LAUUM_CARRY=0 selects them from the start)")
 
     @_on_own_device
     def post_cov_train(self, Kinv, tau, grp, d, out, *, jitter=0.0):
diff --git a/gp-plus_amd/csrc/gpp_api.hip b/gp-plus_amd/csrc/gpp_api.hip
--- a/gp-plus_amd/csrc/gpp_api.hip
+++ b/gp-plus_amd/csrc/gpp_api.hip
@@ -15,6 +15,7 @@
     e.coop_panel = num("GPP_COOP_PANEL", 1) != 0;
     e.dag_sched = num("GPP_DAG_SCHED", 1) != 0;
     e.dag_phased = num("GPP_DAG_PHASED", 0) != 0;
+    e.lauum_carry = num("GPP_LAUUM_CARRY", 1) != 0;
     e.shard_list = num("GPP_SHARD_LIST", 1) != 0;
     e.shard_workers = (int)num("GPP_SHARD_WORKERS", 0);
     e.shard_fill = (int)num("GPP_SHARD_FILL", -1);
@@ -759,6 +760,18 @@
     if (h->panel_flags) (void)hipFree(h->panel_flags);
     h->panel_flags = nullptr;
   }
+  h->lauum_carry = gpp_env().lauum_carry ? 1 : 0;
+  h->carry_ctr = nullptr;
+  h->carry_host = nullptr;
+  if (hipMalloc(reinterpret_cast<void**>(&h->carry_ctr), (GPP_CARRY_WORDS + 1) * sizeof(int32_t)) != hipSuccess ||
+      hipMemset(h->carry_ctr, 0, (GPP_CARRY_WORDS + 1) * sizeof(int32_t)) != hipSuccess ||
+      hipHostMalloc(reinterpret_cast<void**>(&h->carry_host), sizeof(int32_t), hipHostMallocDefault) != hipSuccess) {
+    (void)hipGetLastError();
+    if (h->carry_ctr) (void)hipFree(h->carry_ctr);
+    h->carry_ctr = nullptr;
+  } else {
+    *h->carry_host = 0;
+  }
   *out = h;
   return 0;
 }
@@ -775,6 +788,8 @@
   if (h->handoff) (void)hipEventDestroy(h->handoff);
   if (h->shard_ready) (void)hipEventDestroy(h->shard_ready);
   if (h->panel_flags) (void)hipFree(h->panel_flags);
+  if (h->carry_ctr) (void)hipFree(h->carry_ctr);
+  if (h->carry_host) (void)hipHostFree(h->carry_host);
   for (int i = 0; i < GPP_DAG_PLANS; ++i)
     if (h->dag_plans[i]) gpp_dag_free(h->dag_plans[i]);
   gpp_shard_release_comm(h);
@@ -807,6 +822,7 @@
   if (option == GPP_OPT_COOP_PANEL) h->coop_panel = value ? 1 : 0;
   else if (option == GPP_OPT_PANEL_FAULT) h->panel_fault = value ? 1 : 0;
   else if (option == GPP_OPT_DAG_SCHED || option == GPP_OPT_EXEC_SCHED) h->dag_sched = value ? 1 : 0;
+  else if (option == GPP_OPT_LAUUM_CARRY) h->lauum_carry = value ? 1 : 0;
   else if (option == GPP_OPT_PANEL_TIMEOUT_MS) {
     if (value < 1 || value > 60000) return -3;
     h->panel_timeout_ms = value;
@@ -1327,6 +1343,53 @@
   return 0;
 }
 
+int gpp_lauum_grad_carry(gpp_handle_t h, const double* Linv, int64_t N, int64_t ldi, const double* U, int D, const double* w,
+                         const double* sf2, const int32_t* grp, int S, int kind, int dU, const double* r, double* z, double* alpha,
+                         double* g_w, double* g_sf2, double* g_tau) {
+  if (!h) return -1;
+  if (N < 0) return -3;
+  if (int q = check_mat(Linv, ldi, N, 2)) return q;
+  if (!U) return -5;
+  if (D < 1 || D > 64) return -6;
+  if (!w) return -7;
+  if (!sf2) return -8;
+  if (S < 1 || S > 64) return -10;
+  if (kind < 0 || kind > 2) return -11;
+  if (dU < 0 || dU > D) return -12;
+  if (!r || !aligned16(r)) return -13;
+  if (!z || !aligned16(z)) return -14;
+  if (!alpha) return -15;
+  if (!g_w) return -16;
+  if (!g_sf2) return -17;
+  if (!g_tau) return -18;
+  if (kind != GPP_KIND_RBF || D > 16 || dU != 0 || N < GPP_LAUUM_CARRY_MIN_N) return GPP_NOT_SUPPORTED;
+  if (!h->lauum_carry || !h->carry_ctr || *static_cast<volatile int32_t*>(h->carry_host) != 0) return GPP_NOT_SUPPORTED;
+  hipStreamCaptureStatus cap = hipStreamCaptureStatusNone;
+  if (hipStreamIsCapturing(h->stream, &cap) != hipSuccess || cap != hipStreamCaptureStatusNone) {
+    (void)hipGetLastError();
+    return GPP_NOT_SUPPORTED;
+  }
+  if (!h->ws || h->ws_bytes < gpp_lauum_grad_ws_bytes(N, D)) return GPP_NO_WORKSPACE;
+  GemmArgs g = mk(Linv, ldi, Linv, ldi, nullptr, ldi, N, N, N, 1.0, 0.0);
+  g.a_mask = 2; g.b_mask = 2; g.klo_mode = 3; g.c_lower = 1;
+  const int64_t tiles = (N + NBLK - 1) / NBLK, nrec = tiles * (tiles + 1) / 2;
+  double* rec = reinterpret_cast<double*>(h->ws);
+  double* wdiag = rec + nrec * (D + 1);
+  const CarryArgs c{r, z, alpha, h->carry_ctr};
+  GPP_TRY(gpp_launch_fill_i32(h->stream, h->carry_ctr, GPP_CARRY_WORDS, 0));
+  GPP_TRY(gpp_launch_lauum_carry(h->stream, g, GradEpiArgs{U, w, sf2, alpha, rec, wdiag, D}, c));
+  GPP_TRY(gpp_launch_grad_finish(h->stream, rec, nrec, D, S, wdiag, grp, N, g_w, g_sf2, g_tau));
+  GPP_TRY(hipMemcpyAsync(h->carry_host, h->carry_ctr + GPP_CARRY_WORDS, sizeof(int32_t), hipMemcpyDeviceToHost, h->stream));
+  return 0;
+}
+
+int gpp_lauum_carry_status(gpp_handle_t h, int* timed_out) {
+  if (!h) return -1;
+  if (!timed_out) return -2;
+  *timed_out = (h->carry_host && *static_cast<volatile int32_t*>(h->carry_host) != 0) ? 1 : 0;
+  return 0;
+}
+
 int gpp_post_cov_train(gpp_handle_t h, const double* Kinv, int64_t N, int64_t ldk, const double* tau, const int32_t* grp, int S,
                        const double* d, double jitter, double* A, int64_t lda) {
   if (!h) return -1;
diff --git a/gp-plus_amd/csrc/gpp_gemm.hip b/gp-plus_amd/csrc/gpp_gemm.hip
--- a/gp-plus_amd/csrc/gpp_gemm.hip
+++ b/gp-plus_amd/csrc/gpp_gemm.hip
@@ -406,15 +406,51 @@
 
 }
 
+__device__ __forceinline__ int exec_load(const int* p) { return __hip_atomic_load(p, __ATOMIC_RELAXED, __HIP_MEMORY_SCOPE_AGENT); }
+
+__device__ __forceinline__ bool exec_poll(int* counters, int w0, int v0, int w1, int v1, long long budget, int32_t* info,
+                                          int status = GPP_INFO_EXEC_TIMEOUT) {
+  long long t0 = 0;
+  bool timed = false;
+  for (;;) {
+    const bool r0 = w0 < 0 || exec_load(counters + w0) >= v0;
+    const bool r1 = w1 < 0 || exec_load(counters + w1) >= v1;
+    if (r0 & r1) return true;
+    if (!timed) {
+      t0 = (long long)wall_clock64();
+      timed = true;
+    }
+    const long long waited = (long long)wall_clock64() - t0;
+    if (exec_load(counters) != 0) return false;
+    if (waited > budget) {
+      const long long ms = waited / 100000;
+      __hip_atomic_store(counters, 1, __ATOMIC_RELAXED, __HIP_MEMORY_SCOPE_AGENT);
+      atomicCAS(info, 0, status | (int)(ms > 0xFFFFF ? 0xFFFFF : ms));
+      return false;
+    }
+    __builtin_amdgcn_s_sleep(2);
+  }
+}
+__device__ __forceinline__ void exec_raise_wg(int* counters, int id) {
+  asm volatile("s_waitcnt vmcnt(0)" ::: "memory");
+  __syncthreads();
+  if (threadIdx.x == 0) {
+    __builtin_amdgcn_fence(__ATOMIC_RELEASE, "agent");
+    asm volatile("s_waitcnt vmcnt(0)" ::: "memory");
+    __hip_atomic_fetch_add(counters + id, 1, __ATOMIC_RELAXED, __HIP_MEMORY_SCOPE_AGENT);
+  }
+}
+
 __device__ __forceinline__ double wave_sum(double v) {
 #pragma unroll
   for (int o = 32; o > 0; o >>= 1) v += __shfl_xor(v, o);
   return v;
 }
-template <int DT>
+template <int DT, bool CARRY = false>
 struct GradEpilogue {
   GradEpiArgs e;
   int tile;
+  int* ctr = nullptr;
   static constexpr int T = 128;
   static constexpr int FIXED = 2 * DT * T + 2 * T + DT + 4 * (DT + 1);
   static constexpr int SLAB = (FIXED + 1) & ~1;
@@ -435,12 +471,33 @@
       sa[x] = (d < D && row0 + r < N) ? e.U[(int64_t)(row0 + r) * D + d] : 0.0;
       sb[x] = (d < D && col0 + r < N) ? e.U[(int64_t)(col0 + r) * D + d] : 0.0;
     }
-    if (tid < T) {
-      sal_a[tid] = (row0 + tid < N) ? e.alpha[row0 + tid] : 0.0;
-      sal_b[tid] = (col0 + tid < N) ? e.alpha[col0 + tid] : 0.0;
+    if constexpr (!CARRY) {
+      if (tid < T) {
+        sal_a[tid] = (row0 + tid < N) ? e.alpha[row0 + tid] : 0.0;
+        sal_b[tid] = (col0 + tid < N) ? e.alpha[col0 + tid] : 0.0;
+      }
+    } else if (wave == 0) {
+      int ok = 1;
+      if (lane == 0) {
+        ok = exec_poll(ctr, 3, GPP_CARRY_RA, -1, 0, GPP_CARRY_BUDGET, ctr + GPP_CARRY_WORDS) ? 1 : 0;
+        red[0] = ok ? 1.0 : 0.0;
+      }
+      ok = __builtin_amdgcn_readfirstlane(ok);
+      __builtin_amdgcn_fence(__ATOMIC_ACQUIRE, "agent");
+      if (ok) {
+        for (int x = lane; x < T; x += 64) {
+          sal_a[x] = (row0 + x < N) ? e.alpha[row0 + x] : 0.0;
+          sal_b[x] = (col0 + x < N) ? e.alpha[col0 + x] : 0.0;
+        }
+      }
     }
     if (tid < DT) sw[tid] = (tid < D) ? e.w[tid] : 0.0;
     __syncthreads();
+    if constexpr (CARRY) {
+      const bool ok = red[0] != 0.0;
+      __syncthreads();
+      if (!ok) return;
+    }
 
     const double sf2 = *e.sf2;
     const GppExpConsts ec = gpp_exp_consts();
@@ -537,6 +594,46 @@
   while (tm * (tm + 1) / 2 > t) --tm;
   const int tn = t - tm * (tm + 1) / 2;
   gemm_tile<2, 64, 64, 2, 16, 2, 2>(p, tm, tn, p.A, p.B, nullptr, nullptr, smem, GemmNoHook(), GradEpilogue<DT>{e, t});
+}
+
+template <int DT>
+__global__ __launch_bounds__(256, 2) void gpp_lauum_carry_f64(GemmArgs p, GradEpiArgs e, CarryArgs c) {
+  extern __shared__ __attribute__((aligned(16))) double smem[];
+  __shared__ int s_t;
+  constexpr int Rz = GPP_CARRY_RZ, Ra = GPP_CARRY_RA;
+  const int tid = threadIdx.x, wave = tid >> 6, lane = tid & 63;
+  if (tid == 0) s_t = __hip_atomic_fetch_add(c.ctr + 1, 1, __ATOMIC_RELAXED, __HIP_MEMORY_SCOPE_AGENT);
+  __syncthreads();
+  const int t = __builtin_amdgcn_readfirstlane(s_t);
+  const int64_t N = p.M;
+  if (t < Rz) {
+    for (int64_t i = 4 * (int64_t)t + wave; i < N; i += 4 * Rz) {
+      const double v = gpp_trmv_lower_row(p.A, p.lda, i, c.r, lane);
+      if (lane == 0) c.z[i] = v;
+    }
+    exec_raise_wg(c.ctr, 2);
+    return;
+  }
+  if (t < Rz + Ra) {
+    __syncthreads();
+    if (tid == 0) s_t = exec_poll(c.ctr, 2, Rz, -1, 0, GPP_CARRY_BUDGET, c.ctr + GPP_CARRY_WORDS) ? 1 : 0;
+    __syncthreads();
+    const int ok = s_t;
+    __builtin_amdgcn_fence(__ATOMIC_ACQUIRE, "agent");
+    if (!ok) return;
+    for (int64_t j = 4 * (int64_t)(t - Rz) + wave; j < N; j += 4 * Ra) {
+      const double v = gpp_trmv_upper_row(p.A, p.lda, N, j, c.z, lane);
+      if (lane == 0) c.alpha[j] = v;
+    }
+    exec_raise_wg(c.ctr, 3);
+    return;
+  }
+  const int tt = t - (Rz + Ra);
+  int tm = (int)((sqrtf(8.f * (float)tt + 1.f) - 1.f) * 0.5f);
+  while ((tm + 1) * (tm + 2) / 2 <= tt) ++tm;
+  while (tm * (tm + 1) / 2 > tt) --tm;
+  const int tn = tt - tm * (tm + 1) / 2;
+  gemm_tile<2, 64, 64, 2, 16, 2, 2>(p, tm, tn, p.A, p.B, nullptr, nullptr, smem, GemmNoHook(), GradEpilogue<DT, true>{e, tt, c.ctr});
 }
 
 template <bool MAT>
@@ -851,31 +948,6 @@
 #define GPP_AS4 __attribute__((address_space(4)))
 typedef const GemmArgs GPP_AS4 CGemmArgs;
 
-__device__ __forceinline__ int exec_load(const int* p) { return __hip_atomic_load(p, __ATOMIC_RELAXED, __HIP_MEMORY_SCOPE_AGENT); }
-
-__device__ __forceinline__ bool exec_poll(int* counters, int w0, int v0, int w1, int v1, long long budget, int32_t* info,
-                                          int status = GPP_INFO_EXEC_TIMEOUT) {
-  long long t0 = 0;
-  bool timed = false;
-  for (;;) {
-    const bool r0 = w0 < 0 || exec_load(counters + w0) >= v0;
-    const bool r1 = w1 < 0 || exec_load(counters + w1) >= v1;
-    if (r0 & r1) return true;
-    if (!timed) {
-      t0 = (long long)wall_clock64();
-      timed = true;
-    }
-    const long long waited = (long long)wall_clock64() - t0;
-    if (exec_load(counters) != 0) return false;
-    if (waited > budget) {
-      const long long ms = waited / 100000;
-      __hip_atomic_store(counters, 1, __ATOMIC_RELAXED, __HIP_MEMORY_SCOPE_AGENT);
-      atomicCAS(info, 0, status | (int)(ms > 0xFFFFF ? 0xFFFFF : ms));
-      return false;
-    }
-    __builtin_amdgcn_s_sleep(2);
-  }
-}
 
 typedef const DagTask GPP_AS4 CDagTask;
 __global__ __launch_bounds__(64) void gpp_dag_bind(const GemmArgs* rel, GemmArgs* abs, int n, DagBases bases) {
@@ -1095,6 +1167,32 @@
   return hipGetLastError();
 }
 
+hipError_t gpp_launch_lauum_carry(hipStream_t s, const GemmArgs& a_in, const GradEpiArgs& e, const CarryArgs& c) {
+  GemmArgs a = a_in;
+  if (a.M <= 0) return hipSuccess;
+  if (a.M != a.N || a.c_lower != 1 || e.D < 1 || e.D > 16 || e.alpha != c.alpha) return hipErrorInvalidValue;
+  a.tiles_m = a.tiles_n = (a.M + 127) / 128;
+  a.row_mod = 0;
+  a.swz = 0;
+  a.batch_fast = 0;
+  a.tile_base = 0;
+  const int64_t nt = (int64_t)a.tiles_m * (a.tiles_m + 1) / 2 + GPP_CARRY_RZ + GPP_CARRY_RA;
+  constexpr size_t bytes = gemm_lds_bytes(2, 128, 128, 16, 2);
+  auto* fn = e.D <= 8 ? gpp_lauum_carry_f64<8> : gpp_lauum_carry_f64<16>;
+  static std::atomic<bool> attr_set[2][64];
+  int dev = 0;
+  hipError_t err = hipGetDevice(&dev);
+  if (err != hipSuccess) return err;
+  const int which = e.D <= 8 ? 0 : 1;
+  if (dev < 0 || dev >= 64 || !attr_set[which][dev]) {
+    err = hipFuncSetAttribute(reinterpret_cast<const void*>(fn), hipFuncAttributeMaxDynamicSharedMemorySize, (int)bytes);
+    if (err != hipSuccess) return err;
+    if (dev >= 0 && dev < 64) attr_set[which][dev] = true;
+  }
+  hipLaunchKernelGGL(fn, dim3((unsigned)nt), dim3(256), bytes, s, a, e, c);
+  return hipGetLastError();
+}
+
 hipError_t gpp_launch_post_cross(hipStream_t s, int variant, const GemmArgs& a_in, const PostCrossArgs& e) {
   GemmArgs a = a_in;
   if (a.M <= 0 || a.N <= 0 || a.K <= 0 || (variant != 0 && variant != 2)) return hipErrorInvalidValue;
diff --git a/gp-plus_amd/csrc/gpp_internal.h b/gp-plus_amd/csrc/gpp_internal.h
--- a/gp-plus_amd/csrc/gpp_internal.h
+++ b/gp-plus_amd/csrc/gpp_internal.h
@@ -40,6 +40,9 @@
   int dag_sched;
   int gemm_tile;
   int split_builds;
+  int lauum_carry;
+  int32_t* carry_ctr;
+  int32_t* carry_host;
   gpp_comm_t comm;
   int comm_rank, comm_nranks;
   void* rccl_comm;
@@ -71,6 +74,7 @@
   bool coop_panel;
   bool dag_sched;
   bool dag_phased;
+  bool lauum_carry;
   bool shard_list;
   int shard_workers;
   int shard_fill;
@@ -118,6 +122,64 @@
   p = __builtin_fma(p, r, 1.0);
   p = __builtin_fma(p, r, 1.0);
   return __builtin_ldexp(p, (int)n);
+}
+
+typedef double gpp_v2d __attribute__((ext_vector_type(2)));
+__device__ __forceinline__ double gpp_wave_sum64(double v) {
+#pragma unroll
+  for (int o = 32; o > 0; o >>= 1) v += __shfl_xor(v, o);
+  return v;
+}
+__device__ __forceinline__ void gpp_trmv_fma8(const double* __restrict__ row, const double* __restrict__ x, double& acc) {
+  gpp_v2d t[8], xx[8];
+#pragma unroll
+  for (int u = 0; u < 8; ++u) {
+    t[u] = *reinterpret_cast<const gpp_v2d*>(row + 128 * u);
+    xx[u] = *reinterpret_cast<const gpp_v2d*>(x + 128 * u);
+  }
+#pragma unroll
+  for (int u = 0; u < 8; ++u) {
+    acc = fma(t[u].x, xx[u].x, acc);
+    acc = fma(t[u].y, xx[u].y, acc);
+  }
+}
+__device__ __forceinline__ double gpp_trmv_lower_row(const double* __restrict__ T, int64_t ldt, int64_t i, const double* __restrict__ x,
+                                                     int lane) {
+  const double* row = T + i * ldt;
+  double acc = 0.0;
+  const int64_t len = i + 1;
+  const int64_t len2 = len & ~(int64_t)1;
+  int64_t k = 2 * lane;
+  for (; k + 7 * 128 < len2; k += 8 * 128) gpp_trmv_fma8(row + k, x + k, acc);
+  for (; k < len2; k += 128) {
+    const gpp_v2d t = *reinterpret_cast<const gpp_v2d*>(row + k);
+    const gpp_v2d xx = *reinterpret_cast<const gpp_v2d*>(x + k);
+    acc = fma(t.x, xx.x, acc);
+    acc = fma(t.y, xx.y, acc);
+  }
+  if (lane == 0 && (len & 1)) acc = fma(row[len - 1], x[len - 1], acc);
+  return gpp_wave_sum64(acc);
+}
+__device__ __forceinline__ double gpp_trmv_upper_row(const double* __restrict__ T, int64_t ldt, int64_t N, int64_t j,
+                                                     const double* __restrict__ x, int lane) {
+  const double* row = T + j * ldt;
+  double acc = 0.0;
+  int64_t k0 = j;
+  if (k0 & 1) {
+    if (lane == 0) acc = fma(row[k0], x[k0], acc);
+    ++k0;
+  }
+  const int64_t nvec = (N - k0) >> 1;
+  int64_t v = lane;
+  for (; v + 7 * 64 < nvec; v += 8 * 64) gpp_trmv_fma8(row + k0 + 2 * v, x + k0 + 2 * v, acc);
+  for (; v < nvec; v += 64) {
+    const gpp_v2d t = *reinterpret_cast<const gpp_v2d*>(row + k0 + 2 * v);
+    const gpp_v2d xx = *reinterpret_cast<const gpp_v2d*>(x + k0 + 2 * v);
+    acc = fma(t.x, xx.x, acc);
+    acc = fma(t.y, xx.y, acc);
+  }
+  if (lane == 0 && ((N - k0) & 1)) acc = fma(row[N - 1], x[N - 1], acc);
+  return gpp_wave_sum64(acc);
 }
 #endif
 
@@ -169,6 +231,16 @@
   int D;
 };
 hipError_t gpp_launch_lauum_grad(hipStream_t s, const GemmArgs& lauum, const GradEpiArgs& e);
+constexpr int GPP_CARRY_WORDS = 4;
+constexpr int GPP_CARRY_RZ = 64, GPP_CARRY_RA = 64;
+constexpr long long GPP_CARRY_BUDGET = 200000000;
+struct CarryArgs {
+  const double* r;
+  double* z;
+  double* alpha;
+  int* ctr;
+};
+hipError_t gpp_launch_lauum_carry(hipStream_t s, const GemmArgs& lauum, const GradEpiArgs& e, const CarryArgs& c);
 
 struct PostCrossArgs {
   const double* Uc;
diff --git a/gp-plus_amd/csrc/gpp_reduce.hip b/gp-plus_amd/csrc/gpp_reduce.hip
--- a/gp-plus_amd/csrc/gpp_reduce.hip
+++ b/gp-plus_amd/csrc/gpp_reduce.hip
@@ -21,18 +21,7 @@
   T += (int64_t)blockIdx.y * sT;
   x += (int64_t)blockIdx.y * sv;
   y += (int64_t)blockIdx.y * sv;
-  const double* row = T + i * ldt;
-  double acc = 0.0;
-  const int64_t len = i + 1;
-  const int64_t len2 = len & ~(int64_t)1;
-  for (int64_t k = 2 * lane; k < len2; k += 128) {
-    const v2d t = *reinterpret_cast<const v2d*>(row + k);
-    const v2d xx = *reinterpret_cast<const v2d*>(x + k);
-    acc = fma(t.x, xx.x, acc);
-    acc = fma(t.y, xx.y, acc);
-  }
-  if (lane == 0 && (len & 1)) acc = fma(row[len - 1], x[len - 1], acc);
-  acc = wave_sum(acc);
+  const double acc = gpp_trmv_lower_row(T, ldt, i, x, lane);
   if (lane == 0) y[i] = acc;
 }
 
@@ -45,22 +34,7 @@
   T += (int64_t)blockIdx.y * sT;
   x += (int64_t)blockIdx.y * sv;
   y += (int64_t)blockIdx.y * sv;
-  const double* row = T + j * ldt;
-  double acc = 0.0;
-  int64_t k0 = j;
-  if (k0 & 1) {
-    if (lane == 0) acc = fma(row[k0], x[k0], acc);
-    ++k0;
-  }
-  const int64_t nvec = (N - k0) >> 1;
-  for (int64_t v = lane; v < nvec; v += 64) {
-    const v2d t = *reinterpret_cast<const v2d*>(row + k0 + 2 * v);
-    const v2d xx = *reinterpret_cast<const v2d*>(x + k0 + 2 * v);
-    acc = fma(t.x, xx.x, acc);
-    acc = fma(t.y, xx.y, acc);
-  }
-  if (lane == 0 && ((N - k0) & 1)) acc = fma(row[N - 1], x[N - 1], acc);
-  acc = wave_sum(acc);
+  const double acc = gpp_trmv_upper_row(T, ldt, N, j, x, lane);
   if (lane == 0) y[j] = acc;
 }
 
diff --git a/gp-plus_amd/linalg.py b/gp-plus_amd/linalg.py
--- a/gp-plus_amd/linalg.py
+++ b/gp-plus_amd/linalg.py
@@ -74,12 +74,15 @@
 
 FUSED_GRAD_MIN_N = 5120
 
+LAUUM_CARRY_MIN_N = 6912
+
 STAGE_EVENTS = None
 
 
 class _stage:
     def __init__(self, name: str):
         self.name = name
+        self.keep = True
 
     def __enter__(self):
         if STAGE_EVENTS is not None:
@@ -88,7 +91,7 @@
         return self
 
     def __exit__(self, *exc):
-        if STAGE_EVENTS is not None:
+        if STAGE_EVENTS is not None and self.keep:
             e1 = torch.cuda.Event(enable_timing=True)
             e1.record()
             STAGE_EVENTS.append((self.name, self.e0, e1))
@@ -124,6 +127,7 @@
     def attempt(jit):
         if ws.N >= LOOKAHEAD_MIN_N:
             torch.cuda.current_stream(ctx.index).synchronize()
+            ctx.check_lauum_carry()
         with _stage("kernel_build"):
             pass
         with _stage("potrf"):
@@ -195,6 +199,16 @@
         def rest():
             with _stage("trtri"):
                 gctx.trtri(ws.A, ws.Li, ws.Ki)
+            if need_grad and getattr(fn, "carries_products", False) and N >= LAUUM_CARRY_MIN_N and kind == KIND_RBF \
+                    and not need_U and not torch.cuda.is_current_stream_capturing():
+                with _stage("lauum") as st:
+                    carried = st.keep = gctx.lauum_grad_carry(ws.Li, *ops, ws.r, ws.z, ws.alpha, *grads[:4], kind=kind)
+                if carried:
+                    with _stage("mll_reduce"):
+                        gctx.mll_scalars(ws.A, ws.z, ws.out3)
+                    with _stage("grad_reduce"):
+                        pass
+                    return
             with _stage("mll_reduce"):
                 gctx.mll_reduce(ws.A, ws.Li, ws.r, ws.z, ws.out3)
             if need_grad or fn.value_needs_alpha:
@@ -210,7 +224,7 @@
 
 class ExactMLLFunction(torch.autograd.Function):
 
-    capturable, value_needs_alpha = True, False
+    capturable, value_needs_alpha, carries_products = True, False, True
 
     @staticmethod
     def forward(ctx, U, w, sf2, tau, mean, y, grp, kind, d_split, dU, slot):
diff --git a/include/gpp.h b/include/gpp.h
--- a/include/gpp.h
+++ b/include/gpp.h
@@ -39,6 +39,7 @@
 #define GPP_OPT_EXEC_SCHED 4
 #define GPP_OPT_DAG_SCHED 5
 #define GPP_OPT_GEMM_TILE 6
+#define GPP_OPT_LAUUM_CARRY 7
 #define GPP_INFO_PANEL_TIMEOUT (1 << 30)
 #define GPP_INFO_EXEC_TIMEOUT ((1 << 30) | (1 << 29))
 int gpp_set_option(gpp_handle_t h, int option, int value);
@@ -82,6 +83,12 @@
 int gpp_lauum_grad(gpp_handle_t h, const double* Linv, int64_t N, int64_t ldi, const double* U, int D, const double* w,
                    const double* sf2, const int32_t* grp, int S, int kind, int dU, const double* alpha, double* g_w,
                    double* g_sf2, double* g_tau);
+
+#define GPP_LAUUM_CARRY_MIN_N 5248
+int gpp_lauum_grad_carry(gpp_handle_t h, const double* Linv, int64_t N, int64_t ldi, const double* U, int D, const double* w,
+                         const double* sf2, const int32_t* grp, int S, int kind, int dU, const double* r, double* z, double* alpha,
+                         double* g_w, double* g_sf2, double* g_tau);
+int gpp_lauum_carry_status(gpp_handle_t h, int* timed_out);
 
 int gpp_post_cov_train(gpp_handle_t h, const double* Kinv, int64_t N, int64_t ldk, const double* tau, const int32_t* grp, int S,
                        const double* d, double jitter, double* A, int64_t lda);
```

Result: no change. 7.971 evals/s, median of 6 (+0.2%).
